# BillyXYB/TransEditor

Hardware: AMD Instinct MI355X
Metric: 256x256 images/sec/GPU, G+D fwd+bwd, batch 16; 1/2/4/8-GPU scaling (higher is better)
Workload: dtype f32

## Files before the change

include/te_hip.h:

```cpp
#ifndef TE_HIP_H
#define TE_HIP_H

#include <stdint.h>

#ifdef __cplusplus
extern "C" {
#endif

#define TE_ABI_VERSION 3

#define TE_ERR_NULL -1
#define TE_ERR_SHAPE -2
#define TE_ERR_UNSUPPORTED -3
#define TE_ERR_WORKSPACE -4

typedef void* te_stream_t;

int te_version(void);
const char* te_last_error_string(void);
const char* te_arch(void);

int te_bias_act_f32(float* out, const float* x, const float* b, const float* ref, int act, int grad,
                    float alpha, float scale, int64_t size_x, int64_t step_b, int64_t size_b,
                    te_stream_t stream);
int te_bias_act_f16(void* out, const void* x, const void* b, const void* ref, int act, int grad,
                    float alpha, float scale, int64_t size_x, int64_t step_b, int64_t size_b,
                    te_stream_t stream);
int te_bias_act_f64(double* out, const double* x, const double* b, const double* ref, int act, int grad,
                    float alpha, float scale, int64_t size_x, int64_t step_b, int64_t size_b,
                    te_stream_t stream);

int64_t te_bias_act_bwd_ws_floats(int64_t outer, int64_t C, int64_t inner);
int te_bias_act_bwd_f32(float* gi, float* gb, float* ws, const float* g, const float* ref, float alpha, float scale,
                        int64_t outer, int64_t C, int64_t inner, te_stream_t stream);
int te_bias_act_bwd_rgb_supported(int64_t outer, int64_t C, int64_t inner);
int te_bias_act_bwd_rgb_f32(float* gi, float* gb, float* ws, const float* g, const float* ref, const float* grgb, const float* wrgb,
                            const float* srgb, float wscale, float alpha, float scale, int64_t outer, int64_t C, int64_t inner,
                            te_stream_t stream);

int te_upfirdn2d_f32(float* out, const float* x, const float* k, int64_t major, int in_h, int in_w,
                     int minor, int kh, int kw, int up_x, int up_y, int down_x, int down_y, int pad_x0,
                     int pad_x1, int pad_y0, int pad_y1, const float* b, int64_t size_b, int act,
                     float alpha, float scale, te_stream_t stream);
int te_upfirdn2d_f16(void* out, const void* x, const void* k, int64_t major, int in_h, int in_w,
                     int minor, int kh, int kw, int up_x, int up_y, int down_x, int down_y, int pad_x0,
                     int pad_x1, int pad_y0, int pad_y1, te_stream_t stream);
int te_upfirdn2d_f64(double* out, const double* x, const double* k, int64_t major, int in_h, int in_w,
                     int minor, int kh, int kw, int up_x, int up_y, int down_x, int down_y, int pad_x0,
                     int pad_x1, int pad_y0, int pad_y1, te_stream_t stream);


#define TE_CONV_3X3 0
#define TE_CONV_T2 1
#define TE_CONV_S2 2
#define TE_CONV_1X1 3
#define TE_CONV_3X3W 4
#define TE_CONV_3X3W6 5

#define TE_CONV_S2S6 6

#define TE_CONV_T2S6 7

#define TE_CONV_1X1S6 8
#define TE_CONV_KINDS 9

#define TE_PACK_FWD 0
#define TE_PACK_DGRAD 1
#define TE_PACK_SWAP 2
#define TE_PACK_WFWD 3
#define TE_PACK_WDGRAD 4
#define TE_PACK_W6FWD 5
#define TE_PACK_W6DGRAD 6
#define TE_PACK_S6FWD 7
#define TE_PACK_S6SWAP 8
#define TE_PACK_T6FWD 9
#define TE_PACK_T6SWAP 10
#define TE_PACK_P6FWD 11
#define TE_PACK_P6DGRAD 12
#define TE_PACK_KINDS 13

int64_t te_conv_packed_numel(int kind_pack, int Co, int Ci, int ksize);
int te_conv_pack_weights_f32(float* wp, const float* w, float wscale, int kind_pack, int Co, int Ci,
                             int ksize, te_stream_t stream);
int te_conv_pack_weights2_f32(float* wp_a, int kind_a, float* wp_b, int kind_b, const float* w, float wscale, int Co, int Ci,
                              int ksize, te_stream_t stream);

int te_conv_pack_weights_multi_f32(int n, float* const* wp, const float* const* w, const float* wscale, const int* kind_pack,
                                   const int* Co, const int* Ci, const int* ksize, te_stream_t stream);

int te_conv_f32(float* out, const float* in, const float* wp, const float* isc, const float* osc,
                const float* bias, int act, int kind, int B, int K, int M, int H, int W,
                te_stream_t stream);
int te_conv_splitk_count(int kind, int B, int K, int M, int H, int W);
int te_conv_wino_supported(int B, int K, int M, int H, int W);
int te_conv_wino6_supported(int B, int K, int M, int H, int W);
int te_conv_s2s6_supported(int B, int K, int M, int H, int W);
int te_conv_t2s6_supported(int B, int K, int M, int H, int W);
int te_conv_p1s6_supported(int B, int K, int M, int H, int W);
int te_conv_wino6_form(int form);
int te_conv_wino6_tiles_per_block(int n);
int te_conv_s2s6_form(int form);
int te_conv_t2s6_form(int form);
int64_t te_conv_t2s6_ws_floats(int B, int K, int H);
int te_conv_ws_f32(float* out, float* ws, const float* in, const float* wp, const float* isc, const float* osc,
                   const float* bias, int act, int kind, int B, int K, int M, int H, int W, te_stream_t stream);
int te_conv_res_f32(float* out, float* ws, const float* in, const float* wp, const float* isc, const float* osc,
                    const float* bias, const float* res, const float* mask_ref, float mask_gain, int act, int kind, int B,
                    int K, int M, int H, int W, te_stream_t stream);

int te_wgrad_slab_count(int kind, int B, int Co, int Ci, int H, int W);
int te_wgrad_pair_form(int kind, int Co, int Ci, int H, int W);
int te_wgrad_split_supported(int kind, int Co, int Ci, int H, int W);
int te_wgrad_split_bf16(int on);
int te_wgrad_t2_wide(int on);
enum { TE_WG6_FP32 = 0, TE_WG6_3X3 = 1, TE_WG6_3X3_PAIR = 2, TE_WG6_T2_WIDE = 3, TE_WG6_T2 = 4, TE_WG6_T2_MASKED = 5, TE_WG6_1X1 = 6 };
int te_wgrad6_form(int kind, int B, int Co, int Ci, int H, int W, int NB);
int te_wgrad_f32(float* slabs, const float* g, const float* x, int kind, int B, int Co, int Ci, int H,
                 int W, int S, te_stream_t stream);
int te_wgrad_group_plan(int kind, int B, int Co, int Ci, int H, int W, int* NB, int* S);
int te_wgrad_group_f32(float* slabs, const float* g, const float* x, int kind, int B, int Co, int Ci, int H, int W, int S, int NB,
                       te_stream_t stream);

int64_t te_wgrad_reduce_ws_floats(int B, int S, int Co, int Ci, int taps, int want_w, int want_isc, int want_osc);
int te_wgrad_reduce_f32(float* gw, float* gisc, float* gosc, float* ws, const float* slabs, const float* w,
                        float wscale, const float* isc, const float* osc, int B, int S, int Co, int Ci,
                        int taps, te_stream_t stream);

int te_rgb_supported(int M, int K, int HW);
int te_rgb_fwd_f32(float* out, const float* x, const float* w, const float* isc, const float* bias, float wscale, int B,
                   int K, int HW, te_stream_t stream);
int te_rgb_dgrad_f32(float* gx, const float* g, const float* w, const float* isc, float wscale, int B, int K, int HW,
                     te_stream_t stream);
int te_rgb_expand_f32(float* out, const float* x3, const float* w, const float* bias, int act, float wscale, int B, int K,
                      int HW, te_stream_t stream);
int te_rgb_wgrad_slab_count(int B, int K, int HW);
int te_rgb_wgrad_f32(float* slabs, const float* g, const float* x, int B, int K, int HW, int S, te_stream_t stream);
int te_rgb_wgrad_sum_f32(float* slabs, const float* g, const float* x, int B, int K, int HW, int S, te_stream_t stream);

int te_attn_fwd_f32(float* o, float* sim, const float* q, const float* k, const float* v, float scale,
                    int N, int G, int M, int L, int D, te_stream_t stream);
int te_attn_bwd_f32(float* gq, float* gk, float* gv, const float* go, const float* gsim_or_null,
                    const float* q, const float* k, const float* v, const float* sim, float scale, int N,
                    int G, int M, int L, int D, te_stream_t stream);

int te_blur_actgrad_tiles(int in_h, int in_w, int kh, int kw, int pad_x0, int pad_x1, int pad_y0, int pad_y1);
int te_blur_actgrad_f32(float* gx, float* partial, const float* g, const float* ref, const float* k, int64_t major, int in_h,
                        int in_w, int kh, int kw, int pad_x0, int pad_x1, int pad_y0, int pad_y1, float alpha, float scale,
                        te_stream_t stream);
int te_blur_gradact_f32(float* gx, float* partial, const float* g, const float* ref, const float* k, int64_t major, int in_h,
                        int in_w, int kh, int kw, int pad_x0, int pad_x1, int pad_y0, int pad_y1, float alpha, float scale,
                        te_stream_t stream);

int te_upfirdn2d_plan(int64_t major, int in_h, int in_w, int minor, int kh, int kw, int up_x, int up_y, int down_x, int down_y,
                      int pad_x0, int pad_x1, int pad_y0, int pad_y1, int* zgroups, int* tiles);
int te_blur_actgrad_plan(int64_t major, int in_h, int in_w, int kh, int kw, int pad_x0, int pad_x1, int pad_y0, int pad_y1,
                         int* zgroups, int* tiles);
int te_blur_gradact_plan(int64_t major, int in_h, int in_w, int kh, int kw, int pad_x0, int pad_x1, int pad_y0, int pad_y1,
                         int* zgroups, int* tiles);
int64_t te_upfirdn2d_direct_cover(int64_t outputs);
int64_t te_chan_scale_cover(int64_t rows, int64_t hw, int aligned16);
int64_t te_bias_act_f32_cover(int64_t size_x, int64_t step_b, int aligned16, int* vec);
int64_t te_bias_act_any_cover(int64_t size_x);
int64_t te_conv_finalize_cover(int64_t outputs);
int64_t te_small_gemm_splitk_finish_cover(int I, int J);
int te_conv_pack_plan(int kind_pack, int Co, int Ci, int ksize, int* blocks, int* tiles);
int te_wgrad_reduce_plan(int B, int S, int Co, int Ci, int taps, int* parts, int64_t* cover);

int te_small_gemm_f32(float* c, float* pre, const float* a, const float* b, const float* bias, const float* residual,
                      float* arowsum, float rs_scale, int I, int J, int K, int64_t sai, int64_t sak, int64_t sbk,
                      int64_t sbj, float alpha, float beta, int act, te_stream_t stream);

int te_small_gemm_splitk_f32(float* c, float* pre, float* ws, int S, const float* a, const float* b, const float* bias,
                             const float* residual, int I, int J, int K, int64_t sai, int64_t sak, int64_t sbk, int64_t sbj,
                             float alpha, float beta, int act, te_stream_t stream);

int te_minibatch_stddev_fwd_f32(float* y, const float* x, int B, int group, int C, int HW, float eps, te_stream_t stream);
int te_minibatch_stddev_bwd_f32(float* gx, const float* gy, const float* x, int B, int group, int C, int HW, float eps,
                                te_stream_t stream);

int te_layer_norm_supported(int64_t R, int N);
int te_layer_norm_fwd_f32(float* y, float* stats, const float* x, int64_t R, int N, float eps, te_stream_t stream);
int te_layer_norm_bwd_f32(float* gx, const float* g, const float* y, const float* stats, int64_t R, int N, te_stream_t stream);

int te_pixel_norm_supported(int64_t B, int D, int C);
int te_pixel_norm_fwd_f32(float* y, float* r, const float* x, int64_t B, int D, int C, float eps, te_stream_t stream);
int te_pixel_norm_bwd_f32(float* gx, const float* g, const float* y, const float* r, int64_t B, int D, int C, te_stream_t stream);

int te_small_gemm_batched_f32(float* c, const float* a, const float* b, const float* bias, int nz, int64_t za, int64_t zc,
                              int64_t zb, int64_t zbias, const int64_t* b_tab, const int64_t* bias_tab, int I, int J, int K,
                              int64_t sai, int64_t sak, int64_t sbk, int64_t sbj, int64_t sci, int64_t scj, float alpha,
                              float beta, int act, te_stream_t stream);

int te_demod_fwd_f32(float* d, float* wsq, const float* w, const float* s, float wscale, float eps, int B, int Co, int Ci,
                     int T, te_stream_t stream);
int te_demod_bwd_f32(float* gw, float* gs, const float* gd, const float* d, const float* w, const float* wsq,
                     const float* s, float wscale, int B, int Co, int Ci, int T, int accumulate, te_stream_t stream);

int te_mt_adam_f32(const int64_t* table, const int32_t* chunks, int n_tensors, int n_chunks, int chunk_elems, double lr,
                   double beta1, double beta2, double eps, int step, te_stream_t stream);
int te_mt_ema_f32(const int64_t* table, const int32_t* chunks, int n_tensors, int n_chunks, int chunk_elems, double decay,
                  te_stream_t stream);

int te_chan_scale_f32(float* out, const float* x, const float* s, int64_t rows, int64_t hw, te_stream_t stream);
int te_chan_dot_f32(float* out, const float* a, const float* b, int64_t rows, int64_t hw, te_stream_t stream);

int te_lpips_stem_fwd_f32(float* out, const float* x, const float* w, const float* b, int N, int H, int W, te_stream_t stream);
int te_lpips_stem_dgrad_f32(float* gx, const float* g, const float* y1, const float* w, int N, int H, int W, te_stream_t stream);
int te_maxpool2_fwd_f32(float* out, const float* x, int64_t planes, int H, int W, te_stream_t stream);
int te_maxpool2_bwd_f32(float* gx, const float* g, const float* x, int64_t planes, int H, int W, te_stream_t stream);
int te_lpips_normalize_f32(float* out, const float* x, int N, int C, int64_t HW, te_stream_t stream);
int te_lpips_head_blocks(int64_t HW);
int te_lpips_head_fwd_f32(float* partial, const float* f, const float* t, const float* w, int N, int Nt, int C, int64_t HW,
                          te_stream_t stream);
int te_lpips_dist_f32(float* d, const float* const* partial, const int64_t* hw, int L, int N, te_stream_t stream);
int te_lpips_head_bwd_f32(float* gf, const float* gin, const float* gd, const float* f, const float* t, const float* w, int N, int Nt,
                          int C, int64_t HW, int relu_mask, te_stream_t stream);
int te_lpips_pair_head_fwd_f32(float* partial, const float* f, const float* w, int N, int C, int64_t HW, te_stream_t stream);
int te_crop_resize_bilinear_f32(float* out, const float* img, int B, int H, int W, int y0, int x0, int hc, int wc, int h, int w,
                                te_stream_t stream);

int64_t te_noise_reg_ws_floats(const int* sizes, int n, int B);
int te_noise_reg_fwd_f32(float* loss, float* ws, float* const* maps, const int* sizes, int n, int B, te_stream_t stream);
int te_noise_reg_bwd_f32(float* const* grads, float* tws, const float* gloss, const float* ws, float* const* maps, const int* sizes,
                         int n, int B, te_stream_t stream);
int te_noise_normalize_f32(float* const* maps, const int* sizes, int n, int B, te_stream_t stream);

int64_t te_prdc_ws_bytes(int N, int M, int D, int k);
int te_row_sqnorm_f32(float* out, const float* x, int N, int D, te_stream_t stream);
int te_prdc_knn_f32(float* r2, const float* x, const float* nx, int N, int D, int k, void* ws, te_stream_t stream);
int te_prdc_counts_f32(int32_t* col_count, int32_t* row_any, float* row_min, const float* x, const float* nx, const float* rr2,
                       const float* y, const float* ny, const float* rf2, int N, int M, int D, void* ws, te_stream_t stream);

int te_vgg_stem_fwd_f32(float* out, const float* x, const float* w, const float* b, int N, int H, int W, te_stream_t stream);
int te_adaptive_avgpool_f32(float* out, const float* x, int64_t planes, int H, int W, int OH, int OW, te_stream_t stream);
// ... 65 lines not shown
```

transeditor_amd/_lib.py:

```python
import ctypes as C
import os

import torch

from . import _abi

_HERE = os.path.dirname(os.path.abspath(__file__))
LIB_PATH = os.path.join(_HERE, 'libte_hip.so')
HEADER_PATH = os.path.join(_HERE, '..', 'include', 'te_hip.h')
_lib = _protos = None

CONV_3X3, CONV_T2, CONV_S2, CONV_1X1, CONV_3X3W, CONV_3X3W6, CONV_S2S6, CONV_T2S6, CONV_1X1S6 = 0, 1, 2, 3, 4, 5, 6, 7, 8
(PACK_FWD, PACK_DGRAD, PACK_SWAP, PACK_WFWD, PACK_WDGRAD, PACK_W6FWD, PACK_W6DGRAD, PACK_S6FWD, PACK_S6SWAP, PACK_T6FWD,
 PACK_T6SWAP, PACK_P6FWD, PACK_P6DGRAD) = range(13)


def _header_text():
    if not os.path.exists(HEADER_PATH):
        raise RuntimeError(f'{HEADER_PATH} is missing: the bindings of libte_hip.so are read from it')
    with open(HEADER_PATH) as f:
        return f.read()


def _prototypes():
# ... 69 lines not shown
                           + (f'contiguous={t.is_contiguous()} ' if dense else '') + '(no CPU path exists)')
    _on_current_device(t)
    return t.data_ptr()


_ptr_as = _ptr


def _raw(t):
    return _ptr(t, dense=False)


def _stream():
    return torch.cuda.current_stream().cuda_stream


def _aligned16(t):
    if t is None or t.data_ptr() % 16 == 0:
        return t
    return t.clone(memory_format=torch.contiguous_format)


_OTHER = {torch.float16: 'f16', torch.float64: 'f64'}


def _dispatch(x):
    return (_OTHER[x.dtype], x.dtype) if x.dtype in _OTHER else ('f32', torch.float32)


def _inner(shape):
    n = 1
    for d in shape[2:]:
        n *= d
    return n


@_op
def bias_act(x, b, ref, act, grad, alpha, scale):
    x = x.contiguous()
    sfx, dt = _dispatch(x)
    out = torch.empty_like(x)
    _launch('te_bias_act_' + sfx, _ptr(out, dt), _ptr(x, dt), _ptr(b, dt), _ptr(ref, dt), act, grad, alpha, scale, x.numel(),
            _inner(x.shape), b.numel() if b is not None else 1)
    return out


def _bias_grad_buffers(want_bias, outer, Cn, inner, device):
    if not want_bias:
        return None, None
    n = lib().te_bias_act_bwd_ws_floats(outer, Cn, inner)
    return (torch.empty(Cn, device=device, dtype=torch.float32),
            torch.empty(n, device=device, dtype=torch.float32) if n > 0 else None)


@_op
def bias_act_bwd(g, ref, alpha, scale, want_bias=True):
    g = g.contiguous()
    if g.dtype in _OTHER:
        gi = bias_act(g, None, ref, 3, 1, alpha, scale)
        return gi, (gi.sum(dim=[0] + list(range(2, gi.ndim))) if want_bias else None)
    gi = torch.empty_like(g)
    Cn, inner = g.shape[1], _inner(g.shape)
    gb, ws = _bias_grad_buffers(want_bias, g.shape[0], Cn, inner, g.device)
    _launch('te_bias_act_bwd_f32', _ptr(gi), _ptr(gb), _ptr(ws), _ptr(g), _ptr(ref), alpha, scale, g.shape[0], Cn, inner)
    return gi, gb


def bias_act_bwd_rgb_supported(shape):
    return bool(lib().te_bias_act_bwd_rgb_supported(shape[0], shape[1], _inner(shape)))


@_op
def bias_act_bwd_rgb(g, ref, grgb, wrgb, srgb, wscale, alpha, scale, want_bias=True):
    ref, grgb = _aligned16(ref.contiguous()), _aligned16(grgb.contiguous())
    g = _aligned16(g.contiguous()) if g is not None else None
    gi = torch.empty_like(ref)
    Cn, inner = ref.shape[1], _inner(ref.shape)
    gb, ws = _bias_grad_buffers(want_bias, ref.shape[0], Cn, inner, ref.device)
    _launch('te_bias_act_bwd_rgb_f32', _ptr(gi), _ptr(gb), _ptr(ws), _ptr(g), _ptr(ref), _ptr(grgb), _ptr(wrgb.contiguous()),
            _ptr(srgb.contiguous()) if srgb is not None else None, wscale, alpha, scale, ref.shape[0], Cn, inner)
    return gi, gb


@_op
def upfirdn2d_raw(x, k, up, down, pad, bias=None, act=0, alpha=0.2, scale=1.0):
    x = x.contiguous()
    B, Cn, H, W = x.shape
    kh, kw = k.shape
    px0, px1, py0, py1 = pad
    oh = (H * up[1] + py0 + py1 - kh) // down[1] + 1
    ow = (W * up[0] + px0 + px1 - kw) // down[0] + 1
    if oh <= 0 or ow <= 0:
        raise RuntimeError(f'upfirdn2d: empty output {oh}x{ow}')
    out = torch.empty(B, Cn, oh, ow, device=x.device, dtype=x.dtype)
    sfx, dt = _dispatch(x)
    if sfx != 'f32':
        if bias is not None or act:
            raise RuntimeError('upfirdn2d: the fused bias / activation epilogue exists in fp32 only')
        k = k.to(dt)
    args = [_ptr(out, dt), _ptr(x, dt), _ptr(k.contiguous(), dt), B * Cn, H, W, 1, kh, kw, up[0], up[1], down[0], down[1],
            px0, px1, py0, py1]
    if sfx == 'f32':
        args += [_ptr(bias), bias.numel() if bias is not None else 1, act, alpha, scale]
    _launch('te_upfirdn2d_' + sfx, *args)
    return out


@_op
def blur_actgrad(g, ref, k_flipped, pad, alpha, scale):
    g, ref = g.contiguous(), ref.contiguous()
    B, Cn, H, W = g.shape
    kh, kw = k_flipped.shape
    px0, px1, py0, py1 = pad
    tiles = lib().te_blur_actgrad_tiles(H, W, kh, kw, px0, px1, py0, py1)
    if tiles <= 0:
        raise RuntimeError(f'te_blur_actgrad_tiles failed ({tiles})')
    gx = torch.empty(B, Cn, H + py0 + py1 - kh + 1, W + px0 + px1 - kw + 1, device=g.device, dtype=g.dtype)
    partial = torch.empty(B, Cn, tiles, device=g.device, dtype=g.dtype)
    _launch('te_blur_actgrad_f32', _ptr(gx), _ptr(partial), _ptr(g), _ptr(ref), _ptr(k_flipped.contiguous()), B * Cn, H, W, kh, kw, px0,
            px1, py0, py1, alpha, scale)
    return gx, partial.sum(dim=(0, 2))


@_op
def blur_gradact(g, ref, k_flipped, pad, alpha, scale):
    g, ref = g.contiguous(), ref.contiguous()
    B, Cn, H, W = g.shape
    kh, kw = k_flipped.shape
    px0, px1, py0, py1 = pad
    oh, ow = H + py0 + py1 - kh + 1, W + px0 + px1 - kw + 1
    if tuple(ref.shape) != (B, Cn, oh, ow):
        raise RuntimeError(f'blur_gradact: ref {tuple(ref.shape)} is not the shape of the adjoint blur output {(B, Cn, oh, ow)}')
    tiles = lib().te_blur_actgrad_tiles(H, W, kh, kw, px0, px1, py0, py1)
    if tiles <= 0:
        raise RuntimeError(f'te_blur_actgrad_tiles failed ({tiles})')
    gx = torch.empty(B, Cn, oh, ow, device=g.device, dtype=g.dtype)
    partial = torch.empty(B, Cn, tiles, device=g.device, dtype=g.dtype)
    _launch('te_blur_gradact_f32', _ptr(gx), _ptr(partial), _ptr(g), _ptr(ref), _ptr(k_flipped.contiguous()), B * Cn, H, W, kh, kw, px0,
            px1, py0, py1, alpha, scale)
    return gx, partial.sum(dim=(0, 2))


@_op
def conv_pack(w, kind_pack, wscale=1.0):
    w = w.contiguous()
    Co, Ci, ks, _ = w.shape
    n = lib().te_conv_packed_numel(kind_pack, Co, Ci, ks)
    wp = torch.empty(n, device=w.device, dtype=w.dtype)
    _launch('te_conv_pack_weights_f32', _ptr(wp), _ptr(w), wscale, kind_pack, Co, Ci, ks)
    return wp


@_op
def conv_pack2(w, kind_a, kind_b, wscale=1.0):
    w = w.contiguous()
    Co, Ci, ks, _ = w.shape
    wa = torch.empty(lib().te_conv_packed_numel(kind_a, Co, Ci, ks), device=w.device, dtype=w.dtype)
    wb = torch.empty(lib().te_conv_packed_numel(kind_b, Co, Ci, ks), device=w.device, dtype=w.dtype)
    _launch('te_conv_pack_weights2_f32', _ptr(wa), kind_a, _ptr(wb), kind_b, _ptr(w), wscale, Co, Ci, ks)
    return wa, wb


@_op
def conv_pack_multi(jobs):
    n = len(jobs)
    if not n:
        return
    for wp, w, _, _ in jobs:
        if not (w.is_contiguous() and wp.is_contiguous()):
            raise RuntimeError('te_hip: conv_pack_multi needs dense weights and buffers')
    arr = lambda ty, vals: (ty * n)(*vals)
    _launch('te_conv_pack_weights_multi_f32', n, arr(C.c_void_p, [_ptr(j[0]) for j in jobs]), arr(C.c_void_p, [_ptr(j[1]) for j in jobs]),
            arr(C.c_float, [float(j[3]) for j in jobs]), arr(C.c_int, [int(j[2]) for j in jobs]),
            arr(C.c_int, [j[1].shape[0] for j in jobs]), arr(C.c_int, [j[1].shape[1] for j in jobs]),
            arr(C.c_int, [j[1].shape[2] for j in jobs]))


def wino_ok(B, K, M, H, W):
    return bool(lib().te_conv_wino_supported(B, K, M, H, W))


def s2s6_ok(B, K, M, H, W):
    return bool(lib().te_conv_s2s6_supported(B, K, M, H, W))


def t2s6_ok(B, K, M, H, W):
    return bool(lib().te_conv_t2s6_supported(B, K, M, H, W))


def p1s6_ok(B, K, M, H, W):
    return bool(lib().te_conv_p1s6_supported(B, K, M, H, W))


def wino6_form(form=-1):
    return int(lib().te_conv_wino6_form(form))


def wino6_tiles_per_block(n=-1):
    return int(lib().te_conv_wino6_tiles_per_block(n))


def s2s6_form(form=-1):
    return int(lib().te_conv_s2s6_form(form))


def t2s6_form(form=-1):
    return int(lib().te_conv_t2s6_form(form))


def wino6_ok(B, K, M, H, W):
    return bool(lib().te_conv_wino6_supported(B, K, M, H, W))


def conv_out_shape(kind, B, M, H, W):
    if kind in (CONV_T2, CONV_T2S6):
        return (B, M, 2 * H + 1, 2 * W + 1)
    return (B, M, H, W)


@_op
def conv(x, wp, kind, M, H, W, isc=None, osc=None, bias=None, act=0, res=None, mask_ref=None, mask_gain=1.0):
    x = x.contiguous()
    if kind == CONV_1X1S6:
        x = _aligned16(x)
    res = _aligned16(res.contiguous()) if res is not None else None
    mask_ref = _aligned16(mask_ref.contiguous()) if mask_ref is not None else None
    B, K = x.shape[0], x.shape[1]
    out = torch.empty(conv_out_shape(kind, B, M, H, W), device=x.device, dtype=x.dtype)
    if res is not None and tuple(res.shape) != tuple(out.shape):
        raise RuntimeError(f'te_hip: residual {tuple(res.shape)} does not match the convolution output {tuple(out.shape)}')
    if mask_ref is not None and tuple(mask_ref.shape) != tuple(out.shape):
        raise RuntimeError(f'te_hip: mask reference {tuple(mask_ref.shape)} does not match the convolution output {tuple(out.shape)}')
    S = lib().te_conv_splitk_count(kind, B, K, M, H, W)
    if S < 1:
        raise RuntimeError(f'te_conv_splitk_count failed ({S})')
    ws = torch.empty((S,) + tuple(out.shape), device=x.device, dtype=x.dtype) if S > 1 else None
    if kind == CONV_T2S6:
        ws = torch.empty(B * K * H, device=x.device, dtype=x.dtype)
    _launch('te_conv_res_f32', _ptr(out), _ptr(ws), _ptr(x), _ptr(wp), _ptr(isc), _ptr(osc), _ptr(bias), _ptr(res), _ptr(mask_ref),
            mask_gain, act, kind, B, K, M, H, W)
    return out


@_op
def wgrad_slabs(g, x, kind, H, W, group=False):
    g, x = g.contiguous(), x.contiguous()
    B, Co, Ci = g.shape[0], g.shape[1], x.shape[1]
    taps = 1 if kind == CONV_1X1 else 9
    if group:
        nb, sc = C.c_int(0), C.c_int(0)
        _check(lib().te_wgrad_group_plan(kind, B, Co, Ci, H, W, C.byref(nb), C.byref(sc)), 'te_wgrad_group_plan')
        if nb.value > 1:
            slabs = torch.empty(B // nb.value, sc.value, Co, Ci, taps, device=g.device, dtype=g.dtype)
            _launch('te_wgrad_group_f32', _ptr(slabs), _ptr(g), _ptr(x), kind, B, Co, Ci, H, W, sc.value, nb.value)
            return slabs
    S = lib().te_wgrad_slab_count(kind, B, Co, Ci, H, W)
    if S <= 0:
        raise RuntimeError(f'te_wgrad_slab_count failed ({S})')
    slabs = torch.empty(B, S, Co, Ci, taps, device=g.device, dtype=g.dtype)
    _launch('te_wgrad_f32', _ptr(slabs), _ptr(g), _ptr(x), kind, B, Co, Ci, H, W, S)
    return slabs


def wgrad_t2_wide(on=-1):
    return int(lib().te_wgrad_t2_wide(on))


def wgrad_split(on=-1):
    return int(lib().te_wgrad_split_bf16(on))


def wgrad_split_ok(kind, Co, Ci, H, W):
    return bool(lib().te_wgrad_split_supported(kind, Co, Ci, H, W))


WGRAD6_FORMS = ('fp32', 'w6', 'w6pair', 't2wide', 't2narrow', 't2masked', 'p1')


def wgrad6_form(kind, B, Co, Ci, H, W, NB=1):
    return WGRAD6_FORMS[lib().te_wgrad6_form(kind, B, Co, Ci, H, W, NB)]


def wgrad_pair_form(kind, Co, Ci, H, W):
    return bool(lib().te_wgrad_pair_form(kind, Co, Ci, H, W))


@_op
def wgrad_reduce(slabs, w, wscale=1.0, isc=None, osc=None, want_w=True, want_isc=False, want_osc=False):
    B, S, Co, Ci, taps = slabs.shape
    dev, dt = slabs.device, slabs.dtype
    gw = torch.empty(Co, Ci, taps, device=dev, dtype=dt) if want_w else None
    gisc = torch.empty(B, Ci, device=dev, dtype=dt) if want_isc else None
    gosc = torch.empty(B, Co, device=dev, dtype=dt) if want_osc else None
    n = lib().te_wgrad_reduce_ws_floats(B, S, Co, Ci, taps, int(want_w), int(want_isc), int(want_osc))
    if n < 0:
        raise RuntimeError(f'te_wgrad_reduce_ws_floats failed ({n})')
    ws = torch.empty(n, device=dev, dtype=dt) if n > 0 else None
    _launch('te_wgrad_reduce_f32', _ptr(gw), _ptr(gisc), _ptr(gosc), _ptr(ws), _ptr(slabs), _ptr(w.contiguous()), wscale, _ptr(isc),
            _ptr(osc), B, S, Co, Ci, taps)
    return gw, gisc, gosc


def rgb_supported(M, K, HW):
    return bool(lib().te_rgb_supported(M, K, HW))


@_op
def rgb_fwd(x, w, isc, bias, wscale=1.0):
    x = _aligned16(x.contiguous())
    B, K, H, W = x.shape
    out = torch.empty(B, 3, H, W, device=x.device, dtype=x.dtype)
    _launch('te_rgb_fwd_f32', _ptr(out), _ptr(x), _ptr(w.contiguous()), _ptr(isc), _ptr(bias), wscale, B, K, H * W)
    return out


@_op
def rgb_dgrad(g, w, isc, K, wscale=1.0):
    g = _aligned16(g.contiguous())
    B, _, H, W = g.shape
    gx = torch.empty(B, K, H, W, device=g.device, dtype=g.dtype)
    _launch('te_rgb_dgrad_f32', _ptr(gx), _ptr(g), _ptr(w.contiguous()), _ptr(isc), wscale, B, K, H * W)
# ... 844 lines not shown
```

transeditor_amd/csrc/bias_act.hip:

```cpp
#include "te_common.h"
#include <hip/hip_fp16.h>

namespace {

__device__ __forceinline__ float act_one(float x, float r, int mode, float alpha) {
    switch (mode) {
        case 30: return x > 0.f ? x : x * alpha;
        case 31: return r > 0.f ? x : x * alpha;
        case 12:
        case 32: return 0.f;
        default: return x;
    }
}

__global__ __launch_bounds__(256) void bias_act_vec4_kernel(float4* __restrict__ out, const float4* __restrict__ x,
                                                            const float* __restrict__ b, const float4* __restrict__ ref,
                                                            int mode, float alpha, float scale, uint32_t n4,
                                                            uint32_t step_b4, uint32_t size_b) {
    const uint32_t stride = gridDim.x * blockDim.x;
    for (uint32_t i = blockIdx.x * blockDim.x + threadIdx.x; i < n4; i += stride) {
        float4 v = x[i];
        if (b) {
            const float bb = b[(i / step_b4) % size_b];
            v.x += bb; v.y += bb; v.z += bb; v.w += bb;
        }
        float4 r = make_float4(0.f, 0.f, 0.f, 0.f);
        if (ref) r = ref[i];
        float4 y;
        y.x = act_one(v.x, r.x, mode, alpha) * scale;
        y.y = act_one(v.y, r.y, mode, alpha) * scale;
        y.z = act_one(v.z, r.z, mode, alpha) * scale;
        y.w = act_one(v.w, r.w, mode, alpha) * scale;
        out[i] = y;
    }
}

__global__ __launch_bounds__(256) void bias_act_scalar_kernel(float* __restrict__ out, const float* __restrict__ x,
                                                              const float* __restrict__ b, const float* __restrict__ ref,
                                                              int mode, float alpha, float scale, int64_t n,
                                                              int64_t step_b, int64_t size_b) {
    const int64_t stride = (int64_t)gridDim.x * blockDim.x;
    for (int64_t i = (int64_t)blockIdx.x * blockDim.x + threadIdx.x; i < n; i += stride) {
        float v = x[i];
        if (b) v += b[(i / step_b) % size_b];
        const float r = ref ? ref[i] : 0.f;
        out[i] = act_one(v, r, mode, alpha) * scale;
    }
}

__device__ __forceinline__ float wave_sum(float v) {
#pragma unroll
    for (int off = 32; off > 0; off >>= 1) v += __shfl_down(v, off, 64);
    return v;
}

__device__ __forceinline__ float block_sum_256(float v, float* lds4) {
    v = wave_sum(v);
    const int lane = threadIdx.x & 63, wid = threadIdx.x >> 6;
    if (lane == 0) lds4[wid] = v;
    __syncthreads();
    return lds4[0] + lds4[1] + lds4[2] + lds4[3];
}

constexpr int kBwdVecPerThread = 4;
__global__ __launch_bounds__(256) void bias_act_bwd_rows_kernel(float4* __restrict__ gi, float* __restrict__ part,
                                                                const float4* __restrict__ g, const float4* __restrict__ ref,
                                                                float alpha, float scale, uint32_t C, uint32_t inner4) {
    __shared__ float lds4[4];
    const uint32_t c = blockIdx.y, n = blockIdx.z;
    const size_t row = ((size_t)n * C + c) * inner4;
    const uint32_t base = blockIdx.x * (256 * kBwdVecPerThread);
    float acc = 0.f;
#pragma unroll
    for (int it = 0; it < kBwdVecPerThread; ++it) {
        const uint32_t i = base + it * 256 + threadIdx.x;
        if (i < inner4) {
            const float4 gv = g[row + i], rv = ref[row + i];
            float4 o;
            o.x = gv.x * (rv.x > 0.f ? 1.f : alpha) * scale;
            o.y = gv.y * (rv.y > 0.f ? 1.f : alpha) * scale;
            o.z = gv.z * (rv.z > 0.f ? 1.f : alpha) * scale;
            o.w = gv.w * (rv.w > 0.f ? 1.f : alpha) * scale;
            gi[row + i] = o;
            acc += (o.x + o.y) + (o.z + o.w);
        }
    }
    if (part) {
        const float tot = block_sum_256(acc, lds4);
        if (threadIdx.x == 0) part[((size_t)c * gridDim.z + n) * gridDim.x + blockIdx.x] = tot;
    }
}

__global__ __launch_bounds__(64) void bias_parts_sum_kernel(float* __restrict__ gb, const float* __restrict__ part, uint32_t parts) {
    const float* p = part + (size_t)blockIdx.x * parts;
    float acc = 0.f;
    for (uint32_t j = threadIdx.x; j < parts; j += 64) acc += p[j];
    acc = wave_sum(acc);
    if (threadIdx.x == 0) gb[blockIdx.x] = acc;
}

__global__ __launch_bounds__(256) void bias_act_bwd_rgb_rows_kernel(float4* __restrict__ gi, float* __restrict__ part,
                                                                    const float4* __restrict__ g, const float4* __restrict__ ref,
                                                                    const float4* __restrict__ grgb, const float* __restrict__ wrgb,
                                                                    const float* __restrict__ srgb, float wscale, float alpha,
                                                                    float scale, uint32_t C, uint32_t inner4) {
    __shared__ float lds4[4];
    const uint32_t c = blockIdx.y, n = blockIdx.z;
    const size_t row = ((size_t)n * C + c) * inner4;
    const size_t rrow = (size_t)n * 3 * inner4;
    const float sc = (srgb ? srgb[(size_t)n * C + c] : 1.f) * wscale;
    const float c0 = sc * wrgb[c], c1 = sc * wrgb[C + c], c2 = sc * wrgb[2 * C + c];
    const uint32_t base = blockIdx.x * (256 * kBwdVecPerThread);
    float acc = 0.f;
#pragma unroll
    for (int it = 0; it < kBwdVecPerThread; ++it) {
        const uint32_t i = base + it * 256 + threadIdx.x;
        if (i < inner4) {
            const float4 rv = ref[row + i];
            const float4 r0 = grgb[rrow + i], r1 = grgb[rrow + inner4 + i], r2 = grgb[rrow + 2 * (size_t)inner4 + i];
            float4 gv = g ? g[row + i] : make_float4(0.f, 0.f, 0.f, 0.f);
            gv.x += c0 * r0.x + c1 * r1.x + c2 * r2.x;
            gv.y += c0 * r0.y + c1 * r1.y + c2 * r2.y;
            gv.z += c0 * r0.z + c1 * r1.z + c2 * r2.z;
            gv.w += c0 * r0.w + c1 * r1.w + c2 * r2.w;
            float4 o;
            o.x = gv.x * (rv.x > 0.f ? 1.f : alpha) * scale;
            o.y = gv.y * (rv.y > 0.f ? 1.f : alpha) * scale;
            o.z = gv.z * (rv.z > 0.f ? 1.f : alpha) * scale;
            o.w = gv.w * (rv.w > 0.f ? 1.f : alpha) * scale;
            gi[row + i] = o;
            acc += (o.x + o.y) + (o.z + o.w);
        }
    }
    if (part) {
        const float tot = block_sum_256(acc, lds4);
        if (threadIdx.x == 0) part[((size_t)c * gridDim.z + n) * gridDim.x + blockIdx.x] = tot;
    }
}

__global__ __launch_bounds__(256) void bias_act_bwd_chan_kernel(float* __restrict__ gi, float* __restrict__ gb,
                                                                const float* __restrict__ g, const float* __restrict__ ref,
                                                                float alpha, float scale, int64_t outer, int64_t C,
                                                                int64_t inner) {
    __shared__ float lds4[4];
    const int64_t c = blockIdx.x;
    const int64_t per = outer * inner;
    float acc = 0.f;
    for (int64_t e = threadIdx.x; e < per; e += 256) {
        const int64_t n = e / inner, i = e - n * inner;
        const int64_t idx = (n * C + c) * inner + i;
        const float o = g[idx] * (ref[idx] > 0.f ? 1.f : alpha) * scale;
        gi[idx] = o;
        acc += o;
    }
    if (gb) {
        const float tot = block_sum_256(acc, lds4);
        if (threadIdx.x == 0) gb[c] = tot;
    }
}

__global__ __launch_bounds__(256) void bias_act_bwd_2d_kernel(float* __restrict__ gi, float* __restrict__ gb,
                                                              const float* __restrict__ g, const float* __restrict__ ref,
                                                              float alpha, float scale, int64_t N, int64_t C) {
    const int64_t c = (int64_t)blockIdx.x * 256 + threadIdx.x;
    if (c >= C) return;
    float acc = 0.f;
    for (int64_t n = 0; n < N; ++n) {
        const int64_t idx = n * C + c;
        const float o = g[idx] * (ref[idx] > 0.f ? 1.f : alpha) * scale;
        gi[idx] = o;
        acc += o;
    }
    if (gb) gb[c] = acc;
}

inline int bias_act_grid(int64_t items) { return (int)std::min<int64_t>(te::cdiv(items, 256), te::kNumCU * 8); }
inline bool bias_act_vec(int64_t size_x, bool has_b, int64_t step_b, bool al16) {
    return (size_x % 4 == 0) && (!has_b || step_b % 4 == 0) && al16 && (size_x / 4 < (int64_t)0xFFFFFFFF);
}

template <typename T> struct AccOf { typedef T type; };
template <> struct AccOf<__half> { typedef float type; };

template <typename T>
__global__ __launch_bounds__(256) void bias_act_any_kernel(T* __restrict__ out, const T* __restrict__ x, const T* __restrict__ b,
                                                           const T* __restrict__ ref, int mode, float alpha_, float scale_,
                                                           int64_t n, int64_t step_b, int64_t size_b) {
    typedef typename AccOf<T>::type A;
    const A alpha = (A)(T)alpha_, scale = (A)(T)scale_;
    const int64_t stride = (int64_t)gridDim.x * blockDim.x;
    for (int64_t i = (int64_t)blockIdx.x * blockDim.x + threadIdx.x; i < n; i += stride) {
        A v = (A)x[i];
        if (b) v += (A)b[(i / step_b) % size_b];
        const A r = ref ? (A)ref[i] : (A)0;
        A y;
        switch (mode) {
            case 30: y = v > (A)0 ? v : v * alpha; break;
            case 31: y = r > (A)0 ? v : v * alpha; break;
            case 12:
            case 32: y = (A)0; break;
            default: y = v;
        }
        out[i] = (T)(y * scale);
    }
}

template <typename T>
int bias_act_any(T* out, const T* x, const T* b, const T* ref, int act, int grad, float alpha, float scale, int64_t size_x,
                 int64_t step_b, int64_t size_b, te_stream_t stream_, const char* what) {
    TE_REQUIRE(out && x, TE_ERR_NULL, "%s: out/x is NULL", what);
    TE_REQUIRE(size_x >= 0, TE_ERR_SHAPE, "%s: size_x < 0", what);
    TE_REQUIRE(!b || (step_b > 0 && size_b > 0), TE_ERR_SHAPE, "%s: bias given but step_b/size_b <= 0", what);
    if (size_x == 0) return 0;
    const int grid = bias_act_grid(size_x);
// ... 20 lines not shown
                               te_stream_t stream_) {
    TE_REQUIRE(out && x, TE_ERR_NULL, "te_bias_act_f32: out/x is NULL");
    TE_REQUIRE(size_x >= 0, TE_ERR_SHAPE, "te_bias_act_f32: size_x < 0");
    TE_REQUIRE(!b || (step_b > 0 && size_b > 0), TE_ERR_SHAPE, "te_bias_act_f32: bias given but step_b/size_b <= 0");
    if (size_x == 0) return 0;
    hipStream_t stream = (hipStream_t)stream_;
    const int mode = act * 10 + grad;
    const bool vec = bias_act_vec(size_x, b != nullptr, step_b, te::aligned16(out) && te::aligned16(x) && (!ref || te::aligned16(ref)));
    if (vec) {
        const uint32_t n4 = (uint32_t)(size_x / 4);
        const int grid = bias_act_grid(n4);
        bias_act_vec4_kernel<<<grid, 256, 0, stream>>>((float4*)out, (const float4*)x, b, (const float4*)ref, mode, alpha,
                                                       scale, n4, b ? (uint32_t)(step_b / 4) : 1u,
                                                       b ? (uint32_t)size_b : 1u);
    } else {
        const int grid = bias_act_grid(size_x);
        bias_act_scalar_kernel<<<grid, 256, 0, stream>>>(out, x, b, ref, mode, alpha, scale, size_x, b ? step_b : 1,
                                                         b ? size_b : 1);
    }
    return te::launch_status("te_bias_act_f32");
}

extern "C" int64_t te_bias_act_f32_cover(int64_t size_x, int64_t step_b, int aligned16_, int* vec_out) {
    if (size_x <= 0 || step_b < 0) return TE_ERR_SHAPE;
    const bool vec = bias_act_vec(size_x, step_b > 0, step_b, aligned16_ != 0);
    if (vec_out) *vec_out = vec ? 1 : 0;
    return (int64_t)bias_act_grid(vec ? size_x / 4 : size_x) * 256 * (vec ? 4 : 1);
}

extern "C" int64_t te_bias_act_any_cover(int64_t size_x) {
    return size_x > 0 ? (int64_t)bias_act_grid(size_x) * 256 : TE_ERR_SHAPE;
}

static bool bwd_rows_path(int64_t outer, int64_t C, int64_t inner) {
    return inner % 4 == 0 && inner >= 1024 && C <= 65535 && outer <= 65535;
}

extern "C" int64_t te_bias_act_bwd_ws_floats(int64_t outer, int64_t C, int64_t inner) {
    if (outer <= 0 || C <= 0 || inner <= 0 || !bwd_rows_path(outer, C, inner)) return 0;
    return C * outer * te::cdiv(inner / 4, 256 * kBwdVecPerThread);
}

extern "C" int te_bias_act_bwd_f32(float* gi, float* gb, float* ws, const float* g, const float* ref, float alpha, float scale,
                                   int64_t outer, int64_t C, int64_t inner, te_stream_t stream_) {
    TE_REQUIRE(gi && g && ref, TE_ERR_NULL, "te_bias_act_bwd_f32: gi/g/ref is NULL");
    TE_REQUIRE(outer >= 0 && C > 0 && inner > 0, TE_ERR_SHAPE, "te_bias_act_bwd_f32: bad dims");
    if (outer == 0) return 0;
    hipStream_t stream = (hipStream_t)stream_;
    if (inner == 1) {
        bias_act_bwd_2d_kernel<<<(int)te::cdiv(C, 256), 256, 0, stream>>>(gi, gb, g, ref, alpha, scale, outer, C);
    } else if (bwd_rows_path(outer, C, inner) && te::aligned16(gi) && te::aligned16(g) && te::aligned16(ref) && (!gb || ws)) {
        const uint32_t inner4 = (uint32_t)(inner / 4);
        dim3 grid((unsigned)te::cdiv(inner4, 256 * kBwdVecPerThread), (unsigned)C, (unsigned)outer);
        bias_act_bwd_rows_kernel<<<grid, 256, 0, stream>>>((float4*)gi, gb ? ws : nullptr, (const float4*)g, (const float4*)ref, alpha,
                                                           scale, (uint32_t)C, inner4);
        if (gb) bias_parts_sum_kernel<<<(int)C, 64, 0, stream>>>(gb, ws, (uint32_t)(grid.x * grid.z));
    } else {
        bias_act_bwd_chan_kernel<<<(int)C, 256, 0, stream>>>(gi, gb, g, ref, alpha, scale, outer, C, inner);
    }
    return te::launch_status("te_bias_act_bwd_f32");
}

extern "C" int te_bias_act_bwd_rgb_supported(int64_t outer, int64_t C, int64_t inner) {
    return (outer > 0 && C > 0 && bwd_rows_path(outer, C, inner)) ? 1 : 0;
}

extern "C" int te_bias_act_bwd_rgb_f32(float* gi, float* gb, float* ws, const float* g, const float* ref, const float* grgb,
                                       const float* wrgb, const float* srgb, float wscale, float alpha, float scale, int64_t outer,
                                       int64_t C, int64_t inner, te_stream_t stream_) {
    TE_REQUIRE(gi && ref && grgb && wrgb, TE_ERR_NULL, "te_bias_act_bwd_rgb_f32: gi/ref/grgb/wrgb is NULL");
    TE_REQUIRE(!gb || ws, TE_ERR_NULL, "te_bias_act_bwd_rgb_f32: the bias gradient needs the workspace (te_bias_act_bwd_ws_floats)");
    TE_REQUIRE(te_bias_act_bwd_rgb_supported(outer, C, inner), TE_ERR_UNSUPPORTED,
               "te_bias_act_bwd_rgb_f32: needs inner %% 4 == 0 and inner >= 1024 (use te_rgb_dgrad_f32 + te_bias_act_bwd_f32)");
    TE_REQUIRE(te::aligned16(gi) && (!g || te::aligned16(g)) && te::aligned16(ref) && te::aligned16(grgb), TE_ERR_UNSUPPORTED,
               "te_bias_act_bwd_rgb_f32: 16-byte aligned tensors required");
    const uint32_t inner4 = (uint32_t)(inner / 4);
    dim3 grid((unsigned)te::cdiv(inner4, 256 * kBwdVecPerThread), (unsigned)C, (unsigned)outer);
    hipStream_t stream = (hipStream_t)stream_;
    bias_act_bwd_rgb_rows_kernel<<<grid, 256, 0, stream>>>((float4*)gi, gb ? ws : nullptr, (const float4*)g, (const float4*)ref,
                                                          (const float4*)grgb, wrgb, srgb, wscale, alpha, scale, (uint32_t)C, inner4);
    if (gb) bias_parts_sum_kernel<<<(int)C, 64, 0, stream>>>(gb, ws, (uint32_t)(grid.x * grid.z));
    return te::launch_status("te_bias_act_bwd_rgb_f32");
}
```

transeditor_amd/csrc/conv.hip:

```cpp
#include "conv_common.h"
#ifdef TE_CONV_PROF
#define TE_PROF
#endif
#ifdef TE_CONV_PROF2
#define TE_PROF2
#endif
#include "te_prof.h"

namespace {

constexpr int T2_KC0 = 16;
PROF_BUFFER(conv, 8192 * 8)
template <int KIND, int TC> struct Cfg;
template <int KIND> struct Cfg<KIND, 0> { static constexpr int WM = 2, MBW = 2, NBW = 2, KC = 8, NSP = (KIND == TE_CONV_S2) ? 3 : (KIND == TE_CONV_3X3 ? 2 : 1), NQ = (KIND == TE_CONV_S2) ? 5 : 2; };
template <int KIND> struct Cfg<KIND, 1> { static constexpr int WM = 2, MBW = 1, NBW = (KIND == TE_CONV_S2) ? 2 : 4, KC = 8, NSP = (KIND == TE_CONV_S2) ? 3 : (KIND == TE_CONV_3X3 ? 2 : 1), NQ = (KIND == TE_CONV_S2) ? 5 : 4; };
template <int KIND> struct Cfg<KIND, 2> { static constexpr int WM = 1, MBW = 1, NBW = 2, KC = 8, NSP = (KIND == TE_CONV_S2) ? 5 : (KIND == TE_CONV_3X3 ? 2 : 1), NQ = (KIND == TE_CONV_S2) ? 10 : 4; };
template <> struct Cfg<TE_CONV_T2, 0> { static constexpr int WM = 2, MBW = 1, NBW = 2, KC = T2_KC0, NSP = 1, NQ = 3; };
template <> struct Cfg<TE_CONV_T2, 1> { static constexpr int WM = 2, MBW = 1, NBW = 1, KC = 16, NSP = 1, NQ = 2; };
template <> struct Cfg<TE_CONV_T2, 2> { static constexpr int WM = 1, MBW = 1, NBW = 1, KC = 16, NSP = 1, NQ = 3; };
template <> struct Cfg<TE_CONV_1X1, 3> { static constexpr int WM = 2, MBW = 2, NBW = 2, KC = 64, NSP = 1, NQ = 8; };
template <int KIND, int TC> constexpr int tile_bm() { return Cfg<KIND, TC>::WM * Cfg<KIND, TC>::MBW * 32; }
template <int KIND, int TC> constexpr int tile_cells() { return (4 / Cfg<KIND, TC>::WM) * Cfg<KIND, TC>::NBW * 32; }

struct ConvArgs {
// ... 899 lines not shown
    for (int base = 0; base < n; base += 64) {
        const int cnt = std::min(64, n - base);
        PackJobs P{};
        int64_t biggest = 0;
        for (int i = 0; i < cnt; ++i) {
            const int e = base + i;
            TE_REQUIRE(wp[e] && w[e], TE_ERR_NULL, "%s: NULL pointer in job %d", what, e);
            TE_REQUIRE(Co[e] > 0 && Ci[e] > 0 && (ksize[e] == 1 || ksize[e] == 3), TE_ERR_SHAPE, "%s: bad dims in job %d", what, e);
            TE_REQUIRE(pack_kind_ok(kind_pack[e]), TE_ERR_UNSUPPORTED, "%s: bad kind in job %d", what, e);
            const PackDims d = pack_dims(kind_pack[e], Co[e], Ci[e], ksize[e]);
            const PackDesc& pd = pack_desc(kind_pack[e]);
            TE_REQUIRE((pd.taps == ANY_TAPS || d.ntap == pd.taps) && d.M % pd.mmul == 0 && d.K % pd.kmul == 0, TE_ERR_UNSUPPORTED,
                       "%s: layout %d needs a weight of %d tap(s) with M %% %d == 0 and K %% %d == 0 (job %d)", what, kind_pack[e], pd.taps, pd.mmul, pd.kmul, e);
            P.j[i] = PackJob{wp[e], w[e], wscale[e], kind_pack[e], Ci[e], d.ntap, d.K, d.M, d.Kp, d.Mp};
            biggest = std::max<int64_t>(biggest, pack_job_tiles(d));
        }
        dim3 grid(pack_grid_x(biggest), (unsigned)cnt);
        pack_weights_multi_kernel<<<grid, 256, 0, s>>>(P);
    }
    return te::launch_status(what);
}

extern "C" int te_conv_pack_weights_f32(float* wp, const float* w, float wscale, int kind_pack, int Co, int Ci, int ksize,
                                        te_stream_t stream_) {
    return pack_launch("te_conv_pack_weights_f32", 1, &wp, &w, &wscale, &kind_pack, &Co, &Ci, &ksize, (hipStream_t)stream_);
}

extern "C" int te_conv_pack_weights2_f32(float* wp_a, int kind_a, float* wp_b, int kind_b, const float* w, float wscale, int Co,
                                         int Ci, int ksize, te_stream_t stream_) {
    float* wp[2] = {wp_a, wp_b};
    const float* ws[2] = {w, w};
    const float sc[2] = {wscale, wscale};
    const int kinds[2] = {kind_a, kind_b}, co[2] = {Co, Co}, ci[2] = {Ci, Ci}, ks[2] = {ksize, ksize};
    return pack_launch("te_conv_pack_weights2_f32", 2, wp, ws, sc, kinds, co, ci, ks, (hipStream_t)stream_);
}

extern "C" int te_conv_pack_weights_multi_f32(int n, float* const* wp, const float* const* w, const float* wscale,
                                              const int* kind_pack, const int* Co, const int* Ci, const int* ksize,
                                              te_stream_t stream_) {
    return pack_launch("te_conv_pack_weights_multi_f32", n, wp, w, wscale, kind_pack, Co, Ci, ksize, (hipStream_t)stream_);
}

constexpr int SPLITK_MINSTAGES = 4, SPLITK_BLOCKS = 2;

struct ConvPlan { int tc, ksplit, kchunk; };
static ConvPlan conv_plan(int kind, int B, int K, int M, int H, int W) {
    ConvPlan pl;
    const int Kp = roundup(K, KPAD);
    const bool t2k = (kind == TE_CONV_T2);
    int tc = tile_class(M);
    constexpr int T2_TC1_LIMIT = 1024 * 128;
    if (t2k && tc == 0 && (int64_t)B * H * W * te::cdiv(M, 64) <= (int64_t)T2_TC1_LIMIT) tc = 1;
    pl.tc = tc;
    const TileDims td = tile_dims(kind, tc);
    int r[3][4];
    conv_regions(kind, H, W, r);
    const int rh = r[0][2], rw = r[0][3];
    const CellTile t = first_cell_tile(td.cells, rh, rw);
    const int64_t base_blocks = (int64_t)te::cdiv(rw, t.TW) * te::cdiv(rh, t.TH) * te::cdiv(B, t.NS) * te::cdiv(M, td.BM);
    const int stages = Kp / td.KC;
    int ks = 1;
    if (base_blocks < te::kNumCU) ks = (int)std::min<int64_t>(te::cdiv(SPLITK_BLOCKS * te::kNumCU, base_blocks), std::max(1, stages / SPLITK_MINSTAGES));
    pl.ksplit = std::max(1, ks);
    pl.kchunk = (int)te::cdiv(stages, pl.ksplit) * td.KC;
    pl.ksplit = (int)te::cdiv(Kp, pl.kchunk);
    if (kind == TE_CONV_1X1 && tc == 0 && pl.ksplit == 1 && t.NS == 1 && K % 64 == 0) pl.tc = 3;
    return pl;
}

extern "C" int64_t te_conv_t2s6_ws_floats(int B, int K, int H) { return (B > 0 && K > 0 && H > 0) ? (int64_t)B * K * H : TE_ERR_SHAPE; }

static int conv_finalize_grid(int64_t total) { return (int)std::min<int64_t>(te::cdiv(total, 256), te::kNumCU * 8); }

extern "C" int64_t te_conv_finalize_cover(int64_t outputs) {
    return outputs > 0 ? (int64_t)conv_finalize_grid(outputs) * 256 : TE_ERR_SHAPE;
}

extern "C" int te_conv_splitk_count(int kind, int B, int K, int M, int H, int W) {
    if (B <= 0 || K <= 0 || M <= 0 || H <= 0 || W <= 0 || kind < 0 || kind >= TE_CONV_KINDS) return TE_ERR_SHAPE;
    if (kind == TE_CONV_3X3W || kind == TE_CONV_3X3W6 || kind == TE_CONV_S2S6 || kind == TE_CONV_T2S6 || kind == TE_CONV_1X1S6) return 1;
    return conv_plan(kind, B, K, M, H, W).ksplit;
}

extern "C" int te_conv_res_f32(float* out, float* ws, const float* in, const float* wp, const float* isc, const float* osc,
                               const float* bias, const float* res, const float* mask_ref, float mask_gain, int act, int kind,
                               int B, int K, int M, int H, int W, te_stream_t stream_) {
    TE_REQUIRE(out && in && wp, TE_ERR_NULL, "te_conv_f32: out/in/wp is NULL");
    TE_REQUIRE(!(res || mask_ref) || (kind != TE_CONV_T2 && kind != TE_CONV_T2S6), TE_ERR_UNSUPPORTED,
               "te_conv_res_f32: no residual / mask epilogue for the transposed kind");
    TE_REQUIRE(B > 0 && K > 0 && M > 0 && H > 0 && W > 0, TE_ERR_SHAPE, "te_conv_f32: bad dims");
    TE_REQUIRE(act == 0 || act == 3 || act == 4, TE_ERR_UNSUPPORTED, "te_conv_f32: act must be 0, 3 or 4");
    TE_REQUIRE(kind >= 0 && kind < TE_CONV_KINDS, TE_ERR_UNSUPPORTED, "te_conv_f32: unknown kind %d", kind);
    hipStream_t s = (hipStream_t)stream_;
    if (kind == TE_CONV_1X1S6) {
        TE_REQUIRE(!isc && !osc && !bias && !mask_ref && act == 0, TE_ERR_UNSUPPORTED,
                   "te_conv_f32(TE_CONV_1X1S6): plain product + residual only (no scales, bias, activation or mask)");
        return te_p1s6_launch(out, in, wp, res, B, K, M, H, W, s);
    }
    if (kind == TE_CONV_3X3W) return te_wino_launch(out, in, wp, isc, osc, bias, res, mask_ref, mask_gain, act, B, K, M, H, W, s);
    if (kind == TE_CONV_3X3W6) return te_wino6_launch(out, in, wp, isc, osc, bias, res, mask_ref, mask_gain, act, B, K, M, H, W, s);
    if (kind == TE_CONV_S2S6) return te_s2s6_launch(out, in, wp, isc, osc, bias, res, mask_ref, mask_gain, act, B, K, M, H, W, s);
    if (kind == TE_CONV_T2S6) {
        const int rc = te_t2s6_launch(out, in, wp, isc, osc, bias, act, B, K, M, H, W, s, ws);
        if (rc) return rc;
        return te_t2s6_edge_launch(out, in, wp + t6_plain_offset(K, M), isc, osc, bias, act, B, K, M, H, W, roundup(K, KPAD), roundup(M, MPAD),
                                   s, ws);
    }
    ConvArgs a{};
    a.out = out; a.ws = ws; a.in = in; a.wp = wp; a.isc = isc; a.osc = osc; a.bias = bias; a.res = res; a.mref = mask_ref; a.mgain = mask_gain; a.act = act;
    a.B = B; a.K = K; a.M = M; a.Kp = roundup(K, KPAD); a.Mp = roundup(M, MPAD); a.H = H; a.W = W;
    const ConvPlan pl = conv_plan(kind, B, K, M, H, W);
    a.ksplit = pl.ksplit; a.kchunk = pl.kchunk;
    if (a.ksplit > 1 && !a.ws) {
        a.ksplit = 1;
        a.kchunk = a.Kp;
    }
    if (a.ksplit == 1) a.ws = nullptr;
    int r[3][4];
    const int n = conv_regions(kind, H, W, r);
    a.Hi = a.Ho = H; a.Wi = a.Wo = W;
    int rc = 0;
    switch (kind) {
        case TE_CONV_3X3: rc = launch_regions<TE_CONV_3X3>(a, r, n, s, pl.tc); break;
        case TE_CONV_1X1: rc = launch_regions<TE_CONV_1X1>(a, r, n, s, pl.tc); break;
        case TE_CONV_S2: a.Hi = 2 * H + 1; a.Wi = 2 * W + 1; rc = launch_regions<TE_CONV_S2>(a, r, n, s, pl.tc); break;
        default: a.Ho = 2 * H + 1; a.Wo = 2 * W + 1; rc = launch_regions<TE_CONV_T2>(a, r, n, s, pl.tc); break;
    }
    if (rc) return rc;
    if (a.ksplit > 1 && (a.ws || osc || bias || act)) {
        const int plane = a.Ho * a.Wo;
        const int64_t total = (int64_t)B * M * plane;
        conv_finalize_kernel<<<conv_finalize_grid(total), 256, 0, s>>>(out, a.ws, a.ksplit, osc, bias, res, mask_ref, mask_gain, act, M,
                                                                        plane, total);
    }
    return te::launch_status("te_conv_f32");
}

extern "C" int te_conv_ws_f32(float* out, float* ws, const float* in, const float* wp, const float* isc, const float* osc,
                              const float* bias, int act, int kind, int B, int K, int M, int H, int W, te_stream_t stream_) {
    return te_conv_res_f32(out, ws, in, wp, isc, osc, bias, nullptr, nullptr, 1.f, act, kind, B, K, M, H, W, stream_);
}

extern "C" int te_conv_f32(float* out, const float* in, const float* wp, const float* isc, const float* osc,
                           const float* bias, int act, int kind, int B, int K, int M, int H, int W, te_stream_t stream_) {
    return te_conv_ws_f32(out, nullptr, in, wp, isc, osc, bias, act, kind, B, K, M, H, W, stream_);
}
```

transeditor_amd/csrc/conv_common.h:

```cpp
#pragma once
#include "te_common.h"
#include <stdlib.h>
#include <algorithm>

typedef float f32x16 __attribute__((ext_vector_type(16)));
typedef float f32x4 __attribute__((ext_vector_type(4)));

constexpr unsigned OOBH = 0x40000000u;

__device__ __forceinline__ __amdgpu_buffer_rsrc_t make_rsrc(const float* p, unsigned bytes) {
    return __builtin_amdgcn_make_buffer_rsrc((void*)p, 0, bytes, 0x00020000);
}
__device__ __forceinline__ float buf_load(__amdgpu_buffer_rsrc_t r, unsigned off) {
    return __builtin_bit_cast(float, __builtin_amdgcn_raw_buffer_load_b32(r, off, 0, 0));
}

constexpr int KPAD = 16;
constexpr int MPAD = 128;
constexpr int NTHREADS = 256;


int te_wino_launch(float* out, const float* in, const float* U, const float* isc, const float* osc, const float* bias, const float* res,
                   const float* mask_ref, float mask_gain, int act, int B, int K, int M, int H, int W, hipStream_t s);
int te_wino6_launch(float* out, const float* in, const float* U, const float* isc, const float* osc, const float* bias, const float* res,
                    const float* mask_ref, float mask_gain, int act, int B, int K, int M, int H, int W, hipStream_t s);
int te_s2s6_launch(float* out, const float* in, const float* U, const float* isc, const float* osc, const float* bias, const float* res,
                   const float* mask_ref, float mask_gain, int act, int B, int K, int M, int H, int W, hipStream_t s);
int te_t2s6_launch(float* out, const float* in, const float* U, const float* isc, const float* osc, const float* bias, int act,
                   int B, int K, int M, int H, int W, hipStream_t s, float* colbuf = nullptr);
int te_t2s6_edge_launch(float* out, const float* in, const float* wplain, const float* isc, const float* osc, const float* bias, int act,
                        int B, int K, int M, int H, int W, int Kp, int Mp, hipStream_t s, const float* colbuf = nullptr);
int te_p1s6_launch(float* out, const float* in, const float* U, const float* res, int B, int K, int M, int H, int W, hipStream_t s);
```

transeditor_amd/csrc/s2s6.hip:

```cpp
#include "split6_common.h"
#ifdef S2_PROF
#define TE_PROF
#endif
#include "te_prof.h"

namespace {

constexpr int WT = 512, GT = 256, KC = 16, BM = 64;
constexpr int TH = 8, TWO = 16, PH = 4;
constexpr int IR = 2 * PH + 1, IC = 2 * TWO + 1;
constexpr int CI = 18;
constexpr int NTAP = 9;
constexpr int U_SLOTS = 3 * NTAP * 2;
constexpr int TP_PLANE = IR * 2 * 2 * CI * 4;
constexpr int TP_DWORDS = 3 * TP_PLANE;
constexpr int NG = (IC + 3) / 4;
constexpr int N_ITEMS = IR * NG * 8;
constexpr int P_IN = (N_ITEMS + GT - 1) / GT;
constexpr int N_SLOT = P_IN + 16 * P_IN;
constexpr int SLOT0 = NTAP * 6 - N_SLOT;
constexpr int UA_TAPS = 5;

PROF_BUFFER(s2s6, 2048 * 8 * 8)

struct S2Args {
    float* out; const float* in; const u32x4* U; const float* isc; const float* osc; const float* bias; const float* res;
    const float* mref; float mgain; int act;
    int B, K, M, H, W, Hi, Wi, ntiles, mblocks, tiles_x, tiles_y, nt8;
};


template <bool ISC, bool TWOIMG>
__device__ __attribute__((optnone)) void s2s6_body(const S2Args& p) {
    constexpr int NIMG = TWOIMG ? 2 : 1;
    extern __shared__ __attribute__((aligned(16))) unsigned char smem_raw[];
    u32x4* ul = reinterpret_cast<u32x4*>(smem_raw);
    const int tid = threadIdx.x, lane = tid & 63, l31 = lane & 31, half = lane >> 5;
    const int wid = __builtin_amdgcn_readfirstlane(tid >> 6);
    const int grp = wid >> 2, wq = wid & 3, wm = wq >> 1, wrl = wq & 1, gt = tid & (GT - 1);
    unsigned* tl = reinterpret_cast<unsigned*>(smem_raw + U_SLOTS * 1024) + grp * TP_DWORDS;
    const u32x4* tl4 = reinterpret_cast<const u32x4*>(tl);
    int tile, mbq;
    if (!split6_tile(p.ntiles, p.nt8, p.mblocks, tile, mbq)) return;
    const int tx = tile % p.tiles_x, ty = (tile / p.tiles_x) % p.tiles_y, b = tile / (p.tiles_x * p.tiles_y);
    const int x0 = tx * TWO, y0 = ty * TH, yh = y0 + PH * grp;
    const size_t iplane = (size_t)p.Hi * p.Wi, oplane = (size_t)p.H * p.W;
    const float* inb = p.in + (size_t)b * p.K * iplane;
    const float* iscb = ISC ? p.isc + (size_t)b * p.K : nullptr;

    f32x16 acc[NIMG], accl[NIMG];
#pragma unroll
    for (int m = 0; m < NIMG; ++m)
#pragma unroll
        for (int r = 0; r < 16; ++r) { acc[m][r] = 0.f; accl[m][r] = 0.f; }

    unsigned g_off[P_IN];
    int l_off[P_IN];
    bool last_col[P_IN], live[P_IN];
    unsigned q2[P_IN];
#pragma unroll
    for (int i = 0; i < P_IN; ++i) {
        const int e = gt + GT * i;
        live[i] = e < N_ITEMS;
        const int ee = live[i] ? e : 0;
        const int cg = ee % NG, q = (ee / NG) & 7, row = ee / (NG * 8);
        last_col[i] = cg == NG - 1;
        g_off[i] = (unsigned)((2 * q * p.Hi + 2 * yh + row) * p.Wi + 2 * x0 + 4 * cg - (last_col[i] ? 3 : 0));
        l_off[i] = (((row * 2 + (q >> 2)) * 2) * CI + 2 * cg) * 4 + (q & 3);
        q2[i] = 2u * q;
    }
    const int MT = p.M >> 5;
    f32x4 rin[P_IN][2];
    f32x2 rsc[P_IN];
#pragma unroll
    for (int i = 0; i < P_IN; ++i) rsc[i] = f32x2{1.f, 1.f};
    const int nstage = p.K / KC, nimg = NIMG * nstage;
    auto fetch_scales = [&](int s) {
        if (ISC) {
#pragma unroll
            for (int i = 0; i < P_IN; ++i) rsc[i] = *reinterpret_cast<const f32x2u*>(iscb + s * KC + q2[i]);
        }
    };
    auto fetch_item = [&](int i, int s) {
#pragma unroll
        for (int h2 = 0; h2 < 2; ++h2)
            rin[i][h2] = *reinterpret_cast<const f32x4u*>(inb + ((size_t)s * KC + h2) * iplane + g_off[i]);
    };
    auto issue = [&](int s) {
        fetch_scales(s);
#pragma unroll
        for (int i = 0; i < P_IN; ++i) fetch_item(i, s);
    };
    auto issue_u = [&](int uh, int j) {
        const u32x4* us = p.U + (size_t)(TWOIMG ? j >> 1 : j) * 27 * MT * 64;
        const int mb = TWOIMG ? 2 * mbq + (j & 1) : mbq;
        const int ntap = uh ? NTAP - UA_TAPS : UA_TAPS, tap0 = uh ? UA_TAPS : 0, n = ntap * 6;
#pragma unroll
        for (int r = 0; r < 8; ++r) {
            const int jw = wq + 4 * r;
            if (jw >= n) break;
            const int piece = jw / (ntap * 2), rem = jw % (ntap * 2), tap = tap0 + (rem >> 1), mt = rem & 1;
            const int pt = piece * NTAP + tap;
            const u32x4* g = us + ((size_t)pt * MT + 2 * mb + mt) * 64 + (unsigned)lane;
            __builtin_amdgcn_global_load_lds((const __attribute__((address_space(1))) void*)g,
                                             (__attribute__((address_space(3))) void*)(ul + (pt * 2 + mt) * 64), 16, 0, 0);
        }
    };
    unsigned res[P_IN][4][3];
    float te = 0.f, to = 0.f, fe = 0.f, fo = 0.f;
    auto arith = [&](int k) {
        if (k < 0) {
        } else if (k < P_IN) {
#pragma unroll
            for (int h2 = 0; h2 < 2; ++h2) {
                f32x4 v = rin[k][h2];
                if (last_col[k]) v[0] = v[3];
// ... 103 lines not shown
            _Pragma("unroll")
            for (int i = 0; i < 6; ++i) d[i] = pc[i];
            d[6] = pc[6] | ((__builtin_amdgcn_s_memrealtime() - rstart) << 40);
            d[7] = ((unsigned long long)nstage << 48) | ((__builtin_readcyclecounter() - pstart) & 0xFFFFFFFFFFFFull);
        })
    } else {
        auto multiply = [&](auto mset_tag, int fs) {
            constexpr int MSET = decltype(mset_tag)::value;
#pragma unroll
            for (int q = 0; q < 6; ++q) rd1(0, 0, q);
            __builtin_amdgcn_s_setprio(1);
#pragma unroll
            for (int t = 0; t < NTAP; ++t) {
                const int slot = t & 1;
                if (t == UA_TAPS - 1) split6_barrier();
                __builtin_amdgcn_sched_barrier(0);
#pragma unroll
                for (int q = 0; q < 6; ++q) {
                    split6_product(q, av[slot], bv[slot], acc[MSET], accl[MSET]);
                    if (t + 1 < NTAP && q < 3) { rd1(t + 1, slot ^ 1, 2 * q); rd1(t + 1, slot ^ 1, 2 * q + 1); }
                    const int k = t * 6 + q;
                    if (MSET == 0) {
                        if (k == 5) fetch_scales(fs);
#pragma unroll
                        for (int i = 0; i < P_IN; ++i)
                            if (k == 6 + 12 * i) fetch_item(i, fs);
                    } else {
                        arith(k - SLOT0);
                    }
                    __builtin_amdgcn_sched_barrier(0);
                }
            }
            __builtin_amdgcn_s_setprio(0);
            split6_barrier();
        };
        auto stage = [&](int ph, bool write) {
            const int cs = (ph + 1) >> 1;
            const bool work = cs >= 1 && cs < nimg;
            if (grp == 1 && work) issue_u(1, cs);
            __builtin_amdgcn_sched_barrier(0);
            if (write) write_res();
            if (grp == 1 && work) split6_wait_vm();
            split6_barrier();
            if (grp == 0 && work) {
                issue_u(0, cs);
                split6_wait_vm();
            }
            split6_barrier();
        };
        split6_wait_vm();
        split6_barrier();
        int ph = 0;
        if (grp == 1) { stage(0, false); ph = 1; }
        for (int s = 0; s < nstage; ++s) {
            const int fs = min(s + 1, nstage - 1);
            multiply(std::integral_constant<int, 0>{}, fs);
            stage(ph + 1, false);
            multiply(std::integral_constant<int, 1>{}, fs);
            if (!(grp == 1 && s == nstage - 1)) stage(ph + 3, true);
            ph += 4;
        }
    }

    const float g_pos = p.act == 3 ? 1.4142135623730951f : 1.f;
#pragma unroll
    for (int m = 0; m < NIMG; ++m) {
        const int mbase = (NIMG * mbq + m) * BM + wm * 32;
        const size_t off0 = ((size_t)b * p.M + mbase) * oplane + (size_t)(yh + 2 * wrl + rr) * p.W + x0 + jj;
        float scv[16], biv[16], resv[16], mrefv[16];
#pragma unroll
        for (int r = 0; r < 16; ++r) {
            const int dm = (r & 3) + 8 * (r >> 2) + 4 * half;
            scv[r] = p.osc ? p.osc[(size_t)b * p.M + mbase + dm] : 1.f;
            biv[r] = p.bias ? p.bias[mbase + dm] : 0.f;
        }
        if (p.res) {
#pragma unroll
            for (int r = 0; r < 16; ++r) resv[r] = p.res[off0 + (size_t)((r & 3) + 8 * (r >> 2) + 4 * half) * oplane];
        }
        if (p.mref) {
#pragma unroll
            for (int r = 0; r < 16; ++r) mrefv[r] = p.mref[off0 + (size_t)((r & 3) + 8 * (r >> 2) + 4 * half) * oplane];
        }
#pragma unroll
        for (int r = 0; r < 16; ++r) {
            const int dm = (r & 3) + 8 * (r >> 2) + 4 * half;
            float v = (acc[m][r] + accl[m][r]) * scv[r] + biv[r];
            if (p.act >= 3) v = (v > 0.f ? v : v * 0.2f) * g_pos;
            if (p.res) v += resv[r];
            if (p.mref) v *= mrefv[r] > 0.f ? p.mgain : 0.2f * p.mgain;
            p.out[off0 + (size_t)dm * oplane] = v;
        }
    }
}

template <bool ISC>
__global__ __launch_bounds__(WT, 2) void s2s6_kernel(const S2Args p) { [[clang::always_inline]] s2s6_body<ISC, false>(p); }
template <bool ISC>
__global__ __launch_bounds__(WT, 2) void s2s6q_kernel(const S2Args p) { [[clang::always_inline]] s2s6_body<ISC, true>(p); }

}

PROF_READBACK(s2s6)

extern "C" int te_conv_s2s6_supported(int B, int K, int M, int H, int W) {
    if (!(B > 0 && K >= 32 && K % KC == 0 && M >= BM && M % BM == 0 && H >= TH && H % TH == 0 && W >= TWO && W % TWO == 0)) return 0;
    return ((int64_t)K * (2 * H + 1) * (2 * W + 1) * 4 < 0x7FFFFFFF && (int64_t)B * (H / TH) * (W / TWO) * (M / BM) < 0x7FFFFFF0) ? 1 : 0;
}

static std::atomic<int> g_s2_form{1};
extern "C" int te_conv_s2s6_form(int form) {
    const int old = g_s2_form.load(std::memory_order_relaxed);
    if (form >= 0 && form <= 2) g_s2_form.store(form, std::memory_order_relaxed);
    return old;
}

int te_s2s6_launch(float* out, const float* in, const float* U, const float* isc, const float* osc, const float* bias, const float* res,
                   const float* mask_ref, float mask_gain, int act, int B, int K, int M, int H, int W, hipStream_t s) {
    TE_REQUIRE(te_conv_s2s6_supported(B, K, M, H, W), TE_ERR_UNSUPPORTED,
               "te_conv_f32(TE_CONV_S2S6): needs K %% 16 == 0 (>= 32), M %% 64 == 0, H %% 8 == 0, W %% 16 == 0 (te_conv_s2s6_supported)");
    TE_REQUIRE((reinterpret_cast<uintptr_t>(U) & 15) == 0 && (reinterpret_cast<uintptr_t>(in) & 3) == 0, TE_ERR_UNSUPPORTED,
               "te_conv_f32(TE_CONV_S2S6): 16-byte aligned packed weights required");
    S2Args a{};
    a.out = out; a.in = in; a.U = reinterpret_cast<const u32x4*>(U); a.isc = isc; a.osc = osc; a.bias = bias; a.res = res;
    a.mref = mask_ref; a.mgain = mask_gain; a.act = act;
    a.B = B; a.K = K; a.M = M; a.H = H; a.W = W; a.Hi = 2 * H + 1; a.Wi = 2 * W + 1;
    a.tiles_x = W / TWO; a.tiles_y = H / TH; a.mblocks = M / BM;
    a.ntiles = B * a.tiles_x * a.tiles_y;
    a.nt8 = te::xcd_banded() ? (int)te::cdiv(a.ntiles, 8) : 0;
    const int64_t blocks = te::cdiv(a.ntiles, 8) * 8 * a.mblocks;
    const size_t lds = (size_t)U_SLOTS * 1024 + 2 * (size_t)TP_DWORDS * 4;
    const int form = g_s2_form.load(std::memory_order_relaxed);
    const int64_t blocks_q = te::cdiv(a.ntiles, 8) * 8 * (M / (2 * BM));
    if (split6_two_image(form, M, blocks_q)) {
        a.mblocks = M / (2 * BM);
        SPLIT6_LAUNCH_ISC(s2s6q_kernel, isc, dim3((unsigned)blocks_q), WT, lds, s, a);
    } else {
        SPLIT6_LAUNCH_ISC(s2s6_kernel, isc, dim3((unsigned)blocks), WT, lds, s, a);
    }
    return te::launch_status("te_conv_f32(TE_CONV_S2S6)");
}
```

transeditor_amd/csrc/upfirdn2d.hip:

```cpp
#include "te_common.h"
#include <hip/hip_fp16.h>

namespace {

__host__ __device__ __forceinline__ int fdiv(int a, int b) {
    int q = a / b;
    return (q * b > a) ? q - 1 : q;
}

struct FirParams {
    int in_h, in_w, out_h, out_w;
    int pad_x0, pad_y0;
    int kh, kw, up_x, up_y, down_x, down_y, minor;
    int64_t major;
    int size_b, act;
    float alpha, scale;
    int ext_x, ext_y;
    int tiles_x, tiles_y, zgroups;
};

struct TileId { int bx, by, pg; };
__device__ __forceinline__ TileId xcd_tile(const FirParams& p) {
    const int T = p.tiles_x * p.tiles_y;
    const int xcd = blockIdx.x & 7, j = blockIdx.x >> 3;
    const int t = j % T;
    return TileId{t % p.tiles_x, t / p.tiles_x, xcd + 8 * (j / T)};
}
inline unsigned xcd_grid(FirParams& p, int tiles_x, int tiles_y, int64_t z) {
    p.tiles_x = tiles_x; p.tiles_y = tiles_y;
    p.zgroups = (int)(te::cdiv(z, 8) * 8);
    return (unsigned)((int64_t)p.zgroups * tiles_x * tiles_y);
}

template <bool AG = false>
__device__ __forceinline__ float epilogue(float v, const float* b, int ch, const FirParams& p) {
    if constexpr (AG) return v;
    if (b) v += b[ch];
    if (p.act == 3) v = v > 0.f ? v : v * p.alpha;
    return v * p.scale;
}

constexpr int TOH = 16, TOW = 64;

template <int UP, int DOWN, int KH, int KW, bool AG = false>
__global__ __launch_bounds__(256) void fir_tile_kernel(float* __restrict__ out, const float* __restrict__ x,
                                                       const float* __restrict__ k, const float* __restrict__ b,
                                                       const FirParams p, const float* __restrict__ ref = nullptr,
                                                       float* __restrict__ partial = nullptr) {
    constexpr int TIH = ((TOH - 1) * DOWN + KH - 1) / UP + 1;
    constexpr int TIW = ((TOW - 1) * DOWN + KW - 1) / UP + 1;
    constexpr int TIWP = (TIW + 3) & ~3;
    constexpr int NTY = (KH + UP - 1) / UP, NTX = (KW + UP - 1) / UP;
    static_assert(KH % UP == 0 && KW % UP == 0, "taps must split evenly over the upsampling phases");
    __shared__ __attribute__((aligned(16))) float sx[TIH * TIWP + 4];
    __shared__ float sk[KH * KW];
    __shared__ float sred[4];

    float kf[KH][KW];
#pragma unroll
    for (int a = 0; a < KH; ++a)
#pragma unroll
        for (int c = 0; c < KW; ++c) kf[a][c] = k[(KH - 1 - a) * KW + (KW - 1 - c)];
    if (threadIdx.x < KH * KW) sk[threadIdx.x] = k[KH * KW - 1 - threadIdx.x];

    const TileId tid3 = xcd_tile(p);
    const int ox0 = tid3.bx * TOW, oy0 = tid3.by * TOH;
    const int mid_x0 = ox0 * DOWN + UP - 1 - p.pad_x0, mid_y0 = oy0 * DOWN + UP - 1 - p.pad_y0;
    const int ix0 = fdiv(mid_x0, UP), iy0 = fdiv(mid_y0, UP);
    const int ty = threadIdx.x >> 4, tx = (threadIdx.x & 15) * 4;

    constexpr int NLD = (TIH * TIW + 255) / 256;
    float stage[NLD];
    float rv[AG ? NLD : 1];
    auto fetch = [&](int64_t mj) {
        const float* xin = x + (size_t)mj * p.in_h * p.in_w;
#pragma unroll
        for (int r = 0; r < NLD; ++r) {
            const int e = threadIdx.x + 256 * r;
            const int ry = e / TIW, rx = e - ry * TIW;
            const int gy = iy0 + ry, gx = ix0 + rx;
            const bool ok = e < TIH * TIW && gy >= 0 && gy < p.in_h && gx >= 0 && gx < p.in_w;
            const float v = xin[ok ? (size_t)gy * p.in_w + gx : 0];
            stage[r] = ok ? v : 0.f;
// ... 94 lines not shown
                for (int q = 0; q < 4; ++q) {
                    const int ox = ox0 + tx + q;
                    if (ox < p.out_w) orow[ox] = epilogue<AG>(res[q], b, ch, p);
                }
            }
        }
    }
}

__global__ __launch_bounds__(256) void fir_direct_kernel(float* __restrict__ out, const float* __restrict__ x,
                                                         const float* __restrict__ k, const float* __restrict__ b,
                                                         const FirParams p) {
    const int64_t total = p.major * p.out_h * p.out_w * p.minor;
    const int64_t stride = (int64_t)gridDim.x * blockDim.x;
    for (int64_t e = (int64_t)blockIdx.x * blockDim.x + threadIdx.x; e < total; e += stride) {
        int64_t r = e;
        const int mn = (int)(r % p.minor); r /= p.minor;
        const int ox = (int)(r % p.out_w); r /= p.out_w;
        const int oy = (int)(r % p.out_h);
        const int64_t mj = r / p.out_h;
        const int mid_x = ox * p.down_x + p.up_x - 1 - p.pad_x0, mid_y = oy * p.down_y + p.up_y - 1 - p.pad_y0;
        const int ix0 = fdiv(mid_x, p.up_x), iy0 = fdiv(mid_y, p.up_y);
        const int jx0 = (ix0 + 1) * p.up_x - mid_x - 1, jy0 = (iy0 + 1) * p.up_y - mid_y - 1;
        float acc = 0.f;
        for (int jy = jy0, iy = iy0; jy < p.kh; jy += p.up_y, ++iy) {
            if (iy < 0 || iy >= p.in_h) continue;
            for (int jx = jx0, ix = ix0; jx < p.kw; jx += p.up_x, ++ix) {
                if (ix < 0 || ix >= p.in_w) continue;
                acc += x[(((size_t)mj * p.in_h + iy) * p.in_w + ix) * p.minor + mn] *
                       k[(p.kh - 1 - jy) * p.kw + (p.kw - 1 - jx)];
            }
        }
        out[e] = epilogue(acc, b, b ? (int)(mj % p.size_b) : 0, p);
    }
}

inline int64_t fir_planes_z(int64_t major, int64_t tiles) {
    return std::max<int64_t>(1, std::min<int64_t>(std::min<int64_t>(major, 32768), te::cdiv(6144, tiles)));
}

inline unsigned tile_grid(FirParams& q) {
    const int64_t tiles = te::cdiv(q.out_w, TOW) * te::cdiv(q.out_h, TOH);
    return xcd_grid(q, (int)te::cdiv(q.out_w, TOW), (int)te::cdiv(q.out_h, TOH), fir_planes_z(q.major, tiles));
}

inline int fir_direct_grid(int64_t total) { return (int)std::min<int64_t>(te::cdiv(total, 256), te::kNumCU * 16); }

template <int UP, int DOWN, int KH, int KW>
void launch_tile(float* out, const float* x, const float* k, const float* b, const FirParams& p, hipStream_t s) {
    FirParams q = p;
    dim3 grid(tile_grid(q), 1u, 1u);
    fir_tile_kernel<UP, DOWN, KH, KW><<<grid, 256, 0, s>>>(out, x, k, b, q);
}


constexpr int BOH = 32, BOW = 64;
constexpr int BIH = BOH + 4, BNQ = 18;
constexpr int BST = 128;

typedef float f32x4v __attribute__((ext_vector_type(4)));

template <int MODE, int D, bool EXT>
__global__ __launch_bounds__(256) void blur44_kernel(float* __restrict__ out, const float* __restrict__ x, const float* __restrict__ k,
                                                     const float* __restrict__ b, const FirParams p,
                                                     const float* __restrict__ ref = nullptr, float* __restrict__ partial = nullptr) {
    __shared__ __attribute__((aligned(16))) float sx[BIH * BST];
    __shared__ float sred[4];
    float kf[4][4];
#pragma unroll
    for (int a = 0; a < 4; ++a)
#pragma unroll
        for (int c = 0; c < 4; ++c) kf[a][c] = k[(3 - a) * 4 + (3 - c)];

    const TileId tid3 = xcd_tile(p);
    const int ox0 = tid3.bx * BOW, oy0 = tid3.by * BOH;
    const int ix0 = ox0 - p.pad_x0, iy0 = oy0 - p.pad_y0;
    const int ax0 = ix0 - D;
    const int ty = threadIdx.x >> 4, tx = (threadIdx.x & 15) * 4;
    const unsigned plane_b = (unsigned)p.in_h * p.in_w * 4u;

    constexpr int NIT = BIH * BNQ, NLD = (NIT + 255) / 256;
    f32x4v stage[NLD];
    constexpr bool AG = (MODE == 1);
    f32x4v rv[AG ? NLD : 1];
    unsigned goff[NLD];
    int lds_off[NLD], sh[NLD];
#pragma unroll
    for (int r = 0; r < NLD; ++r) {
        const int e = threadIdx.x + 256 * r;
        const int ry = e / BNQ, q = e - ry * BNQ;
        const int gy = iy0 + ry, gx = ax0 + 4 * q;
        lds_off[r] = ry * BST + 4 * q;
        sh[r] = e < NIT ? 0 : -1;
        goff[r] = 0x80000000u;
        if (e < NIT && gy >= 0 && gy < p.in_h && gx >= 0 && gx < p.in_w) {
            const int gxs = min(gx, p.in_w - 4);
            sh[r] = gx - gxs;
            goff[r] = (unsigned)(gy * p.in_w + gxs) * 4u;
        }
    }
    auto load_tile = [&](const float* base, int64_t mj, f32x4v* dst) {
        const __amdgpu_buffer_rsrc_t rs = __builtin_amdgcn_make_buffer_rsrc((void*)(base + (size_t)mj * p.in_h * p.in_w), 0, plane_b, 0x00020000);
#pragma unroll
        for (int r = 0; r < NLD; ++r) dst[r] = __builtin_bit_cast(f32x4v, __builtin_amdgcn_raw_buffer_load_b128(rs, goff[r], 0, 0));
    };
    const bool edge_x = ax0 + 4 * BNQ > p.in_w;
    auto place = [&](f32x4v L, int s_) {
        if (!edge_x) return L;
        f32x4v v;
        v[0] = s_ == 0 ? L[0] : (s_ == 1 ? L[1] : (s_ == 2 ? L[2] : L[3]));
        v[1] = s_ == 0 ? L[1] : (s_ == 1 ? L[2] : (s_ == 2 ? L[3] : 0.f));
        v[2] = s_ == 0 ? L[2] : (s_ == 1 ? L[3] : 0.f);
        v[3] = s_ == 0 ? L[3] : 0.f;
        return v;
    };
    auto fetch = [&](int64_t mj) {
        load_tile(x, mj, stage);
        if constexpr (AG) load_tile(ref, mj, rv);
    };
    if ((int64_t)tid3.pg < p.major) fetch(tid3.pg);

    for (int64_t mj = tid3.pg; mj < p.major; mj += p.zgroups) {
        __syncthreads();
        if constexpr (AG) {
            float own = 0.f;
            const bool last_y = tid3.by == p.tiles_y - 1, last_x = tid3.bx == p.tiles_x - 1;
#pragma unroll
            for (int r = 0; r < NLD; ++r) {
                const int e = threadIdx.x + 256 * r;
                const int ry = e / BNQ, q = e - ry * BNQ;
                stage[r] = place(stage[r], sh[r]);
                const f32x4v rr = place(rv[r], sh[r]);
#pragma unroll
                for (int j = 0; j < 4; ++j) {
                    stage[r][j] *= rr[j] > 0.f ? p.scale : p.alpha * p.scale;
                    const int rx = 4 * q + j - D;
                    if (sh[r] >= 0 && (ry < BOH || last_y) && rx >= 0 && (rx < BOW || last_x)) own += stage[r][j];
                }
            }
#pragma unroll
            for (int o = 32; o > 0; o >>= 1) own += __shfl_down(own, o, 64);
            if ((threadIdx.x & 63) == 0) sred[threadIdx.x >> 6] = own;
        }
#pragma unroll
        for (int r = 0; r < NLD; ++r)
            if (sh[r] >= 0) *reinterpret_cast<f32x4v*>(&sx[lds_off[r]]) = AG ? stage[r] : place(stage[r], sh[r]);
        __syncthreads();
        if (mj + p.zgroups < p.major) fetch(mj + p.zgroups);
        if constexpr (AG) {
            if (threadIdx.x == 0)
                partial[(size_t)mj * (p.tiles_x * p.tiles_y) + tid3.by * p.tiles_x + tid3.bx] =
                    (sred[0] + sred[1]) + (sred[2] + sred[3]);
        }
        constexpr int NH = EXT ? 3 : 2, NQ = EXT ? 5 : 4;
        const bool xcol = EXT && p.ext_x && tid3.bx == p.tiles_x - 1 && tx == BOW - 4;
        const bool xrow = EXT && p.ext_y && tid3.by == p.tiles_y - 1 && ty == 15;
        float rf[MODE == 2 ? NH : 1][MODE == 2 ? NQ : 1];
        if constexpr (MODE == 2) {
            const float* rp = ref + (size_t)mj * p.out_h * p.out_w;
#pragma unroll
            for (int h = 0; h < NH; ++h) {
                const int oy = oy0 + 2 * ty + h;
                const bool rowok = oy < p.out_h && !(h == 2 && !xrow);
                const float* rrow = rp + (size_t)(rowok ? oy : 0) * p.out_w;
                if (rowok && ox0 + tx + 3 < p.out_w) {
                    typedef float f32x4u __attribute__((ext_vector_type(4), aligned(4)));
                    const f32x4u v = *reinterpret_cast<const f32x4u*>(rrow + ox0 + tx);
                    rf[h][0] = v[0]; rf[h][1] = v[1]; rf[h][2] = v[2]; rf[h][3] = v[3];
                } else {
#pragma unroll
                    for (int q = 0; q < 4; ++q) rf[h][q] = (rowok && ox0 + tx + q < p.out_w) ? rrow[ox0 + tx + q] : 0.f;
                }
                if (EXT) rf[h][NQ - 1] = (rowok && xcol) ? rrow[ox0 + tx + 4] : 0.f;
            }
        }
        float res[NH][NQ];
#pragma unroll
        for (int h = 0; h < NH; ++h)
#pragma unroll
            for (int q = 0; q < NQ; ++q) res[h][q] = 0.f;
        const bool ecol = EXT && p.ext_x && tid3.bx == p.tiles_x - 1;
        const bool erow = EXT && p.ext_y && tid3.by == p.tiles_y - 1;
#pragma unroll
        for (int a = 0; a < 5; ++a) {
            const float* row = &sx[(2 * ty + a) * BST + tx];
            const f32x4v w0 = *reinterpret_cast<const f32x4v*>(row);
            const f32x4v w1 = *reinterpret_cast<const f32x4v*>(row + 4);
            const f32x4v w2 = *reinterpret_cast<const f32x4v*>(row + 8);
            const float w[12] = {w0[0], w0[1], w0[2], w0[3], w1[0], w1[1], w1[2], w1[3], w2[0], w2[1], w2[2], w2[3]};
#pragma unroll
            for (int h = 0; h < 2; ++h) {
                const int ka = a - h;
                if (ka < 0 || ka > 3) continue;
#pragma unroll
                for (int q = 0; q < 4; ++q)
#pragma unroll
                    for (int c = 0; c < 4; ++c) res[h][q] += w[D + q + c] * kf[ka][c];
                if (EXT && ecol) {
#pragma unroll
                    for (int c = 0; c < 4; ++c) res[h][NQ - 1] += w[D + 4 + c] * kf[ka][c];
                }
            }
        }
        if (EXT && erow) {
#pragma unroll
            for (int a = 2; a < 6; ++a) {
                const float* row = &sx[(2 * ty + a) * BST + tx];
                const f32x4v w0 = *reinterpret_cast<const f32x4v*>(row);
                const f32x4v w1 = *reinterpret_cast<const f32x4v*>(row + 4);
                const f32x4v w2 = *reinterpret_cast<const f32x4v*>(row + 8);
                const float w[12] = {w0[0], w0[1], w0[2], w0[3], w1[0], w1[1], w1[2], w1[3], w2[0], w2[1], w2[2], w2[3]};
#pragma unroll
                for (int q = 0; q < NQ; ++q)
#pragma unroll
                    for (int c = 0; c < 4; ++c) res[NH - 1][q] += w[D + q + c] * kf[a - 2][c];
            }
        }
        const int ch = b ? (int)(mj % p.size_b) : 0;
        float own2 = 0.f;
        if constexpr (MODE == 2) {
#pragma unroll
            for (int h = 0; h < NH; ++h)
#pragma unroll
                for (int q = 0; q < NQ; ++q) res[h][q] *= rf[h][q] > 0.f ? p.scale : p.alpha * p.scale;
        }
#pragma unroll
        for (int h = 0; h < NH; ++h) {
            const int oy = oy0 + 2 * ty + h;
            if (oy >= p.out_h || (h == 2 && !xrow)) continue;
            float* orow = out + ((size_t)mj * p.out_h + oy) * p.out_w;
            if (ox0 + tx + 3 < p.out_w) {
                typedef float f32x4u __attribute__((ext_vector_type(4), aligned(4)));
                f32x4u v;
                v[0] = epilogue<MODE != 0>(res[h][0], b, ch, p); v[1] = epilogue<MODE != 0>(res[h][1], b, ch, p);
                v[2] = epilogue<MODE != 0>(res[h][2], b, ch, p); v[3] = epilogue<MODE != 0>(res[h][3], b, ch, p);
                *reinterpret_cast<f32x4u*>(orow + ox0 + tx) = v;
                if (MODE == 2) own2 += (v[0] + v[1]) + (v[2] + v[3]);
                if (EXT && xcol) {
                    orow[ox0 + tx + 4] = epilogue<MODE != 0>(res[h][NQ - 1], b, ch, p);
                    if (MODE == 2) own2 += res[h][NQ - 1];
                }
            } else {
#pragma unroll
                for (int q = 0; q < 4; ++q) {
                    const int ox = ox0 + tx + q;
                    if (ox < p.out_w) {
                        orow[ox] = epilogue<MODE != 0>(res[h][q], b, ch, p);
                        if (MODE == 2) own2 += res[h][q];
                    }
                }
            }
        }
        if constexpr (MODE == 2) {
#pragma unroll
            for (int o = 32; o > 0; o >>= 1) own2 += __shfl_down(own2, o, 64);
            if ((threadIdx.x & 63) == 0) sred[threadIdx.x >> 6] = own2;
            __syncthreads();
            if (threadIdx.x == 0)
                partial[(size_t)mj * (p.tiles_x * p.tiles_y) + tid3.by * p.tiles_x + tid3.bx] =
                    (sred[0] + sred[1]) + (sred[2] + sred[3]);
        }
    }
}

inline int blur44_tiles(int n, int t) { return (n > t && n % t == 1) ? n / t : (int)te::cdiv(n, t); }

inline unsigned blur44_grid(FirParams& q) {
    const int tx_n = blur44_tiles(q.out_w, BOW), ty_n = blur44_tiles(q.out_h, BOH);
    q.ext_x = tx_n * BOW < q.out_w;
    q.ext_y = ty_n * BOH < q.out_h;
    const int64_t tiles = (int64_t)tx_n * ty_n;
    return xcd_grid(q, tx_n, ty_n, fir_planes_z(q.major, 2 * tiles));
}

template <int AG>
void launch_blur44(float* out, const float* x, const float* k, const float* b, const FirParams& p, hipStream_t s, const float* ref,
                   float* partial) {
    FirParams q = p;
    dim3 grid(blur44_grid(q), 1u, 1u);
    auto go = [&](auto EXT) {
        switch ((-p.pad_x0) & 3) {
            case 0: blur44_kernel<AG, 0, decltype(EXT)::value><<<grid, 256, 0, s>>>(out, x, k, b, q, ref, partial); break;
            case 1: blur44_kernel<AG, 1, decltype(EXT)::value><<<grid, 256, 0, s>>>(out, x, k, b, q, ref, partial); break;
            case 2: blur44_kernel<AG, 2, decltype(EXT)::value><<<grid, 256, 0, s>>>(out, x, k, b, q, ref, partial); break;
            default: blur44_kernel<AG, 3, decltype(EXT)::value><<<grid, 256, 0, s>>>(out, x, k, b, q, ref, partial); break;
        }
    };
    if (q.ext_x || q.ext_y) go(std::true_type{});
    else go(std::false_type{});
}

enum FirRoute { FIR_DIRECT, FIR_BLUR44, FIR_TILE_UP2, FIR_TILE_DOWN2 };
inline FirRoute fir_route(const FirParams& p) {
    const bool sq = (p.up_x == p.up_y) && (p.down_x == p.down_y) && p.minor == 1;
    if (sq && p.kh == 4 && p.kw == 4 && p.up_x == 1 && p.down_x == 1 && p.in_w >= 4 && (int64_t)p.in_h * p.in_w * 4 < 0x7FFFFFFF) return FIR_BLUR44;
    if (sq && p.kh == 4 && p.kw == 4 && p.up_x == 2 && p.down_x == 1) return FIR_TILE_UP2;
    if (sq && p.kh == 4 && p.kw == 4 && p.up_x == 1 && p.down_x == 2) return FIR_TILE_DOWN2;
    return FIR_DIRECT;
}

inline FirParams fir_geometry(int64_t major, int in_h, int in_w, int minor, int kh, int kw, int up_x, int up_y, int down_x, int down_y,
                              int pad_x0, int pad_x1, int pad_y0, int pad_y1) {
    FirParams p{};
    p.in_h = in_h; p.in_w = in_w;
    p.out_h = (in_h * up_y + pad_y0 + pad_y1 - kh) / down_y + 1;
    p.out_w = (in_w * up_x + pad_x0 + pad_x1 - kw) / down_x + 1;
    p.pad_x0 = pad_x0; p.pad_y0 = pad_y0; p.kh = kh; p.kw = kw;
    p.up_x = up_x; p.up_y = up_y; p.down_x = down_x; p.down_y = down_y; p.minor = minor; p.major = major;
    return p;
}
inline bool actgrad_blur44(const FirParams& p) { return p.in_w >= 4; }
inline unsigned blur_bwd_grid(FirParams& q) { return actgrad_blur44(q) ? blur44_grid(q) : tile_grid(q); }

int fir_problem(const char* what, FirParams& p, int64_t major, int in_h, int in_w, int minor, int kh, int kw, int up_x, int up_y, int down_x,
                int down_y, int pad_x0, int pad_x1, int pad_y0, int pad_y1, bool has_bias = false, int64_t size_b = 1, int act = 0) {
    TE_REQUIRE(major >= 0 && in_h > 0 && in_w > 0 && minor > 0 && kh > 0 && kw > 0, TE_ERR_SHAPE, "%s: bad dims", what);
    TE_REQUIRE(up_x > 0 && up_y > 0 && down_x > 0 && down_y > 0, TE_ERR_SHAPE, "%s: up/down must be > 0", what);
    TE_REQUIRE(act == 0 || act == 3, TE_ERR_UNSUPPORTED, "%s: act must be 0 or 3", what);
    TE_REQUIRE(!(has_bias || act) || minor == 1, TE_ERR_UNSUPPORTED, "%s: fused epilogue needs minor == 1", what);
    TE_REQUIRE(!has_bias || size_b > 0, TE_ERR_SHAPE, "%s: bias given but size_b <= 0", what);
    p = fir_geometry(major, in_h, in_w, minor, kh, kw, up_x, up_y, down_x, down_y, pad_x0, pad_x1, pad_y0, pad_y1);
    TE_REQUIRE(p.out_h > 0 && p.out_w > 0, TE_ERR_SHAPE, "%s: empty output (%d x %d)", what, p.out_h, p.out_w);
    return 0;
}

int blur_bwd_problem(const char* what, FirParams& p, int64_t major, int in_h, int in_w, int kh, int kw, int pad_x0, int pad_x1, int pad_y0,
                     int pad_y1, int min_w, bool nonneg_pads) {
    TE_REQUIRE(major >= 0 && in_h > 0 && in_w >= min_w, TE_ERR_SHAPE, "%s: bad dims (in_w >= %d)", what, min_w);
    TE_REQUIRE(kh == 4 && kw == 4, TE_ERR_UNSUPPORTED, "%s: 4x4 taps only", what);
    TE_REQUIRE(!nonneg_pads || (pad_x0 >= 0 && pad_x1 >= 0 && pad_y0 >= 0 && pad_y1 >= 0), TE_ERR_UNSUPPORTED,
               "%s: pads must be >= 0 (every input element has to be staged by some tile)", what);
    p = fir_geometry(major, in_h, in_w, 1, kh, kw, 1, 1, 1, 1, pad_x0, pad_x1, pad_y0, pad_y1);
    TE_REQUIRE(p.out_h > 0 && p.out_w > 0, TE_ERR_SHAPE, "%s: empty output", what);
    return 0;
}

template <int MODE>
int blur_bwd_launch(const char* what, float* gx, float* partial, const float* g, const float* ref, const float* k, int64_t major, int in_h,
                    int in_w, int kh, int kw, int pad_x0, int pad_x1, int pad_y0, int pad_y1, float alpha, float scale, hipStream_t s,
                    int min_w, bool nonneg_pads) {
    TE_REQUIRE(gx && partial && g && ref && k, TE_ERR_NULL, "%s: NULL pointer", what);
    FirParams p;
    if (const int rc = blur_bwd_problem(what, p, major, in_h, in_w, kh, kw, pad_x0, pad_x1, pad_y0, pad_y1, min_w, nonneg_pads)) return rc;
    p.size_b = 1; p.act = 0; p.alpha = alpha; p.scale = scale;
    if (major == 0) return 0;
    TE_REQUIRE(major <= 0x7FFFFFFF / 4, TE_ERR_SHAPE, "%s: too many planes", what);
    TE_REQUIRE((int64_t)in_h * in_w * 4 < 0x7FFFFFFF, TE_ERR_UNSUPPORTED, "%s: plane too large", what);
    if (MODE == 2 || actgrad_blur44(p)) {
        launch_blur44<MODE>(gx, g, k, nullptr, p, s, ref, partial);
    } else {
        dim3 grid(tile_grid(p), 1u, 1u);
        fir_tile_kernel<1, 1, 4, 4, true><<<grid, 256, 0, s>>>(gx, g, k, nullptr, p, ref, partial);
    }
    return te::launch_status(what);
}

inline int plan_out(const FirParams& q, bool walks, int* zgroups, int* tiles) {
    *zgroups = walks ? q.zgroups : 0;
    *tiles = walks ? q.tiles_x * q.tiles_y : 0;
    return 0;
}

}

extern "C" int te_blur_actgrad_tiles(int in_h, int in_w, int kh, int kw, int pad_x0, int pad_x1, int pad_y0, int pad_y1) {
    FirParams p = fir_geometry(1, in_h, in_w, 1, kh, kw, 1, 1, 1, 1, pad_x0, pad_x1, pad_y0, pad_y1);
    if (p.out_h <= 0 || p.out_w <= 0) return TE_ERR_SHAPE;
    blur_bwd_grid(p);
    return p.tiles_x * p.tiles_y;
}

extern "C" int te_blur_actgrad_f32(float* gx, float* partial, const float* g, const float* ref, const float* k, int64_t major,
                                   int in_h, int in_w, int kh, int kw, int pad_x0, int pad_x1, int pad_y0, int pad_y1,
                                   float alpha, float scale, te_stream_t stream_) {
    return blur_bwd_launch<1>("te_blur_actgrad_f32", gx, partial, g, ref, k, major, in_h, in_w, kh, kw, pad_x0, pad_x1, pad_y0, pad_y1, alpha,
                              scale, (hipStream_t)stream_, 1, true);
}

extern "C" int te_blur_gradact_f32(float* gx, float* partial, const float* g, const float* ref, const float* k, int64_t major,
                                   int in_h, int in_w, int kh, int kw, int pad_x0, int pad_x1, int pad_y0, int pad_y1,
                                   float alpha, float scale, te_stream_t stream_) {
    return blur_bwd_launch<2>("te_blur_gradact_f32", gx, partial, g, ref, k, major, in_h, in_w, kh, kw, pad_x0, pad_x1, pad_y0, pad_y1, alpha,
                              scale, (hipStream_t)stream_, 4, false);
}

namespace {
template <typename T, typename A>
__global__ __launch_bounds__(256) void fir_direct_any_kernel(T* __restrict__ out, const T* __restrict__ x, const T* __restrict__ k,
                                                             const FirParams p) {
    const int64_t total = p.major * p.out_h * p.out_w * p.minor;
    const int64_t stride = (int64_t)gridDim.x * blockDim.x;
    for (int64_t e = (int64_t)blockIdx.x * blockDim.x + threadIdx.x; e < total; e += stride) {
        int64_t r = e;
        const int mn = (int)(r % p.minor); r /= p.minor;
        const int ox = (int)(r % p.out_w); r /= p.out_w;
        const int oy = (int)(r % p.out_h);
        const int64_t mj = r / p.out_h;
        const int mid_x = ox * p.down_x + p.up_x - 1 - p.pad_x0, mid_y = oy * p.down_y + p.up_y - 1 - p.pad_y0;
        const int ix0 = fdiv(mid_x, p.up_x), iy0 = fdiv(mid_y, p.up_y);
        const int jx0 = (ix0 + 1) * p.up_x - mid_x - 1, jy0 = (iy0 + 1) * p.up_y - mid_y - 1;
        A acc = (A)0;
        for (int jy = jy0, iy = iy0; jy < p.kh; jy += p.up_y, ++iy) {
            if (iy < 0 || iy >= p.in_h) continue;
            for (int jx = jx0, ix = ix0; jx < p.kw; jx += p.up_x, ++ix) {
                if (ix < 0 || ix >= p.in_w) continue;
                acc += (A)x[(((size_t)mj * p.in_h + iy) * p.in_w + ix) * p.minor + mn] *
                       (A)k[(p.kh - 1 - jy) * p.kw + (p.kw - 1 - jx)];
            }
        }
        out[e] = (T)acc;
    }
}

template <typename T, typename A>
int upfirdn2d_any(T* out, const T* x, const T* k, int64_t major, int in_h, int in_w, int minor, int kh, int kw, int up_x, int up_y,
                  int down_x, int down_y, int pad_x0, int pad_x1, int pad_y0, int pad_y1, te_stream_t stream_, const char* what) {
    TE_REQUIRE(out && x && k, TE_ERR_NULL, "%s: out/x/k is NULL", what);
    FirParams p;
    if (const int rc = fir_problem(what, p, major, in_h, in_w, minor, kh, kw, up_x, up_y, down_x, down_y, pad_x0, pad_x1, pad_y0, pad_y1)) return rc;
    if (major == 0) return 0;
    const int64_t total = major * p.out_h * p.out_w * minor;
    const int grid = fir_direct_grid(total);
    fir_direct_any_kernel<T, A><<<grid, 256, 0, (hipStream_t)stream_>>>(out, x, k, p);
    return te::launch_status(what);
}
}

extern "C" int te_upfirdn2d_f16(void* out, const void* x, const void* k, int64_t major, int in_h, int in_w, int minor, int kh,
                                int kw, int up_x, int up_y, int down_x, int down_y, int pad_x0, int pad_x1, int pad_y0, int pad_y1,
                                te_stream_t stream) {
    return upfirdn2d_any<__half, float>((__half*)out, (const __half*)x, (const __half*)k, major, in_h, in_w, minor, kh, kw, up_x,
                                        up_y, down_x, down_y, pad_x0, pad_x1, pad_y0, pad_y1, stream, "te_upfirdn2d_f16");
}

extern "C" int te_upfirdn2d_f64(double* out, const double* x, const double* k, int64_t major, int in_h, int in_w, int minor,
                                int kh, int kw, int up_x, int up_y, int down_x, int down_y, int pad_x0, int pad_x1, int pad_y0,
                                int pad_y1, te_stream_t stream) {
    return upfirdn2d_any<double, double>(out, x, k, major, in_h, in_w, minor, kh, kw, up_x, up_y, down_x, down_y, pad_x0, pad_x1,
                                         pad_y0, pad_y1, stream, "te_upfirdn2d_f64");
}

extern "C" int te_upfirdn2d_f32(float* out, const float* x, const float* k, int64_t major, int in_h, int in_w, int minor,
                                int kh, int kw, int up_x, int up_y, int down_x, int down_y, int pad_x0, int pad_x1,
                                int pad_y0, int pad_y1, const float* b, int64_t size_b, int act, float alpha,
                                float scale, te_stream_t stream_) {
    TE_REQUIRE(out && x && k, TE_ERR_NULL, "te_upfirdn2d_f32: out/x/k is NULL");
    FirParams p;
    if (const int rc = fir_problem("te_upfirdn2d_f32", p, major, in_h, in_w, minor, kh, kw, up_x, up_y, down_x, down_y, pad_x0, pad_x1, pad_y0,
                                   pad_y1, b != nullptr, size_b, act))
        return rc;
    p.size_b = (int)size_b; p.act = act; p.alpha = alpha; p.scale = (b || act) ? scale : 1.f;
    if (major == 0) return 0;
    hipStream_t s = (hipStream_t)stream_;
    switch (fir_route(p)) {
        case FIR_BLUR44: launch_blur44<0>(out, x, k, b, p, s, nullptr, nullptr); break;
        case FIR_TILE_UP2: launch_tile<2, 1, 4, 4>(out, x, k, b, p, s); break;
        case FIR_TILE_DOWN2: launch_tile<1, 2, 4, 4>(out, x, k, b, p, s); break;
        default: {
            const int64_t total = major * p.out_h * p.out_w * minor;
            fir_direct_kernel<<<fir_direct_grid(total), 256, 0, s>>>(out, x, k, b, p);
        }
    }
    return te::launch_status("te_upfirdn2d_f32");
}

extern "C" int te_upfirdn2d_plan(int64_t major, int in_h, int in_w, int minor, int kh, int kw, int up_x, int up_y, int down_x, int down_y,
// ... 36 lines not shown
```

transeditor_amd/csrc/wino6.hip:

```cpp
#include "split6_common.h"
#include "wino6_schedule.h"
#ifdef W6P_PROF
#define TE_PROF
#endif
#include "te_prof.h"

namespace {

constexpr int WT = 512, KC = 16, TW = 32, NP = TW / 2, BM = 64, TH = 8;
constexpr int U_CHUNKS = 36 * 2 * 64;

struct Wino6Args {
    float* out; const float* in; const u32x4* U; const float* isc; const float* osc; const float* bias; const float* res;
    const float* mref; float mgain; int act;
    int B, K, M, H, W, ntiles, mblocks, tiles_x, tiles_y, nt8;
    int lists;
    int lgpw;
};

constexpr int PH = 4, PR = PH + 2;
constexpr int TP_PLANE = PR * 2 * NP * 4;
constexpr int TP_DWORDS = 12 * TP_PLANE;
constexpr int GT = WT / 2;
constexpr int P_IN = (PR * NP * 8) / GT;
static_assert(PR * NP * 8 == P_IN * GT, "items must divide over the group");

PROF_BUFFER(w6p, 2048 * 8 * 8)
constexpr int SLOT0 = 21;

template <bool ISC>
__global__ __launch_bounds__(WT, 2) void wino6p_kernel(const Wino6Args p) {
    extern __shared__ __attribute__((aligned(16))) unsigned char smem_raw[];
    u32x4* ul = reinterpret_cast<u32x4*>(smem_raw);
    const int tid = threadIdx.x, lane = tid & 63, l31 = lane & 31, half = lane >> 5;
    const int wid = __builtin_amdgcn_readfirstlane(tid >> 6);
    const int grp = wid >> 2, wq = wid & 3, wm = wq >> 1, wrl = wq & 1, gt = tid & (GT - 1);
    unsigned* tl = reinterpret_cast<unsigned*>(smem_raw + U_CHUNKS * 16) + grp * TP_DWORDS;
    const u32x4* tl4 = reinterpret_cast<const u32x4*>(tl);
    int tile, mb;
    if (!split6_tile(p.ntiles, p.nt8, p.mblocks, tile, mb)) return;
    const int pwm = (1 << p.lgpw) - 1;
    const int tx = tile % p.tiles_x, ty = (tile / p.tiles_x) % p.tiles_y, b = (tile / (p.tiles_x * p.tiles_y)) << (4 - p.lgpw);
    const int x0 = tx * TW, y0 = ty * TH, yh = y0 + PH * grp;
    const float* inb = p.in + (size_t)b * p.K * p.H * p.W;
    const float* iscb = ISC ? p.isc + (size_t)b * p.K : nullptr;
    const bool has_left = x0 == 0, has_right = x0 + TW >= p.W, has_rowout = (yh == 0) || (yh + PH == p.H);

    f32x16 acc[4];
#pragma unroll
    for (int c = 0; c < 4; ++c)
#pragma unroll
        for (int r = 0; r < 16; ++r) acc[c][r] = 0.f;

    unsigned g_off[P_IN];
    int l_off[P_IN], e_flag[P_IN];
#pragma unroll
    for (int i = 0; i < P_IN; ++i) {
        const int e = gt + GT * i;
        const int jj = e & 15, q = (e >> 4) & 7, row = e >> 7;
        const int gy = yh - 1 + row;
        const int sj = jj >> p.lgpw, jl = jj & pwm;
        const bool left = x0 == 0 && jl == 0, right = x0 + TW >= p.W && jl == pwm, rowout = gy < 0 || gy >= p.H;
        e_flag[i] = (left ? 1 : 0) | (right ? 2 : 0) | (rowout ? 4 : 0);
        const int gyc = gy < 0 ? 0 : (gy >= p.H ? p.H - 1 : gy);
        g_off[i] = (unsigned)(sj * p.K * p.H * p.W + (2 * q * p.H + gyc) * p.W + x0 + 2 * jl - 1 + (left ? 1 : 0) - (right ? 1 : 0));
        l_off[i] = ((row * 2 + (q >> 2)) * NP + jj) * 4 + (q & 3);
    }
    const unsigned q2 = 2u * ((gt >> 4) & 7) + (unsigned)(((gt & 15) >> p.lgpw) * p.K);
    const size_t plane = (size_t)p.H * p.W;
    const int MT = p.M >> 5;
    f32x4 rin[P_IN][2];
    f32x2 rsc = {1.f, 1.f};
    const int nstage = p.K / KC;
    auto fetch_scales = [&](int s) {
        if (ISC) rsc = *reinterpret_cast<const f32x2u*>(iscb + s * KC + q2);
    };
    auto fetch_item = [&](int i, int s) {
#pragma unroll
        for (int h2 = 0; h2 < 2; ++h2)
            rin[i][h2] = *reinterpret_cast<const f32x4u*>(inb + ((size_t)s * KC + h2) * plane + g_off[i]);
    };
    auto issue = [&](int s) {
        fetch_scales(s);
#pragma unroll
        for (int i = 0; i < P_IN; ++i) fetch_item(i, s);
    };
    auto issue_u = [&](int uh, int s) {
        const u32x4* us = p.U + (size_t)s * 36 * MT * 64;
#pragma unroll
        for (int r = 0; r < 9; ++r) {
            const int j = wq * 9 + r, piece = j / 12, rem = j % 12, kc = (rem >> 1) + 6 * uh, mt = rem & 1;
            const int pk = piece * 12 + kc;
            const u32x4* g = us + ((size_t)pk * MT + 2 * mb + mt) * 64 + (unsigned)lane;
            __builtin_amdgcn_global_load_lds((const __attribute__((address_space(1))) void*)g,
                                             (__attribute__((address_space(3))) void*)(ul + (pk * 2 + mt) * 64), 16, 0, 0);
        }
    };
    unsigned res[P_IN][4][3];
    float te = 0.f, to = 0.f, fe = 0.f, fo = 0.f;
    constexpr int N_SLOT = 3 + 4 * 4 * P_IN;
    auto arith = [&](int k) {
// ... 88 lines not shown
                            if (k == (P_IN + 16 * i + 12 < LASTQ ? P_IN + 16 * i + 12 : LASTQ)) fetch_item(i, fs2);
                    }
                    __builtin_amdgcn_sched_barrier(0);
                }
            }
            __builtin_amdgcn_s_setprio(0);
            PROF_ONLY({ asm volatile("s_nop 0" ::: "memory"); PROF_T(tc); pc[2] += tc; })
        } else {
            const int cs = (ph + 1) >> 1;
            const bool work = cs >= 1 && cs < nstage;
            if (grp == 1 && work) issue_u(1, cs);
            __builtin_amdgcn_sched_barrier(0);
            write_res();
            if (grp == 1 && work) split6_wait_vm();
            PROF_T(ta);
            split6_barrier();
            PROF_T(tb);
            if (grp == 0 && work) {
                issue_u(0, cs);
                split6_wait_vm();
            }
            PROF_T(tc);
            PROF_ACC(pc[3], t0, ta); PROF_ACC(pc[4], ta, tb); PROF_ACC(pc[5], tb, tc);
        }
        PROF_T(t8);
        if (!last) split6_barrier();
        PROF_T(t9);
        PROF_ACC(pc[6], t8, t9);
    }
    PROF_ONLY(if (lane == 0 && blockIdx.x < 2048) {
        unsigned long long* d = te_w6p_prof_buf + ((size_t)blockIdx.x * 8 + wid) * 8;
        _Pragma("unroll")
        for (int i = 0; i < 6; ++i) d[i] = pc[i];
        d[6] = pc[6] | ((__builtin_amdgcn_s_memrealtime() - rstart) << 40);
        d[7] = ((unsigned long long)nstage << 48) | ((__builtin_readcyclecounter() - pstart) & 0xFFFFFFFFFFFFull);
    })
    const int wr = grp * 2 + wrl;
    const int mbase = mb * BM + wm * 32;
    const int bo = b + (jj >> p.lgpw);
    const size_t off0 = ((size_t)bo * p.M + mbase) * plane + (size_t)(y0 + 2 * wr + rr) * p.W + x0 + 2 * (jj & pwm);
    const float g_pos = p.act == 3 ? 1.4142135623730951f : 1.f;
    float scv[16], biv[16];
#pragma unroll
    for (int r = 0; r < 16; ++r) {
        const int m = mbase + (r & 3) + 8 * (r >> 2) + 4 * half;
        scv[r] = p.osc ? p.osc[(size_t)bo * p.M + m] : 1.f;
        biv[r] = p.bias ? p.bias[m] : 0.f;
    }
    f32x2 resv[16], mrefv[16];
    if (p.res) {
#pragma unroll
        for (int r = 0; r < 16; ++r)
            resv[r] = *reinterpret_cast<const f32x2*>(p.res + off0 + (size_t)((r & 3) + 8 * (r >> 2) + 4 * half) * plane);
    }
    if (p.mref) {
#pragma unroll
        for (int r = 0; r < 16; ++r)
            mrefv[r] = *reinterpret_cast<const f32x2*>(p.mref + off0 + (size_t)((r & 3) + 8 * (r >> 2) + 4 * half) * plane);
    }
#pragma unroll
    for (int r = 0; r < 16; ++r) {
        const int dm = (r & 3) + 8 * (r >> 2) + 4 * half;
        float v0 = acc[0][r] + acc[1][r] + acc[2][r];
        float v1 = acc[1][r] - acc[2][r] - acc[3][r];
        const float sc = scv[r], bi = biv[r];
        v0 = v0 * sc + bi;
        v1 = v1 * sc + bi;
        if (p.act >= 3) {
            v0 = (v0 > 0.f ? v0 : v0 * 0.2f) * g_pos;
            v1 = (v1 > 0.f ? v1 : v1 * 0.2f) * g_pos;
        }
        const size_t o = off0 + (size_t)dm * plane;
        if (p.res) { v0 += resv[r][0]; v1 += resv[r][1]; }
        if (p.mref) {
            v0 *= mrefv[r][0] > 0.f ? p.mgain : 0.2f * p.mgain;
            v1 *= mrefv[r][1] > 0.f ? p.mgain : 0.2f * p.mgain;
        }
        f32x2 v; v[0] = v0; v[1] = v1;
        *reinterpret_cast<f32x2*>(p.out + o) = v;
    }
}


template <bool ISC>
__global__ __launch_bounds__(WT, 2) void wino6q_kernel(const Wino6Args p) {
    extern __shared__ __attribute__((aligned(16))) unsigned char smem_raw[];
    u32x4* ul = reinterpret_cast<u32x4*>(smem_raw);
    const int tid = threadIdx.x, lane = tid & 63, l31 = lane & 31, half = lane >> 5;
    const int wid = __builtin_amdgcn_readfirstlane(tid >> 6);
    const int grp = wid >> 2, wq = wid & 3, wm = wq >> 1, wrl = wq & 1, gt = tid & (GT - 1);
    unsigned* tl = reinterpret_cast<unsigned*>(smem_raw + U_CHUNKS * 16) + grp * TP_DWORDS;
    const u32x4* tl4 = reinterpret_cast<const u32x4*>(tl);
    int tile, tile_end, tile_step, mbq;
    if (!split6_tile_list(p.ntiles, p.nt8, p.mblocks, p.lists, tile, tile_end, tile_step, mbq)) return;
    const float* inb;
    const float* iscb = nullptr;
    bool has_left, has_right, has_rowout;

    f32x16 acc[2][4];
#pragma unroll
    for (int m = 0; m < 2; ++m)
#pragma unroll
        for (int c = 0; c < 4; ++c)
#pragma unroll
            for (int r = 0; r < 16; ++r) acc[m][c][r] = 0.f;

    unsigned g_off[P_IN];
    int l_off[P_IN], e_flag[P_IN];
    typedef const __attribute__((address_space(4))) Wino6Args* KArgs;
    auto kargs = [&]() {
        KArgs k = (KArgs)__builtin_amdgcn_kernarg_segment_ptr();
        asm volatile("" : "+s"(k));
        return k;
    };
    auto set_tile = [&](int t) {
        const KArgs a = kargs();
        const int aH = a->H, aW = a->W, atx = a->tiles_x, aty = a->tiles_y, aK = a->K;
        const int tx = t % atx, ty = (t / atx) % aty, b = t / (atx * aty);
        const int x0 = tx * TW, yh = ty * TH + PH * grp;
        inb = a->in + (size_t)b * aK * aH * aW;
        if (ISC) iscb = a->isc + (size_t)b * aK;
        has_left = x0 == 0; has_right = x0 + TW == aW; has_rowout = (yh == 0) || (yh + PH == aH);
        int gto = gt;
        asm volatile("" : "+v"(gto));
#pragma unroll
        for (int i = 0; i < P_IN; ++i) {
            const int e = gto + GT * i;
            const int jj = e & 15, q = (e >> 4) & 7, row = e >> 7;
            const int gy = yh - 1 + row;
            const bool left = x0 == 0 && jj == 0, right = x0 + TW == aW && jj == NP - 1, rowout = gy < 0 || gy >= aH;
            e_flag[i] = (left ? 1 : 0) | (right ? 2 : 0) | (rowout ? 4 : 0);
            const int gyc = gy < 0 ? 0 : (gy >= aH ? aH - 1 : gy);
            g_off[i] = (unsigned)((2 * q * aH + gyc) * aW + x0 + 2 * jj - 1 + (left ? 1 : 0) - (right ? 1 : 0));
        }
    };
    set_tile(tile);
#pragma unroll
    for (int i = 0; i < P_IN; ++i) {
        const int e = gt + GT * i;
        const int jj = e & 15, q = (e >> 4) & 7, row = e >> 7;
        l_off[i] = ((row * 2 + (q >> 2)) * NP + jj) * 4 + (q & 3);
    }
    const unsigned q2 = 2u * ((gt >> 4) & 7);
    const size_t plane = (size_t)p.H * p.W;
    const int MT = p.M >> 5;
    f32x4 rin[P_IN][2];
    f32x2 rsc = {1.f, 1.f};
    const int nstage = p.K / KC, nimg = 2 * nstage;
    auto fetch_scales = [&](int s) {
        if (ISC) rsc = *reinterpret_cast<const f32x2u*>(iscb + s * KC + q2);
    };
    auto fetch_item = [&](int i, int s) {
#pragma unroll
        for (int h2 = 0; h2 < 2; ++h2)
            rin[i][h2] = *reinterpret_cast<const f32x4u*>(inb + ((size_t)s * KC + h2) * plane + g_off[i]);
    };
    auto issue_u = [&](int uh, int j) {
        int wqo = wq;
        asm volatile("" : "+s"(wqo));
        const u32x4* us = p.U + ((size_t)(j >> 1) * 36 * MT + 2 * (2 * mbq + (j & 1))) * 64;
        const unsigned pstride = 12u * (unsigned)MT * 64u;
#pragma unroll
        for (int t = 0; t < 3; ++t) {
            const int rem = wqo * 3 + t, kc = (rem >> 1) + 6 * uh, mt = rem & 1;
            const u32x4* g0 = us + (unsigned)(kc * MT + mt) * 64u;
            u32x4* l0 = ul + (kc * 2 + mt) * 64;
#pragma unroll
            for (int piece = 0; piece < 3; ++piece) {
                const u32x4* g = g0 + piece * pstride + (unsigned)lane;
                __builtin_amdgcn_global_load_lds((const __attribute__((address_space(1))) void*)g,
                                                 (__attribute__((address_space(3))) void*)(l0 + piece * 24 * 64), 16, 0, 0);
            }
        }
    };
    unsigned res[P_IN][4][3];
    float te = 0.f, to = 0.f, fe = 0.f, fo = 0.f;
    constexpr int N_SLOT = 3 + 4 * 4 * P_IN;
    auto arith = [&](int k) {
        if (k < 0) {
        } else if (k < P_IN) {
#pragma unroll
            for (int h2 = 0; h2 < 2; ++h2) {
                f32x4 v = rin[k][h2];
                if (has_left) {
                    int f = e_flag[k];
                    asm volatile("" : "+v"(f) :: "memory");
                    if (f & 1) { v[3] = v[2]; v[2] = v[1]; v[1] = v[0]; v[0] = 0.f; }
                }
                if (has_right) {
                    int f = e_flag[k];
                    asm volatile("" : "+v"(f) :: "memory");
                    if (f & 2) { v[0] = v[1]; v[1] = v[2]; v[2] = v[3]; v[3] = 0.f; }
// ... 43 lines not shown
#pragma unroll
        for (int g = 0; g < 12; ++g) {
            const int slot = g & 1, c = g & 3;
            if (g == 5) split6_barrier();
            __builtin_amdgcn_sched_barrier(0);
#pragma unroll
            for (int q = 0; q < 6; ++q) {
                split6_product(q, av[slot], bv[slot], acc[MSET][c], acc[MSET][c]);
                if (g + 1 < 12 && q < 3) { rd1(g + 1, slot ^ 1, 2 * q); rd1(g + 1, slot ^ 1, 2 * q + 1); }
                const int k = g * 6 + q;
                if (MSET == 0) {
                    if (k == 5) fetch_scales(fs);
#pragma unroll
                    for (int i = 0; i < P_IN; ++i)
                        if (k == 6 + 12 * i) fetch_item(i, fs);
                } else {
                    arith(k - SLOT0);
                }
                __builtin_amdgcn_sched_barrier(0);
            }
        }
        __builtin_amdgcn_s_setprio(0);
        split6_barrier();
    };
    auto stage = [&](int ph, bool write, bool has_next) {
        const int cs = wino6_sched::renew_image(ph);
        const bool work = wino6_sched::renew_work(cs, nimg, has_next);
        const int ci = cs == nimg ? 0 : cs;
        if (grp == 1 && work) issue_u(1, ci);
        __builtin_amdgcn_sched_barrier(0);
        if (write) write_res();
        if (grp == 1 && work) split6_wait_vm();
        split6_barrier();
        if (grp == 0 && work) {
            issue_u(0, ci);
            split6_wait_vm();
        }
        split6_barrier();
    };

    fetch_scales(0);
#pragma unroll
    for (int i = 0; i < P_IN; ++i) fetch_item(i, 0);
    if (grp == 0) { issue_u(0, 0); issue_u(1, 0); }
#pragma unroll
    for (int k = 0; k < N_SLOT; ++k) arith(k);
    write_res();
    split6_wait_vm();
    split6_barrier();
    for (;;) {
        const bool has_next = tile + tile_step < tile_end;
        int ph = 0;
        if (wino6_sched::lead_phase(grp)) { stage(0, false, has_next); ph = 1; }
        for (int s = 0; s < nstage; ++s) {
            bool next_tile;
            const int fs = wino6_sched::fetch_stage(s, nstage, has_next, next_tile);
            if (next_tile) set_tile(tile + tile_step);
            multiply(std::integral_constant<int, 0>{}, fs);
            stage(ph + 1, false, has_next);
            multiply(std::integral_constant<int, 1>{}, fs);
            if (wino6_sched::runs_sb(grp, s, nstage, has_next)) stage(ph + 3, true, has_next);
            ph += 4;
        }
        for (int i = 0; i < wino6_sched::tail_barriers(grp, has_next); ++i) split6_barrier();

        const KArgs e = kargs();
        const int tx = tile % e->tiles_x, ty = (tile / e->tiles_x) % e->tiles_y, b = tile / (e->tiles_x * e->tiles_y);
        const int x0 = tx * TW, y0 = ty * TH;
        int elane = lane;
        asm volatile("" : "+v"(elane));
        const int ehalf = elane >> 5, err = (elane & 31) >> 4, ejj = elane & 15;
        const int wr = grp * 2 + wrl;
        const int eM = e->M, eW = e->W, eact = e->act;
        const size_t eplane = (size_t)e->H * eW;
        const float emgain = e->mgain;
        const float g_pos = eact == 3 ? 1.4142135623730951f : 1.f;
        float* const eout = e->out;
        const float* const eosc = e->osc; const float* const ebias = e->bias; const float* const eres = e->res; const float* const emref = e->mref;
#pragma unroll
        for (int m = 0; m < 2; ++m) {
            const int mbase = (2 * mbq + m) * BM + wm * 32;
            const size_t off0 = ((size_t)b * eM + mbase) * eplane + (size_t)(y0 + 2 * wr) * eW + x0;
            const unsigned lo = (unsigned)(err * eW + 2 * ejj) + 4u * (unsigned)ehalf * (unsigned)eplane;
#pragma unroll
            for (int r0 = 0; r0 < 16; r0 += 4) {
                float scv[4], biv[4];
#pragma unroll
                for (int r = r0; r < r0 + 4; ++r) {
                    const int mm = mbase + (r & 3) + 8 * (r >> 2) + 4 * ehalf;
                    scv[r - r0] = eosc ? eosc[(size_t)b * eM + mm] : 1.f;
                    biv[r - r0] = ebias ? ebias[mm] : 0.f;
                }
                f32x2 resv[4], mrefv[4];
                if (eres) {
#pragma unroll
                    for (int r = r0; r < r0 + 4; ++r)
                        resv[r - r0] = *reinterpret_cast<const f32x2*>(eres + off0 + (size_t)((r & 3) + 8 * (r >> 2)) * eplane + lo);
                }
                if (emref) {
#pragma unroll
                    for (int r = r0; r < r0 + 4; ++r)
                        mrefv[r - r0] = *reinterpret_cast<const f32x2*>(emref + off0 + (size_t)((r & 3) + 8 * (r >> 2)) * eplane + lo);
                }
#pragma unroll
                for (int r = r0; r < r0 + 4; ++r) {
                    float v0 = acc[m][0][r] + acc[m][1][r] + acc[m][2][r];
                    float v1 = acc[m][1][r] - acc[m][2][r] - acc[m][3][r];
                    const float sc = scv[r - r0], bi = biv[r - r0];
                    v0 = v0 * sc + bi;
                    v1 = v1 * sc + bi;
                    if (eact >= 3) {
                        v0 = (v0 > 0.f ? v0 : v0 * 0.2f) * g_pos;
                        v1 = (v1 > 0.f ? v1 : v1 * 0.2f) * g_pos;
                    }
                    if (eres) { v0 += resv[r - r0][0]; v1 += resv[r - r0][1]; }
                    if (emref) {
                        v0 *= mrefv[r - r0][0] > 0.f ? emgain : 0.2f * emgain;
                        v1 *= mrefv[r - r0][1] > 0.f ? emgain : 0.2f * emgain;
                    }
                    f32x2 v; v[0] = v0; v[1] = v1;
                    *reinterpret_cast<f32x2*>(eout + off0 + (size_t)((r & 3) + 8 * (r >> 2)) * eplane + lo) = v;
                }
            }
        }
        if (!has_next) break;
        tile += tile_step;
#pragma unroll
        for (int m = 0; m < 2; ++m)
#pragma unroll
            for (int c = 0; c < 4; ++c)
#pragma unroll
                for (int r = 0; r < 16; ++r) acc[m][c][r] = 0.f;
    }
}

}

static std::atomic<int> g_w6_form{2};
extern "C" int te_conv_wino6_form(int form) {
    const int old = g_w6_form.load(std::memory_order_relaxed);
    if (form >= 1 && form <= 3) g_w6_form.store(form, std::memory_order_relaxed);
    return old;
}

constexpr int W6_MAX_TPB = 4096;
static std::atomic<int> g_w6_tpb{0};
extern "C" int te_conv_wino6_tiles_per_block(int n) {
    const int old = g_w6_tpb.load(std::memory_order_relaxed);
    if (n >= 0 && n <= W6_MAX_TPB) g_w6_tpb.store(n, std::memory_order_relaxed);
    return old;
}

static int w6_auto_tpb(int nt8c, int mblocks) {
    const int64_t rounds1 = te::cdiv((int64_t)8 * nt8c * mblocks, te::kNumCU);
    for (int n = 4; n >= 2; --n) {
        const int64_t blocks = (int64_t)8 * te::cdiv(nt8c, n) * mblocks;
        if (blocks >= te::kNumCU && te::cdiv(blocks, te::kNumCU) * n <= rounds1) return n;
    }
    return 1;
}

PROF_READBACK(w6p)

extern "C" int te_conv_wino6_supported(int B, int K, int M, int H, int W) {
    if (!(B > 0 && K >= 32 && K % 32 == 0 && M >= BM && M % BM == 0 && H >= TH && H % TH == 0)) return 0;
    const bool wide = W >= TW && W % TW == 0, pair16 = W == 16 && B % 2 == 0;
    if (!wide && !pair16) return 0;
    const int64_t tiles = wide ? (int64_t)B * (H / TH) * (W / TW) : (int64_t)(B / 2) * (H / TH);
    if (!wide && tiles * (M / BM) < te::kNumCU / 2) return 0;
    return ((int64_t)K * H * W * 4 * (wide ? 1 : 2) < 0x7FFFFFFF && tiles * (M / BM) < 0x7FFFFFF0) ? 1 : 0;
}

int te_wino6_launch(float* out, const float* in, const float* U, const float* isc, const float* osc, const float* bias, const float* res,
                    const float* mask_ref, float mask_gain, int act, int B, int K, int M, int H, int W, hipStream_t s) {
    TE_REQUIRE(te_conv_wino6_supported(B, K, M, H, W), TE_ERR_UNSUPPORTED,
               "te_conv_f32(TE_CONV_3X3W6): needs K %% 32 == 0, M %% 64 == 0, W %% 32 == 0 (or W == 16 and an even batch), H %% 8 == 0 (te_conv_wino6_supported)");
    TE_REQUIRE(((reinterpret_cast<uintptr_t>(out) | reinterpret_cast<uintptr_t>(U) | reinterpret_cast<uintptr_t>(res) |
                 reinterpret_cast<uintptr_t>(mask_ref)) & 15) == 0 && (reinterpret_cast<uintptr_t>(in) & 3) == 0, TE_ERR_UNSUPPORTED,
               "te_conv_f32(TE_CONV_3X3W6): 16-byte aligned tensors required");
    Wino6Args a{};
    a.out = out; a.in = in; a.U = reinterpret_cast<const u32x4*>(U); a.isc = isc; a.osc = osc; a.bias = bias; a.res = res;
    a.mref = mask_ref; a.mgain = mask_gain; a.act = act;
    a.B = B; a.K = K; a.M = M; a.H = H; a.W = W;
    a.lgpw = W >= TW ? 4 : 3;
    a.tiles_x = W >= TW ? W / TW : 1; a.tiles_y = H / TH; a.mblocks = M / BM;
    a.ntiles = (W >= TW ? B : B / 2) * a.tiles_x * a.tiles_y;
    a.nt8 = te::xcd_banded() ? (int)te::cdiv(a.ntiles, 8) : 0;
    const int64_t blocks = te::cdiv(a.ntiles, 8) * 8 * a.mblocks;
    const int form = g_w6_form.load(std::memory_order_relaxed);
    const int64_t blocks_q = te::cdiv(a.ntiles, 8) * 8 * (M / (2 * BM));
    if (W >= TW && split6_two_image(form - 1, M, blocks_q)) {
        a.mblocks = M / (2 * BM);
        const int nt8c = (int)te::cdiv(a.ntiles, 8);
        int tpb = g_w6_tpb.load(std::memory_order_relaxed);
        if (tpb == 0) tpb = w6_auto_tpb(nt8c, a.mblocks);
        a.lists = tpb >= 2 ? (int)te::cdiv(nt8c, tpb) : 0;
        const int64_t blocks2 = a.lists ? (int64_t)8 * a.lists * a.mblocks : blocks_q;
        const size_t lds = (size_t)U_CHUNKS * 16 + 2 * (size_t)TP_DWORDS * 4;
        SPLIT6_LAUNCH_ISC(wino6q_kernel, isc, dim3((unsigned)blocks2), WT, lds, s, a);
    } else {
        const size_t lds = (size_t)U_CHUNKS * 16 + 2 * (size_t)TP_DWORDS * 4;
        SPLIT6_LAUNCH_ISC(wino6p_kernel, isc, dim3((unsigned)blocks), WT, lds, s, a);
    }
    return te::launch_status("te_conv_f32(TE_CONV_3X3W6)");
}
```

transeditor_amd/op/modconv.py:

```python
import contextlib

import os

import torch
from torch.autograd import Function

from .. import _lib
from .chanscale import chan_scale
from .fused_act import fused_leaky_relu

import threading


class _Graph:
    __slots__ = ('skip_w',)

    def __init__(self):
        self.skip_w = False


_DEFAULT_GRAPH = _Graph()


class _Local(threading.local):
# ... 184 lines not shown

def _act_gain(act):
    return _SQRT2 if act is True else float(act)


def _act_code(act):
    if not act:
        return 0
    g = _act_gain(act)
    if abs(g - _SQRT2) < 1e-6:
        return 3
    if abs(g - 1.0) < 1e-6:
        return 4
    raise RuntimeError(f'modconv: leaky-ReLU gain {g} is not one the kernels fuse (sqrt(2) or 1)')


def _lowres_hw(kind, is_output, t):
    H, W = t.shape[2], t.shape[3]
    if (kind == 'up' and is_output) or (kind == 'down' and not is_output):
        if H % 2 == 0 or W % 2 == 0:
            raise RuntimeError(f"kind '{kind}': high-resolution side must be (2H+1)x(2W+1), got {H}x{W}")
        return (H - 1) // 2, (W - 1) // 2
    return H, W


USE_WINOGRAD = True
USE_SPLIT_BF16 = os.environ.get('TE_SPLIT_BF16', '1') != '0'
USE_SPLIT_S2 = os.environ.get('TE_SPLIT_S2', '1') != '0'
USE_SPLIT_T2 = os.environ.get('TE_SPLIT_T2', '1') != '0'
USE_SPLIT_1X1 = os.environ.get('TE_SPLIT_1X1', '1') != '0'

_ROUTES = {
    '3x3': (_lib.CONV_3X3, ((('USE_WINOGRAD', 'USE_SPLIT_BF16'), _lib.wino6_ok, _lib.CONV_3X3W6),
                            (('USE_WINOGRAD',), _lib.wino_ok, _lib.CONV_3X3W))),
    'down': (_lib.CONV_S2, ((('USE_SPLIT_BF16', 'USE_SPLIT_S2'), _lib.s2s6_ok, _lib.CONV_S2S6),)),
    'up': (_lib.CONV_T2, ((('USE_SPLIT_BF16', 'USE_SPLIT_T2'), _lib.t2s6_ok, _lib.CONV_T2S6),)),
    '1x1': (_lib.CONV_1X1, ()),
    'plain1x1': (_lib.CONV_1X1, ((('USE_SPLIT_BF16', 'USE_SPLIT_1X1'), _lib.p1s6_ok, _lib.CONV_1X1S6),)),
}
_ADJOINT = {'3x3': '3x3', 'down': 'up', 'up': 'down', '1x1': '1x1', 'plain1x1': 'plain1x1'}
_PACK = {
    _lib.CONV_3X3: (_lib.PACK_FWD, _lib.PACK_DGRAD), _lib.CONV_1X1: (_lib.PACK_FWD, _lib.PACK_DGRAD),
    _lib.CONV_T2: (_lib.PACK_FWD, _lib.PACK_SWAP), _lib.CONV_S2: (_lib.PACK_FWD, _lib.PACK_SWAP),
    _lib.CONV_3X3W: (_lib.PACK_WFWD, _lib.PACK_WDGRAD), _lib.CONV_3X3W6: (_lib.PACK_W6FWD, _lib.PACK_W6DGRAD),
    _lib.CONV_S2S6: (_lib.PACK_S6FWD, _lib.PACK_S6SWAP), _lib.CONV_T2S6: (_lib.PACK_T6FWD, _lib.PACK_T6SWAP),
    _lib.CONV_1X1S6: (_lib.PACK_P6FWD, _lib.PACK_P6DGRAD),
}


def conv_route(op, B, K, M, H, W, dgrad=False):
    if dgrad:
        op, K, M = _ADJOINT[op], M, K
    ck, preferred = _ROUTES[op]
    switch = globals().__getitem__
    for names, covers, kind in preferred:
        if all(map(switch, names)) and covers(B, K, M, H, W):
            ck = kind
            break
    return _PACK[ck][bool(dgrad)], ck


def fwd_kinds(kind, B, w, H, W):
    return conv_route(kind, B, w.shape[1], w.shape[0], H, W)


def bwd_kinds(kind, B, w, H, W):
    return conv_route(kind, B, w.shape[1], w.shape[0], H, W, dgrad=True)


def plain_1x1_kinds(B, w, H, W, dgrad=False):
    return conv_route('plain1x1', B, w.shape[1], w.shape[0], H, W, dgrad)


def packed_route(op, B, w, H, W, wscale, both):
    K, M = w.shape[1], w.shape[0]
    pk, ck = conv_route(op, B, K, M, H, W)
    if not both:
        return packed(w, pk, wscale), ck, None
    pkb, ckb = conv_route(op, B, K, M, H, W, dgrad=True)
    wp, wpb = packed2(w, pk, pkb, wscale)
    return wp, ck, (wpb, ckb)


def _fwd_raw(x, w, kind, isc=None, osc=None, bias=None, act=0, wscale=1.0, with_bwd_pack=False):
    H, W = _lowres_hw(kind, False, x)
    ahead = _STATE.pack_cache is not None and torch.is_grad_enabled() is False
    wp, ck, bwd = packed_route(kind, x.shape[0], w, H, W, wscale, with_bwd_pack or ahead)
    y = _lib.conv(x, wp, ck, w.shape[0], H, W, isc, osc, bias, act)
    return (y, bwd) if with_bwd_pack else y


def _dgrad_raw(g, w, kind, isc=None, osc=None, wscale=1.0, wp=None):
    H, W = _lowres_hw(kind, True, g)
    if wp is None:
        pk, ck = bwd_kinds(kind, g.shape[0], w, H, W)
        wp = packed(w, pk, wscale)
    else:
        wp, ck = wp
    return _lib.conv(g, wp, ck, w.shape[1], H, W, isc, osc)


def _wgrad_raw(g, x, kind, group=False):
    if kind == 'down':
        H, W = g.shape[2], g.shape[3]
        return _lib.wgrad_slabs(x, g, _lib.CONV_T2, H, W, group)
    H, W = x.shape[2], x.shape[3]
    return _lib.wgrad_slabs(g, x, _ROUTES[kind][0], H, W, group)


def _slab_sum(slabs, kind):
    gw = slabs.sum(dim=(0, 1))
    return gw.transpose(0, 1) if kind == 'down' else gw


def _wgrad_plain(gy, x, kind, ksize, wscale):
    slabs = _wgrad_raw(gy, x, kind, group=True)
    Co, Ci = gy.shape[1], x.shape[1]
    if kind == 'down':
        gw = _slab_sum(slabs, kind)
        gw = gw * wscale if wscale != 1.0 else gw
    else:
        gw, _, _ = _lib.wgrad_reduce(slabs, slabs[0, 0], wscale, None, None, want_w=True)
    return gw.reshape(Co, Ci, ksize, ksize)


class _ConvFwd(Function):
    @staticmethod
    def forward(ctx, x, w, kind, wscale):
        ctx.save_for_backward(x, w)
        ctx.kind, ctx.wscale = kind, wscale
        ctx.graph = current_graph()
        keep_cache(ctx)
        return _fwd_raw(x, w, kind, wscale=wscale)

    @staticmethod
    def backward(ctx, gy):
        x, w = ctx.saved_tensors
        skip_w = ctx.graph.skip_w or _DEFAULT_GRAPH.skip_w
        with cache_of(ctx):
            gx = _ConvDgrad.apply(gy, w, ctx.kind, ctx.wscale) if ctx.needs_input_grad[0] else None
            gw = _ConvWgrad.apply(gy, x, ctx.kind, w.shape[2], ctx.wscale) if (ctx.needs_input_grad[1] and not skip_w) else None
        return gx, gw, None, None


class _ConvDgrad(Function):
    @staticmethod
    def forward(ctx, gy, w, kind, wscale):
        ctx.save_for_backward(gy, w)
        ctx.kind, ctx.wscale = kind, wscale
        keep_cache(ctx)
        return _dgrad_raw(gy, w, kind, wscale=wscale)

    @staticmethod
    def backward(ctx, ggx):
        gy, w = ctx.saved_tensors
        with cache_of(ctx):
            g_gy = _ConvFwd.apply(ggx, w, ctx.kind, ctx.wscale) if ctx.needs_input_grad[0] else None
            g_w = _ConvWgrad.apply(gy, ggx, ctx.kind, w.shape[2], ctx.wscale) if ctx.needs_input_grad[1] else None
        return g_gy, g_w, None, None


class _ConvWgrad(Function):
    @staticmethod
    def forward(ctx, gy, x, kind, ksize, wscale):
        ctx.save_for_backward(gy, x)
        ctx.kind, ctx.wscale = kind, wscale
        keep_cache(ctx)
        return _wgrad_plain(gy, x, kind, ksize, wscale)

    @staticmethod
# ... 283 lines not shown
```

transeditor_amd/op/resblock.py:

```python
import math

import torch
from torch.autograd import Function

from .. import _lib
from .modconv import _act_code, _composite, _dgrad_raw, _wgrad_plain, cache_of, keep_cache, packed_route
from .upfirdn2d import _geometry, flipped_taps, upfirdn2d

_SQRT2 = math.sqrt(2.0)


def resblock_composite(x, w1, b1, w2, b2, ws, k_main, k_skip, s1, s2, ss, pad_main, pad_skip, gain, w0=None, b0=None, s0=1.0):
    if w0 is not None:
        x = _composite(x, w0, None, None, b0, True, '1x1', s0)
    y1 = _composite(x, w1, None, None, b1, True, '3x3', s1)
    yb = upfirdn2d(y1, k_main, pad=pad_main)
    y2 = _composite(yb, w2, None, None, b2, _SQRT2 * gain, 'down', s2)
    xs = upfirdn2d(x, k_skip, down=2, pad=pad_skip)
    return y2 + _composite(xs, ws, None, None, None, False, '1x1', ss * gain)


class _ResBlock(Function):
    @staticmethod
    def forward(ctx, x, w1, b1, w2, b2, ws, k_main, k_skip, s1, s2, ss, pad_main, pad_skip, gain, w0, b0, s0):
        x = x.contiguous()
        need = ctx.needs_input_grad
        keep_cache(ctx)
        ctx.stem = w0 is not None
        img = None
        need_x = need[0]
        if ctx.stem:
            img = x
            x = _lib.rgb_expand(img, w0.reshape(w0.shape[0], 3).t(), b0, 3, s0)
            need_x = need[0] or need[14] or need[15]
        front = need_x or need[1] or need[2]
        H, W = x.shape[2], x.shape[3]
        wp1, ck1, bwd1 = packed_route('3x3', x.shape[0], w1, H, W, s1, need_x)
        y1 = _lib.conv(x, wp1, ck1, w1.shape[0], H, W, None, None, b1, 3)
        pm = (pad_main[0], pad_main[1], pad_main[0], pad_main[1])
        yb = _lib.upfirdn2d_raw(y1, k_main, (1, 1), (1, 1), pm)
        if yb.shape[2] % 2 == 0 or yb.shape[3] % 2 == 0:
            raise RuntimeError(f'resblock: blurred size {tuple(yb.shape[2:])} is not (2h+1)x(2w+1)')
        h, w_ = (yb.shape[2] - 1) // 2, (yb.shape[3] - 1) // 2
        wp2, ck2, bwd2 = packed_route('down', x.shape[0], w2, h, w_, s2, front)
        y2 = _lib.conv(yb, wp2, ck2, w2.shape[0], h, w_, None, None, b2, _act_code(_SQRT2 * gain))
        ps = (pad_skip[0], pad_skip[1], pad_skip[0], pad_skip[1])
        xs = _lib.upfirdn2d_raw(x, k_skip, (1, 1), (2, 2), ps)
        if xs.shape[2:] != y2.shape[2:]:
            raise RuntimeError(f'resblock: branch sizes differ {tuple(xs.shape[2:])} vs {tuple(y2.shape[2:])}')
        wps, cks, bwds = packed_route('plain1x1', x.shape[0], ws, xs.shape[2], xs.shape[3], ss * gain, need_x)
        out = _lib.conv(xs, wps, cks, ws.shape[0], xs.shape[2], xs.shape[3], None, None, None, 0, res=y2)
        ctx.save_for_backward(x, w1, b1, w2, b2, ws, k_main, k_skip, y1, yb, y2, xs, img, w0, b0)
        ctx.packs = (bwd1, bwd2, bwds)
        ctx.cfg = (s1, s2, ss, tuple(pad_main), tuple(pad_skip), gain, pm, ps, s0, need_x)
        return out

    @staticmethod
    def backward(ctx, g):
        with cache_of(ctx):
            return _ResBlock._backward(ctx, g)

    @staticmethod
    def _backward(ctx, g):
        x, w1, b1, w2, b2, ws, k_main, k_skip, y1, yb, y2, xs, img, w0, b0 = ctx.saved_tensors
        s1, s2, ss, pad_main, pad_skip, gain, pm, ps, s0, need_x = ctx.cfg
        need = ctx.needs_input_grad
        if torch.is_grad_enabled():
            with torch.enable_grad():
                src = (img if ctx.stem else x, w1, b1, w2, b2, ws)
                al = [t.view_as(t) for t in src]
                st = [w0.view_as(w0), b0.view_as(b0)] if ctx.stem else [None, None]
                y = resblock_composite(*al, k_main, k_skip, s1, s2, ss, pad_main, pad_skip, gain, st[0], st[1], s0)
                flags = list(need[:6]) + ([need[14], need[15]] if ctx.stem else [])
                ins = [t for t, n in zip(al + (st if ctx.stem else []), flags) if n]
                gs = iter(torch.autograd.grad(y, ins, g, create_graph=True, allow_unused=True))
            first = tuple(next(gs) if n else None for n in need[:6])
            tail = (next(gs) if need[14] else None, next(gs) if need[15] else None) if ctx.stem else (None, None)
            return first + (None,) * 8 + tail + (None,)
        bwd1, bwd2, bwds = ctx.packs
        g = g.contiguous()
        front = need_x or need[1] or need[2]
        gx = gw1 = gb1 = gw2 = gb2 = gws = None
        g2, gb2 = _lib.bias_act_bwd(g, y2, 0.2, _SQRT2 * gain, want_bias=need[4])
        if need[3]:
            gw2 = _wgrad_plain(g2, yb, 'down', 3, s2)
        g1 = None
        if front:
            g_yb = _dgrad_raw(g2, w2, 'down', wscale=s2, wp=bwd2)
            _, g_pad = _geometry(y1.shape[2:], k_main.shape, (1, 1), (1, 1), pm)
            if tuple(k_main.shape) == (4, 4) and g_yb.shape[3] >= 4:
                g1, gb1 = _lib.blur_gradact(g_yb, y1, flipped_taps(k_main), g_pad, 0.2, _SQRT2)
            else:
                g1 = _lib.upfirdn2d_raw(g_yb, flipped_taps(k_main), (1, 1), (1, 1), g_pad)
                g1, gb1 = _lib.bias_act_bwd(g1, y1, 0.2, _SQRT2, want_bias=need[2])
            if not need[2]:
                gb1 = None
            if need[1]:
                gw1 = _wgrad_plain(g1, x, '3x3', 3, s1)
        if need[5]:
            gws = _wgrad_plain(g, xs, '1x1', 1, ss * gain)
        gw0 = gb0 = None
        if need_x:
            (wpsb, cksb), (wp1b, ck1b) = bwds, bwd1
            g_xs = _lib.conv(g, wpsb, cksb, ws.shape[1], xs.shape[2], xs.shape[3])
            _, gp_s = _geometry(x.shape[2:], k_skip.shape, (1, 1), (2, 2), ps)
            gx_b = _lib.upfirdn2d_raw(g_xs, flipped_taps(k_skip), (2, 2), (1, 1), gp_s)
            gx = _lib.conv(g1, wp1b, ck1b, w1.shape[1], x.shape[2], x.shape[3], None, None, None, 0, res=gx_b,
                           mask_ref=x if ctx.stem else None, mask_gain=_SQRT2)
        if ctx.stem:
            gpre, gx = gx, None
            M = w0.shape[0]
            if need[14] or need[15]:
                sl = _lib.rgb_wgrad_sum_slabs(img, gpre).sum(dim=(0, 1))
                if need[14]:
                    gw0 = sl[:3].t().reshape(w0.shape)
                    gw0 = gw0 * s0 if s0 != 1.0 else gw0
                if need[15]:
                    gb0 = sl[3].contiguous()
            if need[0]:
                gx = _lib.rgb_fwd(gpre, w0.reshape(M, 3).t().contiguous(), None, None, s0)
        return (gx, gw1, gb1, gw2, gb2, gws) + (None,) * 8 + (gw0, gb0, None)


def resblock(x, w1, b1, w2, b2, ws, k_main, k_skip, s1, s2, ss, pad_main, pad_skip, gain, stem=None):
    w0, b0, s0 = stem if stem is not None else (None, None, 1.0)
    x = x.contiguous()
    return _ResBlock.apply(x, w1, b1, w2, b2, ws, k_main, k_skip, float(s1), float(s2), float(ss), tuple(pad_main),
                           tuple(pad_skip), float(gain), w0, b0, float(s0))
```

transeditor_amd/op/styled_rgb.py:

```python
import torch
from torch.autograd import Function

from .. import _lib
from .modconv import _DEFAULT_GRAPH, _composite, _dgrad_raw, _fwd_raw, _wgrad_raw, cache_of, keep_cache

_SQRT2 = 2 ** 0.5


def supported(x, w, wr):
    HW = x.shape[2] * x.shape[3]
    return (x.is_cuda and x.dtype == torch.float32 and w.shape[2] == 3 and wr.shape[0] == 3 and wr.shape[1] == w.shape[0]
            and x.shape[0] <= 64 and w.shape[1] <= 8192 and _lib.rgb_supported(3, w.shape[0], HW))


class _ModConvRGB(Function):
    @staticmethod
    def forward(ctx, x, w, s, bias, wr, sr, br, wscale, eps, wscale_r):
        w3 = w.reshape(w.shape[0], w.shape[1], -1)
        d, wsq = _lib.demod_fwd(w3, s, wscale, eps)
        keep_cache(ctx)
        if ctx.needs_input_grad[0]:
            a, wp_bwd = _fwd_raw(x, w, '3x3', s, d, bias, 3, wscale, with_bwd_pack=True)
        else:
            a, wp_bwd = _fwd_raw(x, w, '3x3', s, d, bias, 3, wscale), None
        rgb = _lib.rgb_fwd(a, wr.reshape(3, wr.shape[1]), sr, br, wscale_r)
        ctx.save_for_backward(x, w, s, bias, wr, sr, br, d, wsq, a)
        ctx.wp_bwd = wp_bwd
        ctx.cfg = (wscale, eps, wscale_r)
        ctx.set_materialize_grads(False)
        return a, rgb

    @staticmethod
    def backward(ctx, ga, grgb):
        with cache_of(ctx):
            return _ModConvRGB._backward(ctx, ga, grgb)

    @staticmethod
    def _backward(ctx, ga, grgb):
        x, w, s, bias, wr, sr, br, d, wsq, a = ctx.saved_tensors
        wscale, eps, wscale_r = ctx.cfg
        need = ctx.needs_input_grad
        if torch.is_grad_enabled():
            with torch.enable_grad():
                from .style import demod as _demod
                al = [t.view_as(t) for t in (x, w, s, bias, wr, sr, br)]
                ac = _composite(al[0], al[1], al[2], _demod(al[1], al[2], wscale, eps), al[3], True, '3x3', wscale)
                rc = _composite(ac, al[4], al[5], None, al[6], False, '1x1', wscale_r)
                outs, gouts = [], []
                if ga is not None:
                    outs.append(ac)
                    gouts.append(ga)
                if grgb is not None:
                    outs.append(rc)
                    gouts.append(grgb)
                nd = list(need[:7])
                if _DEFAULT_GRAPH.skip_w:
                    nd[1] = nd[4] = False
                ins = [t for t, n in zip(al, nd) if n]
                gs = iter(torch.autograd.grad(outs, ins, gouts, create_graph=True, allow_unused=True))
            return tuple(next(gs) if n else None for n in nd) + (None, None, None)
        Co = w.shape[0]
        gwr = gsr = gbr = None
        if grgb is not None:
            grgb = grgb.contiguous()
            if need[6]:
                gbr = grgb.sum(dim=(0, 2, 3))
            if need[4] or need[5]:
                sl = _lib.rgb_wgrad_slabs(grgb, a)
                gwr, gsr, _ = _lib.wgrad_reduce(sl, wr.reshape(3, Co, 1), wscale_r, sr, None, want_w=need[4], want_isc=need[5])
                if gwr is not None:
                    gwr = gwr.reshape(wr.shape)
        if ga is None and grgb is None:
            return (None,) * 10
        if grgb is not None and _lib.bias_act_bwd_rgb_supported(a.shape):
            g, gb = _lib.bias_act_bwd_rgb(ga, a, grgb, wr.reshape(3, Co), sr, wscale_r, 0.2, _SQRT2, want_bias=need[3])
        else:
            gt = ga
            if grgb is not None:
                gr = _lib.rgb_dgrad(grgb, wr.reshape(3, Co), sr, Co, wscale_r)
                gt = gr if gt is None else gt + gr
            g, gb = _lib.bias_act_bwd(gt, a, 0.2, _SQRT2, want_bias=need[3])
        gx = _dgrad_raw(g, w, '3x3', isc=d, osc=s, wscale=wscale, wp=ctx.wp_bwd) if need[0] else None
        gw = gs = None
        if need[1] or need[2]:
            slabs = _wgrad_raw(g, x, '3x3')
            w3 = w.reshape(Co, w.shape[1], -1)
            gw, gs, gd = _lib.wgrad_reduce(slabs, w3, wscale, s, d, want_w=need[1], want_isc=need[2], want_osc=True)
            _lib.demod_bwd(gd, d, w3, wsq, s, wscale, into=(gw, gs))
            if gw is not None:
                gw = gw.reshape(w.shape)
        return gx, gw, gs, gb, gwr, gsr, gbr, None, None, None


def styled_conv_rgb(x, w, s, bias, wr, sr, br, wscale, eps, wscale_r):
    return _ModConvRGB.apply(x, w, s.contiguous(), bias, wr, sr.contiguous(), br, float(wscale), float(eps), float(wscale_r))
```

Measured before the change: 148.2.

## Emit bit-packed activation sign masks in conv forward and use them in backward

The conv kernels (winograd 3x3 and stride-2 s6 forms) now optionally write a 1-bit-per-element leaky-ReLU sign mask alongside the activation output. Bias-act backward, the RGB-fused backward, and blur-gradact backward read this mask instead of the full f32 activation. In the resblock, the activations y1 and y2 are no longer saved for backward when a mask exists. The goal is to cut backward memory traffic and saved-activation footprint, at the cost of extra mask writes and bit handling in the forward epilogue.

Result: no change. 148.9 (median of 6 runs) (+0.5%).

```diff
diff --git a/include/te_hip.h b/include/te_hip.h
--- a/include/te_hip.h
+++ b/include/te_hip.h
@@ -37,6 +37,15 @@
 int te_bias_act_bwd_rgb_f32(float* gi, float* gb, float* ws, const float* g, const float* ref, const float* grgb, const float* wrgb,
                             const float* srgb, float wscale, float alpha, float scale, int64_t outer, int64_t C, int64_t inner,
                             te_stream_t stream);
+
+#define TE_MASK_ROW_WORDS(W) (((W) + 31) >> 5)
+int64_t te_act_mask_words(int64_t B, int64_t C, int64_t H, int64_t W);
+int te_bias_act_bwd_mask_supported(int64_t outer, int64_t C, int64_t H, int64_t W);
+int te_bias_act_bwd_mask_f32(float* gi, float* gb, float* ws, const float* g, const uint32_t* mask, float alpha, float scale,
+                             int64_t outer, int64_t C, int64_t H, int64_t W, te_stream_t stream);
+int te_bias_act_bwd_rgb_mask_f32(float* gi, float* gb, float* ws, const float* g, const uint32_t* mask, const float* grgb,
+                                 const float* wrgb, const float* srgb, float wscale, float alpha, float scale, int64_t outer,
+                                 int64_t C, int64_t H, int64_t W, te_stream_t stream);
 
 int te_upfirdn2d_f32(float* out, const float* x, const float* k, int64_t major, int in_h, int in_w,
                      int minor, int kh, int kw, int up_x, int up_y, int down_x, int down_y, int pad_x0,
@@ -107,6 +116,10 @@
 int te_conv_res_f32(float* out, float* ws, const float* in, const float* wp, const float* isc, const float* osc,
                     const float* bias, const float* res, const float* mask_ref, float mask_gain, int act, int kind, int B,
                     int K, int M, int H, int W, te_stream_t stream);
+int te_conv_mask_supported(int kind, int B, int K, int M, int H, int W);
+int te_conv_mask_f32(float* out, float* ws, const float* in, const float* wp, const float* isc, const float* osc,
+                     const float* bias, const float* res, const float* mask_ref, float mask_gain, uint32_t* act_mask, int act,
+                     int kind, int B, int K, int M, int H, int W, te_stream_t stream);
 
 int te_wgrad_slab_count(int kind, int B, int Co, int Ci, int H, int W);
 int te_wgrad_pair_form(int kind, int Co, int Ci, int H, int W);
@@ -150,6 +163,9 @@
 int te_blur_gradact_f32(float* gx, float* partial, const float* g, const float* ref, const float* k, int64_t major, int in_h,
                         int in_w, int kh, int kw, int pad_x0, int pad_x1, int pad_y0, int pad_y1, float alpha, float scale,
                         te_stream_t stream);
+int te_blur_gradact_mask_f32(float* gx, float* partial, const float* g, const uint32_t* mask, const float* k, int64_t major, int in_h,
+                             int in_w, int kh, int kw, int pad_x0, int pad_x1, int pad_y0, int pad_y1, float alpha, float scale,
+                             te_stream_t stream);
 
 int te_upfirdn2d_plan(int64_t major, int in_h, int in_w, int minor, int kh, int kw, int up_x, int up_y, int down_x, int down_y,
                       int pad_x0, int pad_x1, int pad_y0, int pad_y1, int* zgroups, int* tiles);
diff --git a/transeditor_amd/_lib.py b/transeditor_amd/_lib.py
--- a/transeditor_amd/_lib.py
+++ b/transeditor_amd/_lib.py
@@ -175,6 +175,48 @@
     return gi, gb
 
 
+def act_mask_empty(shape, device):
+    n = lib().te_act_mask_words(*shape)
+    if n <= 0:
+        raise RuntimeError(f'te_act_mask_words failed ({n}) for {tuple(shape)}')
+    return torch.empty(n, device=device, dtype=torch.int32)
+
+
+def mask_describes(mask, out):
+    return mask if mask is not None and out._version == 0 else None
+
+
+def bias_act_bwd_mask_ok(shape):
+    return len(shape) == 4 and bool(lib().te_bias_act_bwd_mask_supported(*shape))
+
+
+def conv_mask_ok(kind, B, K, M, H, W):
+    return bool(lib().te_conv_mask_supported(kind, B, K, M, H, W))
+
+
+@_op
+def bias_act_bwd_mask(g, mask, alpha, scale, want_bias=True):
+    g = _aligned16(g.contiguous())
+    gi = torch.empty_like(g)
+    B, Cn, H, W = g.shape
+    gb, ws = _bias_grad_buffers(want_bias, B, Cn, H * W, g.device)
+    _launch('te_bias_act_bwd_mask_f32', _ptr(gi), _ptr(gb), _ptr(ws), _ptr(g), _ptr(mask, torch.int32), alpha, scale, B, Cn, H, W)
+    return gi, gb
+
+
+@_op
+def bias_act_bwd_rgb_mask(g, mask, grgb, wrgb, srgb, wscale, alpha, scale, want_bias=True):
+    grgb = _aligned16(grgb.contiguous())
+    g = _aligned16(g.contiguous()) if g is not None else None
+    B, _, H, W = grgb.shape
+    Cn = wrgb.shape[1]
+    gi = torch.empty(B, Cn, H, W, device=grgb.device, dtype=grgb.dtype)
+    gb, ws = _bias_grad_buffers(want_bias, B, Cn, H * W, grgb.device)
+    _launch('te_bias_act_bwd_rgb_mask_f32', _ptr(gi), _ptr(gb), _ptr(ws), _ptr(g), _ptr(mask, torch.int32), _ptr(grgb),
+            _ptr(wrgb.contiguous()), _ptr(srgb.contiguous()) if srgb is not None else None, wscale, alpha, scale, B, Cn, H, W)
+    return gi, gb
+
+
 @_op
 def upfirdn2d_raw(x, k, up, down, pad, bias=None, act=0, alpha=0.2, scale=1.0):
     x = x.contiguous()
@@ -235,6 +277,25 @@
 
 
 @_op
+def blur_gradact_mask(g, mask, k_flipped, pad, alpha, scale):
+    g = g.contiguous()
+    B, Cn, H, W = g.shape
+    kh, kw = k_flipped.shape
+    px0, px1, py0, py1 = pad
+    oh, ow = H + py0 + py1 - kh + 1, W + px0 + px1 - kw + 1
+    if mask.numel() != lib().te_act_mask_words(B, Cn, oh, ow):
+        raise RuntimeError(f'blur_gradact_mask: {mask.numel()} mask words do not describe the adjoint blur output {(B, Cn, oh, ow)}')
+    tiles = lib().te_blur_actgrad_tiles(H, W, kh, kw, px0, px1, py0, py1)
+    if tiles <= 0:
+        raise RuntimeError(f'te_blur_actgrad_tiles failed ({tiles})')
+    gx = torch.empty(B, Cn, oh, ow, device=g.device, dtype=g.dtype)
+    partial = torch.empty(B, Cn, tiles, device=g.device, dtype=g.dtype)
+    _launch('te_blur_gradact_mask_f32', _ptr(gx), _ptr(partial), _ptr(g), _ptr(mask, torch.int32), _ptr(k_flipped.contiguous()), B * Cn, H, W,
+            kh, kw, px0, px1, py0, py1, alpha, scale)
+    return gx, partial.sum(dim=(0, 2))
+
+
+@_op
 def conv_pack(w, kind_pack, wscale=1.0):
     w = w.contiguous()
     Co, Ci, ks, _ = w.shape
@@ -312,7 +373,7 @@
 
 
 @_op
-def conv(x, wp, kind, M, H, W, isc=None, osc=None, bias=None, act=0, res=None, mask_ref=None, mask_gain=1.0):
+def conv(x, wp, kind, M, H, W, isc=None, osc=None, bias=None, act=0, res=None, mask_ref=None, mask_gain=1.0, act_mask=None):
     x = x.contiguous()
     if kind == CONV_1X1S6:
         x = _aligned16(x)
@@ -330,6 +391,10 @@
     ws = torch.empty((S,) + tuple(out.shape), device=x.device, dtype=x.dtype) if S > 1 else None
     if kind == CONV_T2S6:
         ws = torch.empty(B * K * H, device=x.device, dtype=x.dtype)
+    if act_mask is not None:
+        _launch('te_conv_mask_f32', _ptr(out), _ptr(ws), _ptr(x), _ptr(wp), _ptr(isc), _ptr(osc), _ptr(bias), _ptr(res), _ptr(mask_ref),
+                mask_gain, _ptr(act_mask, torch.int32), act, kind, B, K, M, H, W)
+        return out
     _launch('te_conv_res_f32', _ptr(out), _ptr(ws), _ptr(x), _ptr(wp), _ptr(isc), _ptr(osc), _ptr(bias), _ptr(res), _ptr(mask_ref),
             mask_gain, act, kind, B, K, M, H, W)
     return out
diff --git a/transeditor_amd/csrc/act_mask.h b/transeditor_amd/csrc/act_mask.h
--- /dev/null
+++ b/transeditor_amd/csrc/act_mask.h
@@ -0,0 +1,36 @@
+#pragma once
+#include "te_common.h"
+
+namespace te {
+
+__host__ __device__ __forceinline__ int mask_row_words(int W) { return TE_MASK_ROW_WORDS(W); }
+
+__device__ __forceinline__ uint32_t mask_word(const uint32_t* __restrict__ row_words, int x) { return row_words[x >> 5]; }
+__device__ __forceinline__ bool mask_bit(uint32_t word, int x) { return (word >> (x & 31)) & 1u; }
+__device__ __forceinline__ float mask_slope(uint32_t word, int x, float pos, float neg) { return mask_bit(word, x) ? pos : neg; }
+
+__device__ __forceinline__ void mask_store_half(uint32_t* __restrict__ row_words, int x0, int W, uint32_t bits) {
+    if (x0 + 16 == W && !(x0 & 16)) row_words[x0 >> 5] = bits;
+    else reinterpret_cast<uint16_t*>(row_words)[x0 >> 4] = (uint16_t)bits;
+}
+
+template <int FB, int D>
+__device__ __forceinline__ uint32_t mask_transpose_step(uint32_t s, int jj) {
+    constexpr uint32_t ALL = FB == 2 ? 0xFFFFFFFFu : 0xFFFFu;
+    constexpr uint32_t UNIT = (1u << (FB * D)) - 1u;
+    constexpr uint32_t LOW = ALL / ((UNIT << (FB * D)) | UNIT) * UNIT;
+    const uint32_t q = (uint32_t)__builtin_amdgcn_ds_swizzle((int)s, 0x1F | (D << 10));
+    const bool upper = (jj & D) != 0;
+    const uint32_t keep = upper ? ALL & ~LOW : LOW;
+    const uint32_t moved = upper ? q >> (FB * D) : q << (FB * D);
+    return (s & keep) | (moved & (ALL & ~keep));
+}
+template <int FB>
+__device__ __forceinline__ uint32_t mask_transpose16(uint32_t s, int jj) {
+    s = mask_transpose_step<FB, 8>(s, jj);
+    s = mask_transpose_step<FB, 4>(s, jj);
+    s = mask_transpose_step<FB, 2>(s, jj);
+    return mask_transpose_step<FB, 1>(s, jj);
+}
+
+}
diff --git a/transeditor_amd/csrc/bias_act.hip b/transeditor_amd/csrc/bias_act.hip
--- a/transeditor_amd/csrc/bias_act.hip
+++ b/transeditor_amd/csrc/bias_act.hip
@@ -1,4 +1,5 @@
 #include "te_common.h"
+#include "act_mask.h"
 #include <hip/hip_fp16.h>
 
 namespace {
@@ -130,6 +131,70 @@
             o.w = gv.w * (rv.w > 0.f ? 1.f : alpha) * scale;
             gi[row + i] = o;
             acc += (o.x + o.y) + (o.z + o.w);
+        }
+    }
+    if (part) {
+        const float tot = block_sum_256(acc, lds4);
+        if (threadIdx.x == 0) part[((size_t)c * gridDim.z + n) * gridDim.x + blockIdx.x] = tot;
+    }
+}
+
+struct Pos4 { bool x, y, z, w; };
+__device__ __forceinline__ Pos4 mask_positive4(const uint32_t* __restrict__ mask, uint32_t plane, uint32_t i, uint32_t H, uint32_t W) {
+    const uint32_t e = 4u * i, y = e / W, x = e - y * W;
+    const uint32_t* mrow = mask + ((size_t)plane * H + y) * te::mask_row_words((int)W);
+    bool ps[4];
+    if ((W & 3u) == 0) {
+        const uint32_t w = te::mask_word(mrow, (int)x);
+#pragma unroll
+        for (int j = 0; j < 4; ++j) ps[j] = te::mask_bit(w, (int)x + j);
+    } else {
+#pragma unroll
+        for (int j = 0; j < 4; ++j) {
+            const bool wrap = x + j >= W;
+            const int xj = (int)(x + j - (wrap ? W : 0u));
+            ps[j] = te::mask_bit(te::mask_word(mrow + (wrap ? te::mask_row_words((int)W) : 0), xj), xj);
+        }
+    }
+    return Pos4{ps[0], ps[1], ps[2], ps[3]};
+}
+
+template <bool RGB>
+__global__ __launch_bounds__(256) void bias_act_bwd_rows_mask_kernel(float4* __restrict__ gi, float* __restrict__ part,
+                                                                     const float4* __restrict__ g, const uint32_t* __restrict__ mask,
+                                                                     const float4* __restrict__ grgb, const float* __restrict__ wrgb,
+                                                                     const float* __restrict__ srgb, float wscale, float alpha,
+                                                                     float scale, uint32_t C, uint32_t inner4, uint32_t H, uint32_t W) {
+#pragma clang fp contract(off)
+    __shared__ float lds4[4];
+    const uint32_t c = blockIdx.y, n = blockIdx.z;
+    const size_t row = ((size_t)n * C + c) * inner4;
+    const size_t rrow = (size_t)n * 3 * inner4;
+    float c0 = 0.f, c1 = 0.f, c2 = 0.f;
+    if constexpr (RGB) {
+        const float sc = (srgb ? srgb[(size_t)n * C + c] : 1.f) * wscale;
+        c0 = sc * wrgb[c]; c1 = sc * wrgb[C + c]; c2 = sc * wrgb[2 * C + c];
+    }
+    const uint32_t base = blockIdx.x * (256 * kBwdVecPerThread);
+    float acc = 0.f;
+#pragma unroll
+    for (int it = 0; it < kBwdVecPerThread; ++it) {
+        const uint32_t i = base + it * 256 + threadIdx.x;
+        if (i < inner4) {
+            const Pos4 ps = mask_positive4(mask, n * C + c, i, H, W);
+            float4 gv = (!RGB || g) ? g[row + i] : make_float4(0.f, 0.f, 0.f, 0.f);
+            if constexpr (RGB) {
+                const float4 r0 = grgb[rrow + i], r1 = grgb[rrow + inner4 + i], r2 = grgb[rrow + 2 * (size_t)inner4 + i];
+                gv.x += __builtin_fmaf(c2, r2.x, __builtin_fmaf(c0, r0.x, c1 * r1.x));
+                gv.y += __builtin_fmaf(c2, r2.y, __builtin_fmaf(c0, r0.y, c1 * r1.y));
+                gv.z += __builtin_fmaf(c2, r2.z, __builtin_fmaf(c0, r0.z, c1 * r1.z));
+                gv.w += __builtin_fmaf(c2, r2.w, __builtin_fmaf(c0, r0.w, c1 * r1.w));
+            }
+            const float px = gv.x * (ps.x ? 1.f : alpha), py = gv.y * (ps.y ? 1.f : alpha);
+            const float pz = gv.z * (ps.z ? 1.f : alpha), pw = gv.w * (ps.w ? 1.f : alpha);
+            const float4 o = make_float4(px * scale, py * scale, pz * scale, pw * scale);
+            gi[row + i] = o;
+            acc += __builtin_fmaf(scale, px, o.y) + __builtin_fmaf(scale, pz, o.w);
         }
     }
     if (part) {
@@ -316,3 +381,44 @@
     if (gb) bias_parts_sum_kernel<<<(int)C, 64, 0, stream>>>(gb, ws, (uint32_t)(grid.x * grid.z));
     return te::launch_status("te_bias_act_bwd_rgb_f32");
 }
+
+extern "C" int64_t te_act_mask_words(int64_t B, int64_t C, int64_t H, int64_t W) {
+    if (B <= 0 || C <= 0 || H <= 0 || W <= 0 || W > 0x7FFFFFE0) return TE_ERR_SHAPE;
+    return B * C * H * TE_MASK_ROW_WORDS(W);
+}
+
+extern "C" int te_bias_act_bwd_mask_supported(int64_t outer, int64_t C, int64_t H, int64_t W) {
+    return (outer > 0 && C > 0 && H > 0 && W >= 4 && H * W < 0x7FFFFFFF && bwd_rows_path(outer, C, H * W)) ? 1 : 0;
+}
+
+template <bool RGB>
+static int bias_act_bwd_mask_launch(const char* what, float* gi, float* gb, float* ws, const float* g, const uint32_t* mask, const float* grgb,
+                                    const float* wrgb, const float* srgb, float wscale, float alpha, float scale, int64_t outer, int64_t C,
+                                    int64_t H, int64_t W, te_stream_t stream_) {
+    TE_REQUIRE(gi && mask && (RGB ? grgb && wrgb : g != nullptr), TE_ERR_NULL, "%s: NULL pointer", what);
+    TE_REQUIRE(!gb || ws, TE_ERR_NULL, "%s: the bias gradient needs the workspace (te_bias_act_bwd_ws_floats)", what);
+    TE_REQUIRE(te_bias_act_bwd_mask_supported(outer, C, H, W), TE_ERR_UNSUPPORTED,
+               "%s: needs H W %% 4 == 0, H W >= 1024 and W >= 4 (te_bias_act_bwd_mask_supported)", what);
+    TE_REQUIRE(te::aligned16(gi) && (!g || te::aligned16(g)) && (!grgb || te::aligned16(grgb)) && ((uintptr_t)mask & 3) == 0, TE_ERR_UNSUPPORTED,
+               "%s: 16-byte aligned tensors required", what);
+    const uint32_t inner4 = (uint32_t)(H * W / 4);
+    dim3 grid((unsigned)te::cdiv(inner4, 256 * kBwdVecPerThread), (unsigned)C, (unsigned)outer);
+    hipStream_t stream = (hipStream_t)stream_;
+    bias_act_bwd_rows_mask_kernel<RGB><<<grid, 256, 0, stream>>>((float4*)gi, gb ? ws : nullptr, (const float4*)g, mask, (const float4*)grgb, wrgb,
+                                                                 srgb, wscale, alpha, scale, (uint32_t)C, inner4, (uint32_t)H, (uint32_t)W);
+    if (gb) bias_parts_sum_kernel<<<(int)C, 64, 0, stream>>>(gb, ws, (uint32_t)(grid.x * grid.z));
+    return te::launch_status(what);
+}
+
+extern "C" int te_bias_act_bwd_mask_f32(float* gi, float* gb, float* ws, const float* g, const uint32_t* mask, float alpha, float scale,
+                                        int64_t outer, int64_t C, int64_t H, int64_t W, te_stream_t stream) {
+    return bias_act_bwd_mask_launch<false>("te_bias_act_bwd_mask_f32", gi, gb, ws, g, mask, nullptr, nullptr, nullptr, 1.f, alpha, scale, outer, C,
+                                           H, W, stream);
+}
+
+extern "C" int te_bias_act_bwd_rgb_mask_f32(float* gi, float* gb, float* ws, const float* g, const uint32_t* mask, const float* grgb,
+                                            const float* wrgb, const float* srgb, float wscale, float alpha, float scale, int64_t outer,
+                                            int64_t C, int64_t H, int64_t W, te_stream_t stream) {
+    return bias_act_bwd_mask_launch<true>("te_bias_act_bwd_rgb_mask_f32", gi, gb, ws, g, mask, grgb, wrgb, srgb, wscale, alpha, scale, outer, C, H,
+                                          W, stream);
+}
diff --git a/transeditor_amd/csrc/conv.hip b/transeditor_amd/csrc/conv.hip
--- a/transeditor_amd/csrc/conv.hip
+++ b/transeditor_amd/csrc/conv.hip
@@ -1005,15 +1005,23 @@
     return conv_plan(kind, B, K, M, H, W).ksplit;
 }
 
-extern "C" int te_conv_res_f32(float* out, float* ws, const float* in, const float* wp, const float* isc, const float* osc,
-                               const float* bias, const float* res, const float* mask_ref, float mask_gain, int act, int kind,
-                               int B, int K, int M, int H, int W, te_stream_t stream_) {
+extern "C" int te_conv_mask_supported(int kind, int B, int K, int M, int H, int W) {
+    if (kind == TE_CONV_S2S6) return te_conv_s2s6_supported(B, K, M, H, W);
+    if (kind == TE_CONV_3X3W6) return te_wino6_emits_mask(B, K, M, H, W);
+    return 0;
+}
+
+static int conv_res_launch(float* out, float* ws, const float* in, const float* wp, const float* isc, const float* osc,
+                           const float* bias, const float* res, const float* mask_ref, float mask_gain, uint32_t* act_mask, int act,
+                           int kind, int B, int K, int M, int H, int W, te_stream_t stream_) {
     TE_REQUIRE(out && in && wp, TE_ERR_NULL, "te_conv_f32: out/in/wp is NULL");
     TE_REQUIRE(!(res || mask_ref) || (kind != TE_CONV_T2 && kind != TE_CONV_T2S6), TE_ERR_UNSUPPORTED,
                "te_conv_res_f32: no residual / mask epilogue for the transposed kind");
     TE_REQUIRE(B > 0 && K > 0 && M > 0 && H > 0 && W > 0, TE_ERR_SHAPE, "te_conv_f32: bad dims");
     TE_REQUIRE(act == 0 || act == 3 || act == 4, TE_ERR_UNSUPPORTED, "te_conv_f32: act must be 0, 3 or 4");
     TE_REQUIRE(kind >= 0 && kind < TE_CONV_KINDS, TE_ERR_UNSUPPORTED, "te_conv_f32: unknown kind %d", kind);
+    TE_REQUIRE(!act_mask || te_conv_mask_supported(kind, B, K, M, H, W), TE_ERR_UNSUPPORTED,
+               "te_conv_mask_f32: kind %d does not emit a sign mask at this shape (te_conv_mask_supported)", kind);
     hipStream_t s = (hipStream_t)stream_;
     if (kind == TE_CONV_1X1S6) {
         TE_REQUIRE(!isc && !osc && !bias && !mask_ref && act == 0, TE_ERR_UNSUPPORTED,
@@ -1021,8 +1029,8 @@
         return te_p1s6_launch(out, in, wp, res, B, K, M, H, W, s);
     }
     if (kind == TE_CONV_3X3W) return te_wino_launch(out, in, wp, isc, osc, bias, res, mask_ref, mask_gain, act, B, K, M, H, W, s);
-    if (kind == TE_CONV_3X3W6) return te_wino6_launch(out, in, wp, isc, osc, bias, res, mask_ref, mask_gain, act, B, K, M, H, W, s);
-    if (kind == TE_CONV_S2S6) return te_s2s6_launch(out, in, wp, isc, osc, bias, res, mask_ref, mask_gain, act, B, K, M, H, W, s);
+    if (kind == TE_CONV_3X3W6) return te_wino6_launch(out, in, wp, isc, osc, bias, res, mask_ref, mask_gain, act, B, K, M, H, W, s, act_mask);
+    if (kind == TE_CONV_S2S6) return te_s2s6_launch(out, in, wp, isc, osc, bias, res, mask_ref, mask_gain, act, B, K, M, H, W, s, act_mask);
     if (kind == TE_CONV_T2S6) {
         const int rc = te_t2s6_launch(out, in, wp, isc, osc, bias, act, B, K, M, H, W, s, ws);
         if (rc) return rc;
@@ -1059,6 +1067,18 @@
     return te::launch_status("te_conv_f32");
 }
 
+extern "C" int te_conv_res_f32(float* out, float* ws, const float* in, const float* wp, const float* isc, const float* osc,
+                               const float* bias, const float* res, const float* mask_ref, float mask_gain, int act, int kind,
+                               int B, int K, int M, int H, int W, te_stream_t stream_) {
+    return conv_res_launch(out, ws, in, wp, isc, osc, bias, res, mask_ref, mask_gain, nullptr, act, kind, B, K, M, H, W, stream_);
+}
+
+extern "C" int te_conv_mask_f32(float* out, float* ws, const float* in, const float* wp, const float* isc, const float* osc,
+                                const float* bias, const float* res, const float* mask_ref, float mask_gain, uint32_t* act_mask, int act,
+                                int kind, int B, int K, int M, int H, int W, te_stream_t stream_) {
+    return conv_res_launch(out, ws, in, wp, isc, osc, bias, res, mask_ref, mask_gain, act_mask, act, kind, B, K, M, H, W, stream_);
+}
+
 extern "C" int te_conv_ws_f32(float* out, float* ws, const float* in, const float* wp, const float* isc, const float* osc,
                               const float* bias, int act, int kind, int B, int K, int M, int H, int W, te_stream_t stream_) {
     return te_conv_res_f32(out, ws, in, wp, isc, osc, bias, nullptr, nullptr, 1.f, act, kind, B, K, M, H, W, stream_);
diff --git a/transeditor_amd/csrc/conv_common.h b/transeditor_amd/csrc/conv_common.h
--- a/transeditor_amd/csrc/conv_common.h
+++ b/transeditor_amd/csrc/conv_common.h
@@ -23,9 +23,12 @@
 int te_wino_launch(float* out, const float* in, const float* U, const float* isc, const float* osc, const float* bias, const float* res,
                    const float* mask_ref, float mask_gain, int act, int B, int K, int M, int H, int W, hipStream_t s);
 int te_wino6_launch(float* out, const float* in, const float* U, const float* isc, const float* osc, const float* bias, const float* res,
-                    const float* mask_ref, float mask_gain, int act, int B, int K, int M, int H, int W, hipStream_t s);
+                    const float* mask_ref, float mask_gain, int act, int B, int K, int M, int H, int W, hipStream_t s,
+                    uint32_t* act_mask = nullptr);
+int te_wino6_emits_mask(int B, int K, int M, int H, int W);
 int te_s2s6_launch(float* out, const float* in, const float* U, const float* isc, const float* osc, const float* bias, const float* res,
-                   const float* mask_ref, float mask_gain, int act, int B, int K, int M, int H, int W, hipStream_t s);
+                   const float* mask_ref, float mask_gain, int act, int B, int K, int M, int H, int W, hipStream_t s,
+                   uint32_t* act_mask = nullptr);
 int te_t2s6_launch(float* out, const float* in, const float* U, const float* isc, const float* osc, const float* bias, int act,
                    int B, int K, int M, int H, int W, hipStream_t s, float* colbuf = nullptr);
 int te_t2s6_edge_launch(float* out, const float* in, const float* wplain, const float* isc, const float* osc, const float* bias, int act,
diff --git a/transeditor_amd/csrc/s2s6.hip b/transeditor_amd/csrc/s2s6.hip
--- a/transeditor_amd/csrc/s2s6.hip
+++ b/transeditor_amd/csrc/s2s6.hip
@@ -1,4 +1,5 @@
 #include "split6_common.h"
+#include "act_mask.h"
 #ifdef S2_PROF
 #define TE_PROF
 #endif
@@ -28,10 +29,12 @@
     const float* mref; float mgain; int act;
     int B, K, M, H, W, Hi, Wi, ntiles, mblocks, tiles_x, tiles_y, nt8;
 };
-
-
-template <bool ISC, bool TWOIMG>
-__device__ __attribute__((optnone)) void s2s6_body(const S2Args& p) {
+struct S2ArgsM : S2Args { uint32_t* amask; };
+
+
+template <bool ISC, bool TWOIMG, class Args = S2Args>
+__device__ __attribute__((optnone)) void s2s6_body(const Args& p) {
+    constexpr bool EMIT = std::is_same<Args, S2ArgsM>::value;
     constexpr int NIMG = TWOIMG ? 2 : 1;
     extern __shared__ __attribute__((aligned(16))) unsigned char smem_raw[];
     u32x4* ul = reinterpret_cast<u32x4*>(smem_raw);
@@ -301,14 +304,21 @@
 #pragma unroll
             for (int r = 0; r < 16; ++r) mrefv[r] = p.mref[off0 + (size_t)((r & 3) + 8 * (r >> 2) + 4 * half) * oplane];
         }
+        [[maybe_unused]] uint32_t signs = 0;
 #pragma unroll
         for (int r = 0; r < 16; ++r) {
             const int dm = (r & 3) + 8 * (r >> 2) + 4 * half;
             float v = (acc[m][r] + accl[m][r]) * scv[r] + biv[r];
             if (p.act >= 3) v = (v > 0.f ? v : v * 0.2f) * g_pos;
+            if constexpr (EMIT) signs |= v > 0.f ? 1u << r : 0u;
             if (p.res) v += resv[r];
             if (p.mref) v *= mrefv[r] > 0.f ? p.mgain : 0.2f * p.mgain;
             p.out[off0 + (size_t)dm * oplane] = v;
+        }
+        if constexpr (EMIT) {
+            const int dmj = (jj & 3) + 8 * (jj >> 2) + 4 * half;
+            const size_t mrow = ((size_t)b * p.M + mbase + dmj) * p.H + (yh + 2 * wrl + rr);
+            te::mask_store_half(p.amask + mrow * te::mask_row_words(p.W), x0, p.W, te::mask_transpose16<1>(signs, jj));
         }
     }
 }
@@ -317,6 +327,10 @@
 __global__ __launch_bounds__(WT, 2) void s2s6_kernel(const S2Args p) { [[clang::always_inline]] s2s6_body<ISC, false>(p); }
 template <bool ISC>
 __global__ __launch_bounds__(WT, 2) void s2s6q_kernel(const S2Args p) { [[clang::always_inline]] s2s6_body<ISC, true>(p); }
+template <bool ISC>
+__global__ __launch_bounds__(WT, 2) void s2s6m_kernel(const S2ArgsM p) { [[clang::always_inline]] s2s6_body<ISC, false>(p); }
+template <bool ISC>
+__global__ __launch_bounds__(WT, 2) void s2s6qm_kernel(const S2ArgsM p) { [[clang::always_inline]] s2s6_body<ISC, true>(p); }
 
 }
 
@@ -335,7 +349,7 @@
 }
 
 int te_s2s6_launch(float* out, const float* in, const float* U, const float* isc, const float* osc, const float* bias, const float* res,
-                   const float* mask_ref, float mask_gain, int act, int B, int K, int M, int H, int W, hipStream_t s) {
+                   const float* mask_ref, float mask_gain, int act, int B, int K, int M, int H, int W, hipStream_t s, uint32_t* act_mask) {
     TE_REQUIRE(te_conv_s2s6_supported(B, K, M, H, W), TE_ERR_UNSUPPORTED,
                "te_conv_f32(TE_CONV_S2S6): needs K %% 16 == 0 (>= 32), M %% 64 == 0, H %% 8 == 0, W %% 16 == 0 (te_conv_s2s6_supported)");
     TE_REQUIRE((reinterpret_cast<uintptr_t>(U) & 15) == 0 && (reinterpret_cast<uintptr_t>(in) & 3) == 0, TE_ERR_UNSUPPORTED,
@@ -351,8 +365,15 @@
     const size_t lds = (size_t)U_SLOTS * 1024 + 2 * (size_t)TP_DWORDS * 4;
     const int form = g_s2_form.load(std::memory_order_relaxed);
     const int64_t blocks_q = te::cdiv(a.ntiles, 8) * 8 * (M / (2 * BM));
-    if (split6_two_image(form, M, blocks_q)) {
-        a.mblocks = M / (2 * BM);
+    const bool two = split6_two_image(form, M, blocks_q);
+    if (two) a.mblocks = M / (2 * BM);
+    if (act_mask) {
+        S2ArgsM am{};
+        static_cast<S2Args&>(am) = a;
+        am.amask = act_mask;
+        if (two) SPLIT6_LAUNCH_ISC(s2s6qm_kernel, isc, dim3((unsigned)blocks_q), WT, lds, s, am);
+        else SPLIT6_LAUNCH_ISC(s2s6m_kernel, isc, dim3((unsigned)blocks), WT, lds, s, am);
+    } else if (two) {
         SPLIT6_LAUNCH_ISC(s2s6q_kernel, isc, dim3((unsigned)blocks_q), WT, lds, s, a);
     } else {
         SPLIT6_LAUNCH_ISC(s2s6_kernel, isc, dim3((unsigned)blocks), WT, lds, s, a);
diff --git a/transeditor_amd/csrc/upfirdn2d.hip b/transeditor_amd/csrc/upfirdn2d.hip
--- a/transeditor_amd/csrc/upfirdn2d.hip
+++ b/transeditor_amd/csrc/upfirdn2d.hip
@@ -1,4 +1,5 @@
 #include "te_common.h"
+#include "act_mask.h"
 #include <hip/hip_fp16.h>
 
 namespace {
@@ -259,6 +260,7 @@
     constexpr int NIT = BIH * BNQ, NLD = (NIT + 255) / 256;
     f32x4v stage[NLD];
     constexpr bool AG = (MODE == 1);
+    constexpr bool GA = (MODE >= 2);
     f32x4v rv[AG ? NLD : 1];
     unsigned goff[NLD];
     int lds_off[NLD], sh[NLD];
@@ -351,6 +353,19 @@
                 if (EXT) rf[h][NQ - 1] = (rowok && xcol) ? rrow[ox0 + tx + 4] : 0.f;
             }
         }
+        [[maybe_unused]] uint32_t mw[MODE == 3 ? NH : 1], mx[MODE == 3 ? NH : 1];
+        if constexpr (MODE == 3) {
+            const int wpr = te::mask_row_words(p.out_w);
+            const uint32_t* mp = reinterpret_cast<const uint32_t*>(ref) + (size_t)mj * p.out_h * wpr;
+#pragma unroll
+            for (int h = 0; h < NH; ++h) {
+                const int oy = oy0 + 2 * ty + h;
+                const bool rowok = oy < p.out_h && !(h == 2 && !xrow);
+                const uint32_t* mrow = mp + (size_t)(rowok ? oy : 0) * wpr;
+                mw[h] = (rowok && ox0 + tx < p.out_w) ? te::mask_word(mrow, ox0 + tx) : 0u;
+                mx[h] = (EXT && rowok && xcol) ? te::mask_word(mrow, ox0 + tx + 4) : 0u;
+            }
+        }
         float res[NH][NQ];
 #pragma unroll
         for (int h = 0; h < NH; ++h)
@@ -400,6 +415,13 @@
             for (int h = 0; h < NH; ++h)
 #pragma unroll
                 for (int q = 0; q < NQ; ++q) res[h][q] *= rf[h][q] > 0.f ? p.scale : p.alpha * p.scale;
+        }
+        if constexpr (MODE == 3) {
+#pragma unroll
+            for (int h = 0; h < NH; ++h)
+#pragma unroll
+                for (int q = 0; q < NQ; ++q)
+                    res[h][q] *= te::mask_slope(q < 4 ? mw[h] : mx[h], ox0 + tx + q, p.scale, p.alpha * p.scale);
         }
 #pragma unroll
         for (int h = 0; h < NH; ++h) {
@@ -412,10 +434,10 @@
                 v[0] = epilogue<MODE != 0>(res[h][0], b, ch, p); v[1] = epilogue<MODE != 0>(res[h][1], b, ch, p);
                 v[2] = epilogue<MODE != 0>(res[h][2], b, ch, p); v[3] = epilogue<MODE != 0>(res[h][3], b, ch, p);
                 *reinterpret_cast<f32x4u*>(orow + ox0 + tx) = v;
-                if (MODE == 2) own2 += (v[0] + v[1]) + (v[2] + v[3]);
+                if (GA) own2 += (v[0] + v[1]) + (v[2] + v[3]);
                 if (EXT && xcol) {
                     orow[ox0 + tx + 4] = epilogue<MODE != 0>(res[h][NQ - 1], b, ch, p);
-                    if (MODE == 2) own2 += res[h][NQ - 1];
+                    if (GA) own2 += res[h][NQ - 1];
                 }
             } else {
 #pragma unroll
@@ -423,12 +445,12 @@
                     const int ox = ox0 + tx + q;
                     if (ox < p.out_w) {
                         orow[ox] = epilogue<MODE != 0>(res[h][q], b, ch, p);
-                        if (MODE == 2) own2 += res[h][q];
+                        if (GA) own2 += res[h][q];
                     }
                 }
             }
         }
-        if constexpr (MODE == 2) {
+        if constexpr (GA) {
 #pragma unroll
             for (int o = 32; o > 0; o >>= 1) own2 += __shfl_down(own2, o, 64);
             if ((threadIdx.x & 63) == 0) sred[threadIdx.x >> 6] = own2;
@@ -523,7 +545,7 @@
     if (major == 0) return 0;
     TE_REQUIRE(major <= 0x7FFFFFFF / 4, TE_ERR_SHAPE, "%s: too many planes", what);
     TE_REQUIRE((int64_t)in_h * in_w * 4 < 0x7FFFFFFF, TE_ERR_UNSUPPORTED, "%s: plane too large", what);
-    if (MODE == 2 || actgrad_blur44(p)) {
+    if (MODE >= 2 || actgrad_blur44(p)) {
         launch_blur44<MODE>(gx, g, k, nullptr, p, s, ref, partial);
     } else {
         dim3 grid(tile_grid(p), 1u, 1u);
@@ -559,6 +581,13 @@
                                    float alpha, float scale, te_stream_t stream_) {
     return blur_bwd_launch<2>("te_blur_gradact_f32", gx, partial, g, ref, k, major, in_h, in_w, kh, kw, pad_x0, pad_x1, pad_y0, pad_y1, alpha,
                               scale, (hipStream_t)stream_, 4, false);
+}
+
+extern "C" int te_blur_gradact_mask_f32(float* gx, float* partial, const float* g, const uint32_t* mask, const float* k, int64_t major,
+                                        int in_h, int in_w, int kh, int kw, int pad_x0, int pad_x1, int pad_y0, int pad_y1,
+                                        float alpha, float scale, te_stream_t stream_) {
+    return blur_bwd_launch<3>("te_blur_gradact_mask_f32", gx, partial, g, reinterpret_cast<const float*>(mask), k, major, in_h, in_w, kh, kw,
+                              pad_x0, pad_x1, pad_y0, pad_y1, alpha, scale, (hipStream_t)stream_, 4, false);
 }
 
 namespace {
diff --git a/transeditor_amd/csrc/wino6.hip b/transeditor_amd/csrc/wino6.hip
--- a/transeditor_amd/csrc/wino6.hip
+++ b/transeditor_amd/csrc/wino6.hip
@@ -1,5 +1,6 @@
 #include "split6_common.h"
 #include "wino6_schedule.h"
+#include "act_mask.h"
 #ifdef W6P_PROF
 #define TE_PROF
 #endif
@@ -17,6 +18,11 @@
     int lists;
     int lgpw;
 };
+struct Wino6ArgsM : Wino6Args { uint32_t* amask; };
+
+__device__ __forceinline__ uint32_t w6_sign_field(float v0, float v1, int r) {
+    return (v0 > 0.f ? 1u << (2 * r) : 0u) | (v1 > 0.f ? 2u << (2 * r) : 0u);
+}
 
 constexpr int PH = 4, PR = PH + 2;
 constexpr int TP_PLANE = PR * 2 * NP * 4;
@@ -271,8 +277,9 @@
 }
 
 
-template <bool ISC>
-__global__ __launch_bounds__(WT, 2) void wino6q_kernel(const Wino6Args p) {
+template <bool ISC, class Args = Wino6Args>
+__device__ __attribute__((optnone)) void wino6q_body(const Args& p) {
+    constexpr bool EMIT = std::is_same<Args, Wino6ArgsM>::value;
     extern __shared__ __attribute__((aligned(16))) unsigned char smem_raw[];
     u32x4* ul = reinterpret_cast<u32x4*>(smem_raw);
     const int tid = threadIdx.x, lane = tid & 63, l31 = lane & 31, half = lane >> 5;
@@ -296,7 +303,7 @@
 
     unsigned g_off[P_IN];
     int l_off[P_IN], e_flag[P_IN];
-    typedef const __attribute__((address_space(4))) Wino6Args* KArgs;
+    typedef const __attribute__((address_space(4))) Args* KArgs;
     auto kargs = [&]() {
         KArgs k = (KArgs)__builtin_amdgcn_kernarg_segment_ptr();
         asm volatile("" : "+s"(k));
@@ -506,6 +513,7 @@
             const int mbase = (2 * mbq + m) * BM + wm * 32;
             const size_t off0 = ((size_t)b * eM + mbase) * eplane + (size_t)(y0 + 2 * wr) * eW + x0;
             const unsigned lo = (unsigned)(err * eW + 2 * ejj) + 4u * (unsigned)ehalf * (unsigned)eplane;
+            [[maybe_unused]] uint32_t signs = 0;
 #pragma unroll
             for (int r0 = 0; r0 < 16; r0 += 4) {
                 float scv[4], biv[4];
@@ -532,11 +540,12 @@
                     float v1 = acc[m][1][r] - acc[m][2][r] - acc[m][3][r];
                     const float sc = scv[r - r0], bi = biv[r - r0];
                     v0 = v0 * sc + bi;
-                    v1 = v1 * sc + bi;
+                    v1 = sc * v1 + bi;
                     if (eact >= 3) {
                         v0 = (v0 > 0.f ? v0 : v0 * 0.2f) * g_pos;
                         v1 = (v1 > 0.f ? v1 : v1 * 0.2f) * g_pos;
                     }
+                    if constexpr (EMIT) signs |= w6_sign_field(v0, v1, r);
                     if (eres) { v0 += resv[r - r0][0]; v1 += resv[r - r0][1]; }
                     if (emref) {
                         v0 *= mrefv[r - r0][0] > 0.f ? emgain : 0.2f * emgain;
@@ -546,6 +555,12 @@
                     *reinterpret_cast<f32x2*>(eout + off0 + (size_t)((r & 3) + 8 * (r >> 2)) * eplane + lo) = v;
                 }
             }
+            if constexpr (EMIT) {
+                const int eH = e->H, wpr = te::mask_row_words(eW);
+                const size_t mbase0 = (((size_t)b * eM + mbase) * eH + (y0 + 2 * wr)) * wpr + (x0 >> 5);
+                const unsigned mlo = (unsigned)(((ejj & 3) + 8 * (ejj >> 2) + 4 * ehalf) * eH + err) * (unsigned)wpr;
+                e->amask[mbase0 + mlo] = te::mask_transpose16<2>(signs, ejj);
+            }
         }
         if (!has_next) break;
         tile += tile_step;
@@ -557,6 +572,11 @@
                 for (int r = 0; r < 16; ++r) acc[m][c][r] = 0.f;
     }
 }
+
+template <bool ISC>
+__global__ __launch_bounds__(WT, 2) void wino6q_kernel(const Wino6Args p) { [[clang::always_inline]] wino6q_body<ISC>(p); }
+template <bool ISC>
+__global__ __launch_bounds__(WT, 2) void wino6qm_kernel(const Wino6ArgsM p) { [[clang::always_inline]] wino6q_body<ISC>(p); }
 
 }
 
@@ -595,8 +615,15 @@
     return ((int64_t)K * H * W * 4 * (wide ? 1 : 2) < 0x7FFFFFFF && tiles * (M / BM) < 0x7FFFFFF0) ? 1 : 0;
 }
 
+static bool w6_two_image(int B, int M, int H, int W) {
+    if (W < TW) return false;
+    const int64_t ntiles = (int64_t)B * (W / TW) * (H / TH);
+    return split6_two_image(g_w6_form.load(std::memory_order_relaxed) - 1, M, te::cdiv(ntiles, 8) * 8 * (M / (2 * BM)));
+}
+int te_wino6_emits_mask(int B, int K, int M, int H, int W) { return te_conv_wino6_supported(B, K, M, H, W) && w6_two_image(B, M, H, W); }
+
 int te_wino6_launch(float* out, const float* in, const float* U, const float* isc, const float* osc, const float* bias, const float* res,
-                    const float* mask_ref, float mask_gain, int act, int B, int K, int M, int H, int W, hipStream_t s) {
+                    const float* mask_ref, float mask_gain, int act, int B, int K, int M, int H, int W, hipStream_t s, uint32_t* act_mask) {
     TE_REQUIRE(te_conv_wino6_supported(B, K, M, H, W), TE_ERR_UNSUPPORTED,
                "te_conv_f32(TE_CONV_3X3W6): needs K %% 32 == 0, M %% 64 == 0, W %% 32 == 0 (or W == 16 and an even batch), H %% 8 == 0 (te_conv_wino6_supported)");
     TE_REQUIRE(((reinterpret_cast<uintptr_t>(out) | reinterpret_cast<uintptr_t>(U) | reinterpret_cast<uintptr_t>(res) |
@@ -611,9 +638,8 @@
     a.ntiles = (W >= TW ? B : B / 2) * a.tiles_x * a.tiles_y;
     a.nt8 = te::xcd_banded() ? (int)te::cdiv(a.ntiles, 8) : 0;
     const int64_t blocks = te::cdiv(a.ntiles, 8) * 8 * a.mblocks;
-    const int form = g_w6_form.load(std::memory_order_relaxed);
     const int64_t blocks_q = te::cdiv(a.ntiles, 8) * 8 * (M / (2 * BM));
-    if (W >= TW && split6_two_image(form - 1, M, blocks_q)) {
+    if (w6_two_image(B, M, H, W)) {
         a.mblocks = M / (2 * BM);
         const int nt8c = (int)te::cdiv(a.ntiles, 8);
         int tpb = g_w6_tpb.load(std::memory_order_relaxed);
@@ -621,9 +647,17 @@
         a.lists = tpb >= 2 ? (int)te::cdiv(nt8c, tpb) : 0;
         const int64_t blocks2 = a.lists ? (int64_t)8 * a.lists * a.mblocks : blocks_q;
         const size_t lds = (size_t)U_CHUNKS * 16 + 2 * (size_t)TP_DWORDS * 4;
-        SPLIT6_LAUNCH_ISC(wino6q_kernel, isc, dim3((unsigned)blocks2), WT, lds, s, a);
+        if (act_mask) {
+            Wino6ArgsM am{};
+            static_cast<Wino6Args&>(am) = a;
+            am.amask = act_mask;
+            SPLIT6_LAUNCH_ISC(wino6qm_kernel, isc, dim3((unsigned)blocks2), WT, lds, s, am);
+        } else {
+            SPLIT6_LAUNCH_ISC(wino6q_kernel, isc, dim3((unsigned)blocks2), WT, lds, s, a);
+        }
     } else {
         const size_t lds = (size_t)U_CHUNKS * 16 + 2 * (size_t)TP_DWORDS * 4;
+        TE_REQUIRE(!act_mask, TE_ERR_UNSUPPORTED, "te_conv_mask_f32(TE_CONV_3X3W6): only the two-image form emits a sign mask (te_conv_mask_supported)");
         SPLIT6_LAUNCH_ISC(wino6p_kernel, isc, dim3((unsigned)blocks), WT, lds, s, a);
     }
     return te::launch_status("te_conv_f32(TE_CONV_3X3W6)");
diff --git a/transeditor_amd/op/modconv.py b/transeditor_amd/op/modconv.py
--- a/transeditor_amd/op/modconv.py
+++ b/transeditor_amd/op/modconv.py
@@ -290,10 +290,16 @@
     return wp, ck, (wpb, ckb)
 
 
-def _fwd_raw(x, w, kind, isc=None, osc=None, bias=None, act=0, wscale=1.0, with_bwd_pack=False):
+def _fwd_raw(x, w, kind, isc=None, osc=None, bias=None, act=0, wscale=1.0, with_bwd_pack=False, with_mask=False):
     H, W = _lowres_hw(kind, False, x)
     ahead = _STATE.pack_cache is not None and torch.is_grad_enabled() is False
     wp, ck, bwd = packed_route(kind, x.shape[0], w, H, W, wscale, with_bwd_pack or ahead)
+    if with_mask:
+        shape = _lib.conv_out_shape(ck, x.shape[0], w.shape[0], H, W)
+        ok = _lib.conv_mask_ok(ck, x.shape[0], x.shape[1], w.shape[0], H, W) and _lib.bias_act_bwd_mask_ok(shape)
+        mask = _lib.act_mask_empty(shape, x.device) if ok else None
+        y = _lib.conv(x, wp, ck, w.shape[0], H, W, isc, osc, bias, act, act_mask=mask)
+        return y, (bwd if with_bwd_pack else None), _lib.mask_describes(mask, y)
     y = _lib.conv(x, wp, ck, w.shape[0], H, W, isc, osc, bias, act)
     return (y, bwd) if with_bwd_pack else y
 
diff --git a/transeditor_amd/op/resblock.py b/transeditor_amd/op/resblock.py
--- a/transeditor_amd/op/resblock.py
+++ b/transeditor_amd/op/resblock.py
@@ -8,6 +8,8 @@
 from .upfirdn2d import _geometry, flipped_taps, upfirdn2d
 
 _SQRT2 = math.sqrt(2.0)
+
+USE_SIGN_MASKS = True
 
 
 def resblock_composite(x, w1, b1, w2, b2, ws, k_main, k_skip, s1, s2, ss, pad_main, pad_skip, gain, w0=None, b0=None, s0=1.0):
@@ -36,21 +38,32 @@
         front = need_x or need[1] or need[2]
         H, W = x.shape[2], x.shape[3]
         wp1, ck1, bwd1 = packed_route('3x3', x.shape[0], w1, H, W, s1, need_x)
-        y1 = _lib.conv(x, wp1, ck1, w1.shape[0], H, W, None, None, b1, 3)
+        m1 = None
+        if (USE_SIGN_MASKS and front and tuple(k_main.shape) == (4, 4) and _lib.conv_mask_ok(ck1, x.shape[0], x.shape[1], w1.shape[0], H, W)):
+            m1 = _lib.act_mask_empty((x.shape[0], w1.shape[0], H, W), x.device)
+        y1 = _lib.conv(x, wp1, ck1, w1.shape[0], H, W, None, None, b1, 3, act_mask=m1)
+        m1 = _lib.mask_describes(m1, y1)
         pm = (pad_main[0], pad_main[1], pad_main[0], pad_main[1])
         yb = _lib.upfirdn2d_raw(y1, k_main, (1, 1), (1, 1), pm)
         if yb.shape[2] % 2 == 0 or yb.shape[3] % 2 == 0:
             raise RuntimeError(f'resblock: blurred size {tuple(yb.shape[2:])} is not (2h+1)x(2w+1)')
         h, w_ = (yb.shape[2] - 1) // 2, (yb.shape[3] - 1) // 2
         wp2, ck2, bwd2 = packed_route('down', x.shape[0], w2, h, w_, s2, front)
-        y2 = _lib.conv(yb, wp2, ck2, w2.shape[0], h, w_, None, None, b2, _act_code(_SQRT2 * gain))
+        m2 = None
+        y2_shape = (x.shape[0], w2.shape[0], h, w_)
+        if (USE_SIGN_MASKS and any(need) and _lib.conv_mask_ok(ck2, x.shape[0], yb.shape[1], w2.shape[0], h, w_)
+                and _lib.bias_act_bwd_mask_ok(y2_shape)):
+            m2 = _lib.act_mask_empty(y2_shape, x.device)
+        y2 = _lib.conv(yb, wp2, ck2, w2.shape[0], h, w_, None, None, b2, _act_code(_SQRT2 * gain), act_mask=m2)
+        m2 = _lib.mask_describes(m2, y2)
         ps = (pad_skip[0], pad_skip[1], pad_skip[0], pad_skip[1])
         xs = _lib.upfirdn2d_raw(x, k_skip, (1, 1), (2, 2), ps)
         if xs.shape[2:] != y2.shape[2:]:
             raise RuntimeError(f'resblock: branch sizes differ {tuple(xs.shape[2:])} vs {tuple(y2.shape[2:])}')
         wps, cks, bwds = packed_route('plain1x1', x.shape[0], ws, xs.shape[2], xs.shape[3], ss * gain, need_x)
         out = _lib.conv(xs, wps, cks, ws.shape[0], xs.shape[2], xs.shape[3], None, None, None, 0, res=y2)
-        ctx.save_for_backward(x, w1, b1, w2, b2, ws, k_main, k_skip, y1, yb, y2, xs, img, w0, b0)
+        ctx.save_for_backward(x, w1, b1, w2, b2, ws, k_main, k_skip, y1 if m1 is None else None, yb, y2 if m2 is None else None, xs, img,
+                              w0, b0, m1, m2)
         ctx.packs = (bwd1, bwd2, bwds)
         ctx.cfg = (s1, s2, ss, tuple(pad_main), tuple(pad_skip), gain, pm, ps, s0, need_x)
         return out
@@ -62,7 +75,7 @@
 
     @staticmethod
     def _backward(ctx, g):
-        x, w1, b1, w2, b2, ws, k_main, k_skip, y1, yb, y2, xs, img, w0, b0 = ctx.saved_tensors
+        x, w1, b1, w2, b2, ws, k_main, k_skip, y1, yb, y2, xs, img, w0, b0, m1, m2 = ctx.saved_tensors
         s1, s2, ss, pad_main, pad_skip, gain, pm, ps, s0, need_x = ctx.cfg
         need = ctx.needs_input_grad
         if torch.is_grad_enabled():
@@ -81,14 +94,19 @@
         g = g.contiguous()
         front = need_x or need[1] or need[2]
         gx = gw1 = gb1 = gw2 = gb2 = gws = None
-        g2, gb2 = _lib.bias_act_bwd(g, y2, 0.2, _SQRT2 * gain, want_bias=need[4])
+        if m2 is not None:
+            g2, gb2 = _lib.bias_act_bwd_mask(g, m2, 0.2, _SQRT2 * gain, want_bias=need[4])
+        else:
+            g2, gb2 = _lib.bias_act_bwd(g, y2, 0.2, _SQRT2 * gain, want_bias=need[4])
         if need[3]:
             gw2 = _wgrad_plain(g2, yb, 'down', 3, s2)
         g1 = None
         if front:
             g_yb = _dgrad_raw(g2, w2, 'down', wscale=s2, wp=bwd2)
-            _, g_pad = _geometry(y1.shape[2:], k_main.shape, (1, 1), (1, 1), pm)
-            if tuple(k_main.shape) == (4, 4) and g_yb.shape[3] >= 4:
+            _, g_pad = _geometry(x.shape[2:], k_main.shape, (1, 1), (1, 1), pm)
+            if m1 is not None:
+                g1, gb1 = _lib.blur_gradact_mask(g_yb, m1, flipped_taps(k_main), g_pad, 0.2, _SQRT2)
+            elif tuple(k_main.shape) == (4, 4) and g_yb.shape[3] >= 4:
                 g1, gb1 = _lib.blur_gradact(g_yb, y1, flipped_taps(k_main), g_pad, 0.2, _SQRT2)
             else:
                 g1 = _lib.upfirdn2d_raw(g_yb, flipped_taps(k_main), (1, 1), (1, 1), g_pad)
diff --git a/transeditor_amd/op/styled_rgb.py b/transeditor_amd/op/styled_rgb.py
--- a/transeditor_amd/op/styled_rgb.py
+++ b/transeditor_amd/op/styled_rgb.py
@@ -5,6 +5,8 @@
 from .modconv import _DEFAULT_GRAPH, _composite, _dgrad_raw, _fwd_raw, _wgrad_raw, cache_of, keep_cache
 
 _SQRT2 = 2 ** 0.5
+
+USE_SIGN_MASKS = True
 
 
 def supported(x, w, wr):
@@ -19,12 +21,15 @@
         w3 = w.reshape(w.shape[0], w.shape[1], -1)
         d, wsq = _lib.demod_fwd(w3, s, wscale, eps)
         keep_cache(ctx)
-        if ctx.needs_input_grad[0]:
+        wp_bwd = am = None
+        if USE_SIGN_MASKS and any(ctx.needs_input_grad):
+            a, wp_bwd, am = _fwd_raw(x, w, '3x3', s, d, bias, 3, wscale, with_bwd_pack=ctx.needs_input_grad[0], with_mask=True)
+        elif ctx.needs_input_grad[0]:
             a, wp_bwd = _fwd_raw(x, w, '3x3', s, d, bias, 3, wscale, with_bwd_pack=True)
         else:
-            a, wp_bwd = _fwd_raw(x, w, '3x3', s, d, bias, 3, wscale), None
+            a = _fwd_raw(x, w, '3x3', s, d, bias, 3, wscale)
         rgb = _lib.rgb_fwd(a, wr.reshape(3, wr.shape[1]), sr, br, wscale_r)
-        ctx.save_for_backward(x, w, s, bias, wr, sr, br, d, wsq, a)
+        ctx.save_for_backward(x, w, s, bias, wr, sr, br, d, wsq, a, am)
         ctx.wp_bwd = wp_bwd
         ctx.cfg = (wscale, eps, wscale_r)
         ctx.set_materialize_grads(False)
@@ -37,7 +42,7 @@
 
     @staticmethod
     def _backward(ctx, ga, grgb):
-        x, w, s, bias, wr, sr, br, d, wsq, a = ctx.saved_tensors
+        x, w, s, bias, wr, sr, br, d, wsq, a, am = ctx.saved_tensors
         wscale, eps, wscale_r = ctx.cfg
         need = ctx.needs_input_grad
         if torch.is_grad_enabled():
@@ -72,14 +77,19 @@
                     gwr = gwr.reshape(wr.shape)
         if ga is None and grgb is None:
             return (None,) * 10
-        if grgb is not None and _lib.bias_act_bwd_rgb_supported(a.shape):
+        if grgb is not None and am is not None:
+            g, gb = _lib.bias_act_bwd_rgb_mask(ga, am, grgb, wr.reshape(3, Co), sr, wscale_r, 0.2, _SQRT2, want_bias=need[3])
+        elif grgb is not None and _lib.bias_act_bwd_rgb_supported(a.shape):
             g, gb = _lib.bias_act_bwd_rgb(ga, a, grgb, wr.reshape(3, Co), sr, wscale_r, 0.2, _SQRT2, want_bias=need[3])
         else:
             gt = ga
             if grgb is not None:
                 gr = _lib.rgb_dgrad(grgb, wr.reshape(3, Co), sr, Co, wscale_r)
                 gt = gr if gt is None else gt + gr
-            g, gb = _lib.bias_act_bwd(gt, a, 0.2, _SQRT2, want_bias=need[3])
+            if am is not None:
+                g, gb = _lib.bias_act_bwd_mask(gt, am, 0.2, _SQRT2, want_bias=need[3])
+            else:
+                g, gb = _lib.bias_act_bwd(gt, a, 0.2, _SQRT2, want_bias=need[3])
         gx = _dgrad_raw(g, w, '3x3', isc=d, osc=s, wscale=wscale, wp=ctx.wp_bwd) if need[0] else None
         gw = gs = None
         if need[1] or need[2]:
```
